# gongaa/Feedback-GNN

Measured on AMD Instinct MI355X. Metric: decoded codewords/sec, [[882,24]] 64-iter BP4 + feedback-GNN, higher is better.
Workload: dtype f32

## Files before the change

### feedback_gnn_amd/_lib.py

```python
import ctypes as C
import os
import subprocess

_HERE = os.path.dirname(os.path.abspath(__file__))
LIB_PATH = os.path.join(_HERE, "lib", "libfgnn_hip.so")
CSRC = os.path.join(_HERE, "csrc")

CN_TYPES = {"boxplus": 0, "boxplus-phi": 1, "minsum": 2}
ROWS_X_LOGIT, ROWS_Z_LOGIT, ROWS_HX_PERP, ROWS_HZ_PERP, ROWS_LX, ROWS_LZ = 0, 1, 2, 3, 4, 5


class FgnnError(RuntimeError):
    pass


def build(force=False, verbose=False):
    cmd = ["make", "-C", CSRC, "-j4"] + (["-B"] if force else [])
    res = subprocess.run(cmd, stdout=subprocess.PIPE, stderr=subprocess.STDOUT, text=True)
    if verbose or res.returncode != 0:
        print(res.stdout)
    if res.returncode != 0:
        raise FgnnError("building libfgnn_hip.so failed")
    return LIB_PATH


KERNEL_SOURCES = {
    "bp4": ("fgnn_bp4.hip", "fgnn_math.h", "fgnn_math_ranged.h", "fgnn_internal.h", "fgnn_rng.h", "fgnn_cn.h", "Makefile"),
    "gnn": ("fgnn_gnn.hip", "fgnn_math.h", "fgnn_internal.h", "fgnn_pk.h", "fgnn_mlp.h", "Makefile"),
    "gnnbp4": ("fgnn_gnnbp4.hip", "fgnn_math.h", "fgnn_internal.h", "fgnn_pk.h", "fgnn_mlp.h", "Makefile"),
}


def source_fingerprint(kind):
    import hashlib
    h = hashlib.sha256()
    for name in KERNEL_SOURCES[kind]:
        h.update(name.encode() + b"\0")
        with open(os.path.join(CSRC, name), "rb") as f:
            h.update(f.read())
        h.update(b"\0")
    return h.hexdigest()


def library_sha256(path=None):
    import hashlib
    h = hashlib.sha256()
    with open(path or os.environ.get("FGNN_LIB_PATH", LIB_PATH), "rb") as f:
        for blk in iter(lambda: f.read(1 << 20), b""):
            h.update(blk)
    return h.hexdigest()


_SIGNATURES = {
    "fgnn_last_error": (C.c_char_p, []),
    "fgnn_version": (C.c_int, []),
    "fgnn_graph_create": (C.c_int, [C.c_int, C.c_int, C.c_int, C.c_int, C.c_void_p, C.c_void_p, C.c_int, C.c_void_p,
                                    C.c_void_p, C.c_int, C.POINTER(C.c_void_p)]),
    "fgnn_graph_destroy": (None, [C.c_void_p]),
    "fgnn_graph_set_rows": (C.c_int, [C.c_void_p, C.c_int, C.c_int, C.c_int, C.c_void_p, C.c_void_p]),
    "fgnn_graph_set_launch": (C.c_int, [C.c_void_p, C.c_int, C.c_int]),
    "fgnn_graph_set_option": (C.c_int, [C.c_void_p, C.c_int, C.c_int]),
    "fgnn_graph_force_generic": (C.c_int, [C.c_void_p, C.c_int]),
    "fgnn_graph_info": (C.c_int, [C.c_void_p, C.c_void_p]),
    "fgnn_graph_edges": (C.c_int, [C.c_void_p, C.c_int, C.c_void_p, C.c_void_p]),
    "fgnn_profile_enable": (C.c_int, [C.c_void_p, C.c_int]),
    "fgnn_profile_read": (C.c_int, [C.c_void_p, C.c_void_p, C.c_void_p, C.c_void_p, C.c_int, C.c_void_p]),
    "fgnn_bp4_decode": (C.c_int, [C.c_void_p, C.c_int, C.c_int, C.c_float, C.c_void_p, C.c_float, C.c_void_p, C.c_void_p,
                                  C.c_int] + [C.c_void_p] * 10),
    "fgnn_bp4_decode_trace": (C.c_int, [C.c_void_p, C.c_int, C.c_int, C.c_float, C.c_void_p, C.c_float, C.c_void_p, C.c_void_p,
                                        C.c_int] + [C.c_void_p] * 10),
    "fgnn_weights_create": (C.c_int, [C.c_void_p, C.c_int, C.POINTER(C.c_void_p)]),
    "fgnn_weights_destroy": (None, [C.c_void_p]),
    "fgnn_feedback_gnn": (C.c_int, [C.c_void_p] * 7 + [C.c_int, C.c_void_p, C.c_void_p]),
    "fgnn_pauli_noise": (C.c_int, [C.c_uint64, C.c_float, C.c_uint64, C.c_int, C.c_int, C.c_void_p, C.c_void_p, C.c_void_p]),
    "fgnn_pauli_noise_xyz": (C.c_int, [C.c_uint64, C.c_float, C.c_float, C.c_float, C.c_uint64, C.c_int, C.c_int, C.c_void_p, C.c_void_p, C.c_void_p]),
    "fgnn_pauli_noise_wt": (C.c_int, [C.c_uint64, C.c_int, C.c_uint64, C.c_int, C.c_int, C.c_void_p, C.c_void_p, C.c_void_p]),
    "fgnn_pauli_noise_dev": (C.c_int, [C.c_uint64, C.c_float, C.c_void_p, C.c_uint64, C.c_int, C.c_int, C.c_void_p, C.c_void_p, C.c_void_p]),
    "fgnn_syndrome": (C.c_int, [C.c_void_p, C.c_void_p, C.c_void_p, C.c_int, C.c_void_p, C.c_void_p, C.c_void_p]),
    "fgnn_flag_update": (C.c_int, [C.c_void_p] * 5 + [C.c_int, C.c_void_p, C.c_void_p]),
    "fgnn_merge": (C.c_int, [C.c_void_p] * 3 + [C.c_int, C.c_int, C.c_void_p, C.c_void_p, C.c_void_p]),
    "fgnn_residual": (C.c_int, [C.c_void_p] * 5 + [C.c_int] + [C.c_void_p] * 4),
    "fgnn_count_flags": (C.c_int, [C.c_void_p, C.c_int, C.c_void_p, C.c_void_p]),
    "fgnn_count_flags_batches": (C.c_int, [C.c_void_p, C.c_int, C.c_int, C.c_void_p, C.c_void_p, C.c_void_p, C.c_void_p]),
    "fgnn_pack_decisions": (C.c_int, [C.c_void_p, C.c_void_p, C.c_int, C.c_int, C.c_void_p, C.c_void_p]),
    "fgnn_unpack_decisions": (C.c_int, [C.c_void_p, C.c_int, C.c_int, C.c_void_p, C.c_void_p, C.c_void_p]),
    "fgnn_sandwich_workspace_bytes": (C.c_size_t, [C.c_void_p, C.c_int]),
    "fgnn_sandwich_decode": (C.c_int, [C.c_void_p, C.c_int, C.c_void_p, C.c_void_p, C.c_void_p, C.c_void_p, C.c_float,
                                       C.c_void_p, C.c_void_p, C.c_int, C.c_int, C.c_void_p, C.c_void_p, C.c_void_p,
                                       C.c_void_p, C.c_void_p, C.c_size_t, C.c_void_p]),
    "fgnn_bp2_decode": (C.c_int, [C.c_void_p, C.c_int, C.c_int, C.c_float, C.c_void_p, C.c_float, C.c_void_p, C.c_int, C.c_void_p,
                                  C.c_void_p, C.c_void_p]),
    "fgnn_relay_decode": (C.c_int, [C.c_void_p, C.c_float, C.c_int, C.c_int, C.c_int, C.c_int, C.c_void_p, C.c_void_p, C.c_float,
                                    C.c_void_p, C.c_int, C.c_void_p, C.c_void_p, C.c_void_p]),
    "fgnn_relay4_decode": (C.c_int, [C.c_void_p, C.c_int, C.c_float, C.c_int, C.c_int, C.c_int, C.c_int, C.c_void_p, C.c_void_p, C.c_float,
                                     C.c_void_p, C.c_void_p, C.c_int, C.c_void_p, C.c_void_p, C.c_void_p, C.c_void_p]),
    "fgnn_bsc_noise": (C.c_int, [C.c_uint64, C.c_float, C.c_uint64, C.c_int, C.c_int, C.c_void_p, C.c_void_p]),
    "fgnn_residual_rows": (C.c_int, [C.c_void_p, C.c_int, C.c_int] + [C.c_void_p] * 4 + [C.c_int] + [C.c_void_p] * 4),
    "fgnn_graph_set_basis": (C.c_int, [C.c_void_p, C.c_int, C.c_int, C.c_void_p]),
    "fgnn_osd0": (C.c_int, [C.c_void_p, C.c_int, C.c_void_p, C.c_void_p, C.c_void_p, C.c_int, C.c_void_p, C.c_int, C.c_void_p, C.c_void_p]),
    "fgnn_osd": (C.c_int, [C.c_void_p, C.c_int, C.c_int, C.c_int, C.c_void_p, C.c_void_p, C.c_void_p, C.c_int, C.c_void_p, C.c_int,
                           C.c_void_p, C.c_void_p, C.c_void_p]),
    "fgnn_osd_resident": (C.c_int, [C.c_void_p, C.c_int, C.c_int, C.POINTER(C.c_int)]),
    "fgnn_osd_workspace_bytes": (C.c_int, [C.c_void_p, C.c_int, C.c_int, C.c_int, C.c_int, C.POINTER(C.c_size_t)]),
    "fgnn_osd_ws": (C.c_int, [C.c_void_p, C.c_int, C.c_int, C.c_int, C.c_void_p, C.c_void_p, C.c_void_p, C.c_int, C.c_void_p, C.c_int,
                              C.c_void_p, C.c_void_p, C.c_void_p, C.c_size_t, C.c_void_p]),
    "fgnn_compact": (C.c_int, [C.c_void_p, C.c_int, C.c_int, C.c_void_p, C.c_void_p, C.c_void_p]),
    "fgnn_gnnbp4_weights_create": (C.c_int, [C.c_void_p, C.c_int, C.c_int, C.c_int, C.POINTER(C.c_void_p)]),
    "fgnn_gnnbp4_weights_destroy": (None, [C.c_void_p]),
    "fgnn_gnnbp4_weights_create_general": (C.c_int, [C.c_void_p, C.c_void_p, C.c_void_p, C.c_int, C.POINTER(C.c_void_p)]),
    "fgnn_gnnbp4_weights_workspace_bytes": (C.c_size_t, [C.c_void_p, C.c_void_p, C.c_int]),
    "fgnn_gnnbp4_workspace_bytes": (C.c_size_t, [C.c_void_p, C.c_int]),
    "fgnn_gnnbp4_decode": (C.c_int, [C.c_void_p, C.c_void_p, C.c_int, C.c_void_p, C.c_void_p, C.c_int] + [C.c_void_p] * 6
                           + [C.c_size_t, C.c_void_p]),
    "fgnn_weights_create_general": (C.c_int, [C.c_void_p, C.c_void_p, C.c_int, C.c_int, C.POINTER(C.c_void_p)]),
    "fgnn_bp4_backward": (C.c_int, [C.c_void_p, C.c_int, C.c_float, C.c_void_p, C.c_void_p, C.c_void_p, C.c_int]
                          + [C.c_void_p] * 7),
    "fgnn_feedback_gnn_backward": (C.c_int, [C.c_void_p, C.c_void_p] + [C.c_void_p] * 5 + [C.c_int] + [C.c_void_p] * 9),
    "fgnn_feedback_gnn_backward_general": (C.c_int, [C.c_void_p, C.c_void_p] + [C.c_void_p] * 5 + [C.c_int] + [C.c_void_p] * 3
                                           + [C.c_int, C.c_void_p]),
    "fgnn_gnnbp4_grad_count": (C.c_int, [C.c_void_p, C.c_void_p, C.POINTER(C.c_int)]),
    "fgnn_gnnbp4_tape_bytes": (C.c_int, [C.c_void_p, C.c_void_p, C.c_int, C.c_int, C.POINTER(C.c_size_t)]),
    "fgnn_gnnbp4_backward_workspace_bytes": (C.c_int, [C.c_void_p, C.c_void_p, C.c_int, C.POINTER(C.c_size_t)]),
    "fgnn_gnnbp4_forward_tape": (C.c_int, [C.c_void_p, C.c_void_p, C.c_int, C.c_void_p, C.c_void_p, C.c_int, C.c_void_p, C.c_void_p,
                                           C.c_void_p, C.c_size_t, C.c_void_p]),
    "fgnn_gnnbp4_backward": (C.c_int, [C.c_void_p, C.c_void_p, C.c_int, C.c_void_p, C.c_void_p, C.c_int, C.c_void_p, C.c_size_t,
                                       C.c_void_p, C.c_void_p, C.c_void_p, C.c_int, C.c_void_p, C.c_size_t, C.c_void_p]),
}

ABI_SYMBOLS = tuple(_SIGNATURES)

_lib = None


def lib():
    global _lib
    if _lib is None:
        if not os.path.exists(LIB_PATH):
            raise FgnnError(f"{LIB_PATH} not found: run `python -c 'import __graft_entry__ as g; g.build()'` "
                            "(there is no CPU fallback for the decoder)")
        import torch
        override = os.environ.get("FGNN_LIB_PATH")
        L = C.CDLL(override or LIB_PATH)
        for name, (res, args) in _SIGNATURES.items():
            try:
                fn = getattr(L, name)
            except AttributeError:
                if override:
                    continue
                raise
            fn.restype = res
            fn.argtypes = args
        _lib = L
    return _lib


def check(rc):
    if rc != 0:
        msg = lib().fgnn_last_error().decode()
        if rc == -1:
            raise ValueError(msg)
        raise FgnnError(f"libfgnn_hip error {rc}: {msg}")
```

### feedback_gnn_amd/csrc/fgnn_bp4.hip

```cpp

#include <type_traits>

#include "fgnn_internal.h"
#include "fgnn_math.h"
#include "fgnn_math_ranged.h"
#include "fgnn_cn.h"

#ifndef FGNN_BP4_WAVES
#define FGNN_BP4_WAVES 7
#endif
#ifndef FGNN_HWT_PIN_CLIP_POINTS
#define FGNN_HWT_PIN_CLIP_POINTS 1
#endif
#ifndef FGNN_PHI_STAGE
#define FGNN_PHI_STAGE 1
#endif

namespace {

struct BpArgs {
    int B, num_iter, tpc, cpb, lds_per_cw, lch_off;
    float factor, llr_const;
    const float* llr_ch;
    const uint8_t* synd_x;
    const uint8_t* synd_z;
    const float* msg_init_x;
    const float* msg_init_z;
    float* llr_out;
    uint8_t* x_hat;
    uint8_t* z_hat;
    float* x_logit;
    float* z_logit;
    float* msg_out_x;
    float* msg_out_z;
    const int* index;
    int shortcut;
    int early_exit;
    int sig_off;
    int lreg;
    int hwt;
    uint8_t* flagged;
    int flag_off;
    float* gmem;
    float* trace_x;
    float* trace_z;
    int trace_off;
    float* tape_x;
    float* tape_z;
    int nt;
    int shared_lse;
};

template <bool HWT>
struct Mx {
    static __device__ __forceinline__ float softplus(float t) { return fg_softplus(t); }
    static __device__ __forceinline__ float lse2(float a, float b) { return fg_lse2_ranged(a, b); }
    static __device__ __forceinline__ float lse2_corr(float a, float b) { return fg_lse2_corr_ranged(a, b); }
    static __device__ __forceinline__ float phi(float x) { return fg_phi(x); }
};
template <>
struct Mx<true> {
    static __device__ __forceinline__ float exp(float x) { return __builtin_amdgcn_exp2f(x * FG_LOG2E); }
    static __device__ __forceinline__ float log(float x) { return __builtin_amdgcn_logf(x) * 0.693147182f; }
    static __device__ __forceinline__ float softplus(float t)
    {
        const float y = exp(FG_CLAMP(t, -87.0f, FG_SOFTPLUS_THRESH));
        const float r = (t < -FG_SOFTPLUS_THRESH) ? ((t < -87.0f) ? 0.0f : y) : log(1.0f + y);
        return (t > FG_SOFTPLUS_THRESH) ? t : r;
    }
    static __device__ __forceinline__ float lse2_corr(float a, float b)
    {
        const float y = exp(-FG_MIN(FG_ABS(a - b), 20.0f));
        return log(1.0f + y);
    }
    static __device__ __forceinline__ float lse2(float a, float b)
    {
        return lse2_corr(a, b) + FG_MAX(a, b);
    }
    static __device__ __forceinline__ float phi(float x)
    {
        const float xc = FG_CLAMP(x, FG_PHI_MIN, FG_PHI_MAX);
        const float y = exp(xc);
        const float sp = (xc > FG_SOFTPLUS_THRESH) ? xc : log(1.0f + y);
        float r = sp - log(y - 1.0f);
#if FGNN_HWT_PIN_CLIP_POINTS
        r = (x >= FG_PHI_MAX) ? 0.0f : r;
        r = (x <= FG_PHI_MIN) ? 16.6355324f : r;
#endif
        return r;
    }
};

template <bool HWT = false>
__device__ __forceinline__ float logit_row_opt(const float* llr, const int* __restrict__ col, int deg, float phi0, bool shortcut)
{
    if (shortcut) {
        unsigned neg = 0;
        bool sat = true;
        for (int j = 0; j < deg; ++j) {
            const float v = llr[col[j]];
            neg ^= (v < 0.0f);
            sat = sat && (FG_ABS(v) >= FG_PHI_MAX);
        }
        if (__all(sat)) return with_sign(phi0, neg);
    }
    return logit_row<Mx<HWT>>(llr, col, deg);
}

template <int N, bool HWT = false>
__device__ __forceinline__ void phi_n(const float (&x)[N], float (&out)[N])
{
    if constexpr (HWT) {
#pragma unroll
        for (int k = 0; k < N; ++k) out[k] = Mx<true>::phi(x[k]);
        return;
    }
    const float* tab = fg_log_tab();
    float xc[N], y[N];
    uint32_t eb1[N], eb2[N], j1[N], j2[N];
#pragma unroll
    for (int k = 0; k < N; ++k) {
        xc[k] = FG_CLAMP(x[k], FG_PHI_MIN, FG_PHI_MAX);
        y[k] = fg_exp(xc[k]);
        const uint32_t w1 = fg_f2u(1.0f + y[k]) - FG_LOG_OFFS;
        const uint32_t w2 = fg_f2u(y[k] - 1.0f) - FG_LOG_OFFS;
        eb1[k] = w1 & 0xff800000u;
        eb2[k] = w2 & 0xff800000u;
        j1[k] = (w1 >> 18) & 31u;
        j2[k] = (w2 >> 18) & 31u;
    }
    __builtin_amdgcn_sched_barrier(0);
    float rc1[N], lc1[N], rc2[N], lc2[N];
#pragma unroll
    for (int k = 0; k < N; ++k) {
        rc1[k] = tab[j1[k]];
        lc1[k] = tab[32 + j1[k]];
        rc2[k] = tab[j2[k]];
        lc2[k] = tab[32 + j2[k]];
    }
    __builtin_amdgcn_sched_barrier(0);
#pragma unroll
    for (int k = 0; k < N; ++k) {
        const float a = fg_u2f(fg_f2u(rc1[k]) - eb1[k]);
        const float r1 = FG_FMA(y[k], a, a - 1.0f);
        float sp = FG_FMA((float)(int32_t)eb1[k], FG_LN2_S23, lc1[k] + fg_log1p_small(r1));
        sp = (xc[k] > FG_SOFTPLUS_THRESH) ? xc[k] : sp;
        const float mm = fg_u2f(fg_f2u(y[k] - 1.0f) - eb2[k]);
        const float r2 = FG_FMA(mm, rc2[k], -1.0f);
        const float lg = FG_FMA((float)(int32_t)eb2[k], FG_LN2_S23, lc2[k] + fg_log1p_small(r2));
        out[k] = sp - lg;
    }
}

template <int DC, bool HWT = false, bool F1 = false>
__device__ __forceinline__ bool cn_phi_regular(float* msg, const int (&sl)[DC], uint32_t neg0, float factor, float phi0,
                                               bool shortcut)
{
    constexpr int H = (DC % FGNN_PHI_STAGE == 0) ? FGNN_PHI_STAGE : DC / 2;
    static_assert(DC % H == 0, "a phi stage must take a whole fraction of a check");
    float v[DC], aa[DC];
    uint32_t neg = neg0;
    bool sat = true;
#pragma unroll
    for (int j = 0; j < DC; ++j) {
        v[j] = slot_ref(msg, sl[j]);
        neg ^= fg_f2u(v[j]);
        sat = sat && (FG_ABS(v[j]) >= FG_PHI_MAX);
    }
    if (shortcut && __all(sat)) {
#pragma unroll
        for (int j = 0; j < DC; ++j) {
            const float o = fg_u2f(fg_f2u(phi0) | ((neg ^ fg_f2u(v[j])) & 0x80000000u));
            slot_ref(msg, sl[j]) = F1 ? o : o * factor;
        }
        return true;
    }
#pragma unroll
    for (int g0 = 0; g0 < DC; g0 += H) {
        float xa[H], oa[H];
#pragma unroll
        for (int j = 0; j < H; ++j) xa[j] = FG_ABS(v[g0 + j]);
        phi_n<H, HWT>(xa, oa);
#pragma unroll
        for (int j = 0; j < H; ++j) aa[g0 + j] = oa[j];
    }
    float T = 0.0f;
#pragma unroll
    for (int j = 0; j < DC; ++j) T = T + aa[j];
#pragma unroll
    for (int g0 = 0; g0 < DC; g0 += H) {
        float xa[H], oa[H];
#pragma unroll
        for (int j = 0; j < H; ++j) xa[j] = T - aa[g0 + j];
        phi_n<H, HWT>(xa, oa);
#pragma unroll
        for (int j = 0; j < H; ++j) {
            const float o = fg_u2f(fg_f2u(oa[j]) | ((neg ^ fg_f2u(v[g0 + j])) & 0x80000000u));
            slot_ref(msg, sl[g0 + j]) = F1 ? o : o * factor;
        }
    }
    return false;
}

template <int DC>
__device__ __forceinline__ void cn_tanh_regular(float* msg, const int (&sl)[DC], unsigned synd, float factor)
{
    float t[DC];
    float P = 1.0f;
#pragma unroll
    for (int j = 0; j < DC; ++j) {
        float tj = fg_tanh(slot_ref(msg, sl[j]) / 2.0f);
        tj = (tj == 0.0f) ? 1e-12f : tj;
        P = (j == 0) ? tj : P * tj;
        t[j] = tj;
    }
    P = P * (synd ? -1.0f : 1.0f);
    const float clipv = 0.99999988f;
#pragma unroll
    for (int j = 0; j < DC; ++j) {
        float q = fg_rcp_unit(t[j]) * P;
        q = (FG_ABS(q) < 1e-7f) ? 0.0f : q;
        q = FG_MIN(FG_MAX(q, -clipv), clipv);
        slot_ref(msg, sl[j]) = (2.0f * fg_atanh(q)) * factor;
    }
}

template <bool HWT = false>
__device__ __forceinline__ bool cn_phi_generic(float* msg, const int* __restrict__ slot, int deg, unsigned synd, float factor,
                                               float phi0, bool shortcut)
{
    if (shortcut) {
        unsigned neg = synd;
        bool sat = true;
        for (int j = 0; j < deg; ++j) {
            const float v = msg[slot[j]];
            neg ^= (v < 0.0f);
            sat = sat && (FG_ABS(v) >= FG_PHI_MAX);
        }
        if (__all(sat)) {
            for (int j = 0; j < deg; ++j) {
                const int s = slot[j];
                msg[s] = with_sign(phi0, neg ^ (unsigned)(msg[s] < 0.0f)) * factor;
            }
            return true;
        }
    }
    cn_update<FGNN_CN_BOXPLUS_PHI, Mx<HWT>>(msg, slot, deg, synd, factor);
    return false;
}

__device__ __forceinline__ float softplus_saturated(float t)
{
    const float y = fg_exp(FG_MIN(FG_MAX(t, -87.0f), 0.0f));
    return (t > 0.0f) ? t : ((t < -87.0f) ? 0.0f : y);
}

template <int CN_TYPE, int DVX, int DVZ, int DC, bool OPT, bool HWT = false, int NQ = 0, bool TRACE = false, bool GMEM = false, int LSE = 2,
          int NT = 0>
__global__ void __launch_bounds__(1024) __attribute__((amdgpu_waves_per_eu(NQ > 0 ? FGNN_BP4_WAVES - 1 : FGNN_BP4_WAVES)))
bp4_kernel(GraphDev g, BpArgs a)
{
    static_assert(!(HWT && OPT), "the hardware-transcendental variant is the fixed dataflow only: the exact shortcuts are proofs about fgnn_math.h");
    static_assert(!GMEM || (DVX == 0 && !OPT && !HWT && NQ == 0 && !TRACE), "the global-memory variant is the plain runtime-degree kernel");
    using MX = Mx<HWT>;
    FG_LOG_TAB_SETUP();
    constexpr bool REGULAR = DVX > 0;
    constexpr bool LREG = NQ > 0;
    constexpr int NQA = LREG ? NQ : 1;
    static_assert(NT == 0 || (DVX > 0 && CN_TYPE == FGNN_CN_BOXPLUS_PHI && !LREG && !TRACE && !GMEM), "compile-time trips: the regular phi kernel");
    constexpr int CT = LREG ? NQ : NT;
    const int tpc = NT > 0 ? 256 : a.tpc;
    const bool opt_shortcut = OPT && a.shortcut != 0;
    const bool opt_exit = OPT && a.early_exit != 0;
    const bool shl = LSE == 2 ? a.shared_lse != 0 : LSE == 1;
    extern __shared__ float lds[];
    const int cwl = NT > 0 ? 0 : threadIdx.x / tpc;
    const int lane = threadIdx.x - cwl * tpc;
    const int slot_b = NT > 0 ? blockIdx.x : blockIdx.x * a.cpb + cwl;
    const bool active = slot_b < a.B;
    const int b = (active && a.index) ? a.index[slot_b] : slot_b;
    float* msg;
    if constexpr (GMEM) msg = a.gmem + (size_t)slot_b * a.lds_per_cw;
    else if constexpr (NT > 0) msg = lds;
    else msg = lds + (size_t)cwl * a.lds_per_cw;
    float* Lch = msg + a.lch_off;
    const int n = g.n;

    constexpr bool CLOSED_OK = REGULAR && CN_TYPE == FGNN_CN_BOXPLUS_PHI && !LREG && !TRACE;
    const bool zero_start = REGULAR && !TRACE && !a.msg_init_x && !a.msg_init_z && a.num_iter > 0;
    const bool first_closed = CLOSED_OK && zero_start && !a.llr_ch;
    const bool first_peeled = zero_start && a.llr_ch != nullptr;
    const bool fill = !first_closed && !first_peeled;
    if (active) {
        if (fill) {
            for (int e = lane; e < g.E_x; e += tpc) msg[e] = a.msg_init_x ? a.msg_init_x[(size_t)b * g.E_x + e] : 0.0f;
            for (int e = lane; e < g.E_z; e += tpc)
                msg[g.E_x + e] = a.msg_init_z ? a.msg_init_z[(size_t)b * g.E_z + e] : 0.0f;
        }
        if (a.llr_ch && !LREG)
            for (int i = lane; i < 3 * n; i += tpc) Lch[i] = a.llr_ch[(size_t)b * 3 * n + i];
    }
    float lreg[3][NQA];
    if constexpr (LREG) {
#pragma unroll
        for (int i = 0; i < NQ; ++i) {
            const int v = lane + i * tpc;
            const bool in = active && v < n;
#pragma unroll
            for (int c = 0; c < 3; ++c) lreg[c][i] = in ? a.llr_ch[(size_t)b * 3 * n + c * n + v] : 0.0f;
        }
    }
    if (fill || (a.llr_ch && !LREG)) __syncthreads();

    const uint8_t* sx = a.synd_x + (size_t)b * g.m_x;
    const uint8_t* sz = a.synd_z + (size_t)b * g.m_z;
    const int lane_c = lane + (tpc >> 1) < tpc ? lane + (tpc >> 1) : lane - tpc + (tpc >> 1);

    const float phi0 = MX::phi(0.0f);
    (void)phi0;
    unsigned* sigw = reinterpret_cast<unsigned*>(msg + a.sig_off);
    int* flags = reinterpret_cast<int*>(sigw + n);
    bool a1 = false, a2 = false;
    if (opt_exit) {
        for (int v = lane; v < n; v += tpc) sigw[v] = fill ? 0xffffffffu : 0u;
        if (lane < 4) flags[lane] = 0;
        __syncthreads();
    }
    int it_begin = 0;
    if constexpr (CLOSED_OK) {
        if (first_closed) {
            const float L = a.llr_const;
            const float Y = (0.0f + 0.0f) + L, X = 0.0f + L, Z = 0.0f + L;
            const float nu_x = MX::softplus(-X) - MX::lse2(-(Z - 0.0f), -(Y - 0.0f));
            const float nu_z = MX::softplus(-Z) - MX::lse2(-(X - 0.0f), -(Y - 0.0f));
            if (active)
                for (int c = lane_c; c < g.m; c += tpc) {
                    const unsigned synd = (c < g.m_x ? sx[c] : sz[c - g.m_x]) & 1u;
                    const uint4 pk = reinterpret_cast<const uint4*>(g.cslot16)[c];
                    const unsigned w[4] = {pk.x, pk.y, pk.z, pk.w};
                    const float nu = c < g.m_x ? nu_x : nu_z;
                    const unsigned ng = nu < 0.0f;
                    unsigned neg = synd;
                    const float aa = MX::phi(FG_ABS(nu));
                    float T = 0.0f;
#pragma unroll
                    for (int j = 0; j < DC; ++j) {
                        neg ^= ng;
                        T = T + aa;
                    }
                    const float val = with_sign(MX::phi(T - aa), neg ^ ng) * a.factor;
#pragma unroll
                    for (int j = 0; j < DC; ++j) slot_ref(msg, (int)((w[j >> 1] >> ((j & 1) * 16)) & 0xffffu)) = val;
                }
            if (opt_exit) a1 = FG_ABS(nu_x) >= FG_PHI_MAX && FG_ABS(nu_z) >= FG_PHI_MAX;
            it_begin = 1;
            __syncthreads();
        }
    }
    const bool cn_one = a.cpb == 1, cn_f1 = a.factor == 1.0f;
    unsigned synd_bits = 0;
    if (active) {
        int i = 0;
        for (int c = lane_c; c < g.m && i < 32; c += tpc, ++i) synd_bits |= ((c < g.m_x ? sx[c] : sz[c - g.m_x]) & 1u) << i;
    }
    const bool synd_in_reg = (g.m + tpc - 1) / tpc <= 32;
    unsigned row_off = 16u * (unsigned)lane_c;
    auto trace_step = [&](const int k) __attribute__((always_inline)) {
        float* tlx = msg + a.trace_off;
        float* tlz = tlx + n;
        if (active && a.tape_x) {
            float* px = a.tape_x + ((size_t)k * a.B + b) * g.E_x;
            float* pz = a.tape_z + ((size_t)k * a.B + b) * g.E_z;
            for (int e = lane; e < g.E_x; e += tpc) px[e] = msg[e];
            for (int e = lane; e < g.E_z; e += tpc) pz[e] = msg[g.E_x + e];
        }
        if (active)
            for (int v = lane; v < n; v += tpc) {
                const int x0 = g.vptr_x[v], x1 = g.vptr_x[v + 1], z0 = g.vptr_z[v], z1 = g.vptr_z[v + 1];
                float Sz = 0.0f, Sx = 0.0f;
                for (int e = z0; e < z1; ++e) Sz = Sz + msg[e];
                for (int e = x0; e < x1; ++e) Sx = Sx + msg[e];
                const float lx = a.llr_ch ? Lch[v] : a.llr_const, ly = a.llr_ch ? Lch[n + v] : a.llr_const,
                            lz = a.llr_ch ? Lch[2 * n + v] : a.llr_const;
                const float Y = (Sz + Sx) + ly;
                const float X = Sz + lx;
                const float Z = Sx + lz;
                tlz[v] = MX::softplus(-X) - MX::lse2(-Z, -Y);
                tlx[v] = MX::softplus(-Z) - MX::lse2(-X, -Y);
            }
        __syncthreads();
        if (active) {
            float* tx = a.trace_x + ((size_t)k * a.B + b) * g.rows[0];
            for (int r = lane; r < g.rows[0]; r += tpc) {
                const int p0 = g.rptr[0][r];
                tx[r] = logit_row<Mx<HWT>>(tlx, g.rcol[0] + p0, g.rptr[0][r + 1] - p0);
            }
            float* tz = a.trace_z + ((size_t)k * a.B + b) * g.rows[1];
            for (int r = lane; r < g.rows[1]; r += tpc) {
                const int p0 = g.rptr[1][r];
                tz[r] = logit_row<Mx<HWT>>(tlz, g.rcol[1] + p0, g.rptr[1][r + 1] - p0);
            }
        }
    };
    if constexpr (TRACE) trace_step(0);
    if constexpr (REGULAR && !TRACE) {
        if (first_peeled && active) {
            auto vn_first = [&](const int v, const float lx, const float ly, const float lz) __attribute__((always_inline)) {
                const float Y = (0.0f + 0.0f) + ly;
                const float X = 0.0f + lx;
                const float Z = 0.0f + lz;
                const float numx = MX::softplus(-X);
                const float numz = MX::softplus(-Z);
                const float Ze = Z - 0.0f, Xe = X - 0.0f, Ye = Y - 0.0f;
                float ox, oz;
                if (shl) {
                    ox = numx - (MX::lse2_corr(-Z, -Y) + FG_MAX(-Ze, -Ye));
                    oz = numz - (MX::lse2_corr(-X, -Y) + FG_MAX(-Xe, -Ye));
                } else {
                    ox = numx - MX::lse2(-Ze, -Ye);
                    oz = numz - MX::lse2(-Xe, -Ye);
                }
                float* px = msg + v * DVX;
                float* pz = msg + g.E_x + v * DVZ;
#pragma unroll
                for (int k = 0; k < DVX; ++k) px[k] = ox;
#pragma unroll
                for (int k = 0; k < DVZ; ++k) pz[k] = oz;
            };
            if constexpr (LREG) {
#pragma unroll
                for (int i = 0; i < NQ; ++i) {
                    const int v = lane + i * tpc;
                    if (v < n) vn_first(v, lreg[0][i], lreg[1][i], lreg[2][i]);
                }
            } else {
                for (int v = lane; v < n; v += tpc) vn_first(v, Lch[v], Lch[n + v], Lch[2 * n + v]);
            }
        }
    }
    for (int it = it_begin; it < a.num_iter; ++it) {
        bool changed = false, cn_slow = false;
        auto vn_body = [&](const int v, const float lx, const float ly, const float lz) __attribute__((always_inline)) {
                if constexpr (REGULAR) {
                    float* px = msg + v * DVX;
                    float* pz = msg + g.E_x + v * DVZ;
                    float mx[DVX], mz[DVZ];
                    float Sz = 0.0f, Sx = 0.0f;
#pragma unroll
                    for (int k = 0; k < DVZ; ++k) { mz[k] = pz[k]; Sz = Sz + mz[k]; }
#pragma unroll
                    for (int k = 0; k < DVX; ++k) { mx[k] = px[k]; Sx = Sx + mx[k]; }
                    if (opt_exit) {
                        unsigned sig = 0;
#pragma unroll
                        for (int k = 0; k < DVX; ++k) sig |= sign_bit(mx[k]) << k;
#pragma unroll
                        for (int k = 0; k < DVZ; ++k) sig |= sign_bit(mz[k]) << (DVX + k);
                        if (sigw[v] != sig) {
                            changed = true;
                            sigw[v] = sig;
                        }
                    }
                    const float Y = (Sz + Sx) + ly;
                    const float X = Sz + lx;
                    const float Z = Sx + lz;
                    bool sat = opt_shortcut && FG_ABS(X) > FG_SOFTPLUS_THRESH && FG_ABS(Z) > FG_SOFTPLUS_THRESH;
                    if (shl) {
                        sat = sat && FG_ABS((-Z) - (-Y)) >= 20.0f && FG_ABS((-X) - (-Y)) >= 20.0f;
                    } else {
#pragma unroll
                        for (int k = 0; k < DVX; ++k) sat = sat && (FG_ABS((Z - mx[k]) - (Y - mx[k])) >= 20.0f);
#pragma unroll
                        for (int k = 0; k < DVZ; ++k) sat = sat && (FG_ABS((X - mz[k]) - (Y - mz[k])) >= 20.0f);
                    }
                    if (opt_shortcut && __all(sat)) {
                        const float numx = softplus_saturated(-X);
                        const float numz = softplus_saturated(-Z);
#pragma unroll
                        for (int k = 0; k < DVX; ++k) {
                            const float Ze = Z - mx[k], Ye = Y - mx[k];
                            px[k] = numx - (0.0f + FG_MAX(-Ze, -Ye));
                        }
#pragma unroll
                        for (int k = 0; k < DVZ; ++k) {
                            const float Xe = X - mz[k], Ye = Y - mz[k];
                            pz[k] = numz - (0.0f + FG_MAX(-Xe, -Ye));
                        }
                        return;
                    }
                    const float numx = MX::softplus(-X);
                    const float numz = MX::softplus(-Z);
                    if (shl) {
                        const float cx = MX::lse2_corr(-Z, -Y), cz = MX::lse2_corr(-X, -Y);
#pragma unroll
                        for (int k = 0; k < DVX; ++k) {
                            const float Ze = Z - mx[k], Ye = Y - mx[k];
                            px[k] = numx - (cx + FG_MAX(-Ze, -Ye));
                        }
#pragma unroll
                        for (int k = 0; k < DVZ; ++k) {
                            const float Xe = X - mz[k], Ye = Y - mz[k];
                            pz[k] = numz - (cz + FG_MAX(-Xe, -Ye));
                        }
                        return;
                    }
#pragma unroll
                    for (int k = 0; k < DVX; ++k) {
                        const float Ze = Z - mx[k], Ye = Y - mx[k];
                        px[k] = numx - MX::lse2(-Ze, -Ye);
                    }
#pragma unroll
                    for (int k = 0; k < DVZ; ++k) {
                        const float Xe = X - mz[k], Ye = Y - mz[k];
                        pz[k] = numz - MX::lse2(-Xe, -Ye);
                    }
                } else {
                    const int x0 = g.vptr_x[v], x1 = g.vptr_x[v + 1], z0 = g.vptr_z[v], z1 = g.vptr_z[v + 1];
                    float Sz = 0.0f, Sx = 0.0f;
                    for (int e = z0; e < z1; ++e) Sz = Sz + msg[e];
                    for (int e = x0; e < x1; ++e) Sx = Sx + msg[e];
                    const float Y = (Sz + Sx) + ly;
                    const float X = Sz + lx;
                    const float Z = Sx + lz;
                    if (opt_shortcut) {
                        bool sat = FG_ABS(X) > FG_SOFTPLUS_THRESH && FG_ABS(Z) > FG_SOFTPLUS_THRESH;
                        if (shl) sat = sat && FG_ABS((-Z) - (-Y)) >= 20.0f && FG_ABS((-X) - (-Y)) >= 20.0f;
                        unsigned sig = 0;
                        for (int e = x0; e < x1; ++e) {
                            const float mm = msg[e];
                            sat = sat && (shl || FG_ABS((Z - mm) - (Y - mm)) >= 20.0f);
                            sig |= sign_bit(mm) << (e - x0);
                        }
                        for (int e = z0; e < z1; ++e) {
                            const float mm = msg[e];
                            sat = sat && (shl || FG_ABS((X - mm) - (Y - mm)) >= 20.0f);
                            sig |= sign_bit(mm) << ((x1 - x0) + (e - z0));
                        }
                        if (opt_exit && sigw[v] != sig) {
                            changed = true;
                            sigw[v] = sig;
                        }
                        if (__all(sat)) {
                            const float nx = softplus_saturated(-X), nz = softplus_saturated(-Z);
                            for (int e = x0; e < x1; ++e) {
                                const float mm = msg[e];
                                const float Ze = Z - mm, Ye = Y - mm;
                                msg[e] = nx - (0.0f + FG_MAX(-Ze, -Ye));
                            }
                            for (int e = z0; e < z1; ++e) {
                                const float mm = msg[e];
                                const float Xe = X - mm, Ye = Y - mm;
                                msg[e] = nz - (0.0f + FG_MAX(-Xe, -Ye));
                            }
                            return;
                        }
                    }
                    const float numx = MX::softplus(-X);
                    const float numz = MX::softplus(-Z);
                    if (shl) {
                        const float cx = MX::lse2_corr(-Z, -Y), cz = MX::lse2_corr(-X, -Y);
                        for (int e = x0; e < x1; ++e) {
                            float m = msg[e];
                            float Ze = Z - m, Ye = Y - m;
                            msg[e] = numx - (cx + FG_MAX(-Ze, -Ye));
                        }
                        for (int e = z0; e < z1; ++e) {
                            float m = msg[e];
                            float Xe = X - m, Ye = Y - m;
                            msg[e] = numz - (cz + FG_MAX(-Xe, -Ye));
                        }
                        return;
                    }
                    for (int e = x0; e < x1; ++e) {
                        float m = msg[e];
                        float Ze = Z - m, Ye = Y - m;
                        msg[e] = numx - MX::lse2(-Ze, -Ye);
                    }
                    for (int e = z0; e < z1; ++e) {
                        float m = msg[e];
                        float Xe = X - m, Ye = Y - m;
                        msg[e] = numz - MX::lse2(-Xe, -Ye);
                    }
                }
            };
        if (active && !(first_peeled && it == 0)) {
            if constexpr (LREG) {
#pragma unroll
                for (int i = 0; i < NQ; ++i) {
                    const int v = lane + i * tpc;
                    if (v < n) vn_body(v, lreg[0][i], lreg[1][i], lreg[2][i]);
                }
            } else if constexpr (NT > 0) {
#pragma unroll
                for (int i = 0; i < NT; ++i) {
                    const int v = lane + i * 256;
                    if (i + 1 < NT || v < n) vn_body(v, a.llr_const, a.llr_const, a.llr_const);
                }
            } else {
                for (int v = lane; v < n; v += tpc) {
                    if (a.llr_ch) vn_body(v, Lch[v], Lch[n + v], Lch[2 * n + v]);
                    else vn_body(v, a.llr_const, a.llr_const, a.llr_const);
                }
            }
        }
        if (opt_exit && changed) flags[2 * (it & 1)] = 1;
        __syncthreads();
        if (opt_exit && lane == 0) {
            flags[2 * ((it + 1) & 1)] = 0;
            flags[2 * ((it + 1) & 1) + 1] = 0;
        }
        if constexpr (REGULAR && CT > 0 && CN_TYPE == FGNN_CN_BOXPLUS_PHI) {
            auto cn_trips = [&](auto f1) __attribute__((always_inline)) {
                constexpr bool F1 = decltype(f1)::value;
                const char* rows = reinterpret_cast<const char*>(g.cslot16);
#pragma unroll
                for (int i = 0; i < CT; ++i) {
                    const bool in = (!LREG && i + 1 < CT) || lane_c + i * tpc < g.m;
                    if (in) {
                        const char* base = rows + (size_t)i * (size_t)(16u * (unsigned)tpc);
                        asm volatile("" : "+v"(row_off));
                        if constexpr (NT > 0) asm volatile("" : "+s"(base));
                        typedef unsigned Row __attribute__((ext_vector_type(4)));
                        const Row pk = *(const __attribute__((address_space(1))) Row*)(base + row_off);
                        const unsigned w[4] = {pk.x, pk.y, pk.z, pk.w};
                        int sl[DC];
#pragma unroll
                        for (int j = 0; j < DC; ++j) sl[j] = (int)((w[j >> 1] >> ((j & 1) * 16)) & 0xffffu);
                        const bool fast = cn_phi_regular<DC, HWT, F1>(lds, sl, synd_bits << (31 - i), F1 ? 1.0f : a.factor, phi0, opt_shortcut);
                        cn_slow = !fast || cn_slow;
                    }
                }
            };
            if (active) {
                if (cn_f1) cn_trips(std::true_type{});
                else cn_trips(std::false_type{});
            }
        } else if (active) {
            int ci = 0;
            for (int c = lane_c; c < g.m; c += tpc, ++ci) {
                const unsigned synd = synd_in_reg ? (synd_bits >> ci) & 1u : (c < g.m_x ? sx[c] : sz[c - g.m_x]) & 1u;
                if constexpr (REGULAR) {
                    const uint4 pk = reinterpret_cast<const uint4*>(g.cslot16)[c];
                    const unsigned w[4] = {pk.x, pk.y, pk.z, pk.w};
                    int sl[DC];
#pragma unroll
                    for (int j = 0; j < DC; ++j) sl[j] = (int)((w[j >> 1] >> ((j & 1) * 16)) & 0xffffu);
                    if constexpr (CN_TYPE == FGNN_CN_BOXPLUS_PHI) {
                        bool fast;
                        if (cn_one && cn_f1) fast = cn_phi_regular<DC, HWT, true>(lds, sl, synd << 31, 1.0f, phi0, opt_shortcut);
                        else if (cn_one) fast = cn_phi_regular<DC, HWT, false>(lds, sl, synd << 31, a.factor, phi0, opt_shortcut);
                        else fast = cn_phi_regular<DC, HWT, false>(msg, sl, synd << 31, a.factor, phi0, opt_shortcut);
                        cn_slow = !fast || cn_slow;
                    } else if constexpr (CN_TYPE == FGNN_CN_MINSUM) {
                        cn_minsum_regular<DC>(msg, sl, DC, synd, a.factor);
                    } else {
                        cn_tanh_regular<DC>(msg, sl, synd, a.factor);
                    }
                } else {
                    const int c0 = g.cptr[c], deg = g.cptr[c + 1] - c0;
                    if constexpr (CN_TYPE == FGNN_CN_BOXPLUS_PHI)
                        cn_slow = !cn_phi_generic<HWT>(msg, g.cslot + c0, deg, synd, a.factor, phi0, opt_shortcut) || cn_slow;
                    else cn_update<CN_TYPE, Mx<HWT>>(msg, g.cslot + c0, deg, synd, a.factor);
                }
            }
        }
        if (opt_exit && cn_slow) flags[2 * (it & 1) + 1] = 1;
        __syncthreads();
        if (opt_exit) {
            const bool stable = a1 && a2 && flags[2 * (it & 1)] == 0;
            a2 = a1;
            a1 = flags[2 * (it & 1) + 1] == 0;
            if (stable) break;
        }
        if constexpr (TRACE) trace_step(it + 1);
    }

    if (active) {
        if (a.msg_out_x)
            for (int e = lane; e < g.E_x; e += tpc) a.msg_out_x[(size_t)b * g.E_x + e] = msg[e];
        if (a.msg_out_z)
            for (int e = lane; e < g.E_z; e += tpc) a.msg_out_z[(size_t)b * g.E_z + e] = msg[g.E_x + e];
    }
    auto total_body = [&](const int v, const float lx, const float ly, const float lz) __attribute__((always_inline)) {
            const int x0 = g.vptr_x[v], x1 = g.vptr_x[v + 1], z0 = g.vptr_z[v], z1 = g.vptr_z[v + 1];
            float Sz = 0.0f, Sx = 0.0f;
            for (int e = z0; e < z1; ++e) Sz = Sz + msg[e];
            for (int e = x0; e < x1; ++e) Sx = Sx + msg[e];
            const float Y = (Sz + Sx) + ly;
            const float X = Sz + lx;
            const float Z = Sx + lz;
            float* o = a.llr_out + (size_t)b * 3 * n;
            o[v] = X;
            o[n + v] = Y;
            o[2 * n + v] = Z;
            int d = 0;
            float best = 0.0f;
            if (X < best) { best = X; d = 1; }
            if (Z < best) { best = Z; d = 2; }
            if (Y < best) { best = Y; d = 3; }
            a.x_hat[(size_t)b * n + v] = (uint8_t)(d & 1);
            a.z_hat[(size_t)b * n + v] = (uint8_t)(d >> 1);
    };
    if (active) {
        if constexpr (LREG) {
#pragma unroll
            for (int i = 0; i < NQ; ++i) {
                const int v = lane + i * tpc;
                if (v < n) total_body(v, lreg[0][i], lreg[1][i], lreg[2][i]);
            }
        } else {
            for (int v = lane; v < n; v += tpc) {
                if (a.llr_ch) total_body(v, Lch[v], Lch[n + v], Lch[2 * n + v]);
                else total_body(v, a.llr_const, a.llr_const, a.llr_const);
            }
        }
    }
    if (a.flagged) {
        uint8_t* dec = reinterpret_cast<uint8_t*>(msg + a.flag_off);
        unsigned* fword = reinterpret_cast<unsigned*>(dec + ((n + 3) & ~3));
        __syncthreads();
        if (active)
            for (int v = lane; v < n; v += tpc) {
                dec[v] = (uint8_t)(a.x_hat[(size_t)b * n + v] | (a.z_hat[(size_t)b * n + v] << 1));
            }
        if (lane == 0) *fword = 0u;
        __syncthreads();
        unsigned mine = 0;
        if (active)
            for (int c = lane; c < g.m; c += tpc) {
                const int sh = c < g.m_x ? 1 : 0;
                unsigned par = (c < g.m_x ? sx[c] : sz[c - g.m_x]) & 1u;
                for (int e = g.cptr[c]; e < g.cptr[c + 1]; ++e) par ^= (dec[g.cvn[e]] >> sh) & 1u;
                mine |= par;
            }
        if (mine) atomicOr(fword, 1u);
        __syncthreads();
        if (active && lane == 0) a.flagged[b] = (uint8_t)(*fword != 0u);
    }
    if (!a.x_logit && !a.z_logit) return;
    __syncthreads();
    float* llx = msg;
    float* llz = msg + n;
    if (active)
        for (int v = lane; v < n; v += tpc) {
            const float* o = a.llr_out + (size_t)b * 3 * n;
            const float X = o[v], Y = o[n + v], Z = o[2 * n + v];
            const bool sat = opt_shortcut && FG_ABS(X) > FG_SOFTPLUS_THRESH && FG_ABS(Z) > FG_SOFTPLUS_THRESH &&
                             FG_ABS((-Z) - (-Y)) >= 20.0f && FG_ABS((-X) - (-Y)) >= 20.0f;
            if (opt_shortcut && __all(sat)) {
                llz[v] = softplus_saturated(-X) - (0.0f + FG_MAX(-Z, -Y));
                llx[v] = softplus_saturated(-Z) - (0.0f + FG_MAX(-X, -Y));
                continue;
            }
            llz[v] = MX::softplus(-X) - MX::lse2(-Z, -Y);
            llx[v] = MX::softplus(-Z) - MX::lse2(-X, -Y);
        }
    __syncthreads();
    if (active) {
        if (a.x_logit)
            for (int r = lane; r < g.rows[0]; r += tpc) {
                const int p0 = g.rptr[0][r];
                a.x_logit[(size_t)b * g.rows[0] + r] = logit_row_opt<HWT>(llx, g.rcol[0] + p0, g.rptr[0][r + 1] - p0, phi0, opt_shortcut);
            }
        if (a.z_logit)
            for (int r = lane; r < g.rows[1]; r += tpc) {
                const int p0 = g.rptr[1][r];
                a.z_logit[(size_t)b * g.rows[1] + r] = logit_row_opt<HWT>(llz, g.rcol[1] + p0, g.rptr[1][r + 1] - p0, phi0, opt_shortcut);
            }
    }
}

using Bp4Kernel = void (*)(GraphDev, BpArgs);

template <int NQ, bool OPT, int LSE, int NT = 0>
constexpr Bp4Kernel bp4_lse_kernel = bp4_kernel<FGNN_CN_BOXPLUS_PHI, 3, 3, 6, OPT, false, NQ, false, false, LSE, NT>;
constexpr Bp4Kernel bp4_lse_kernels[3][2][2] = {
    {{bp4_lse_kernel<0, false, 0>, bp4_lse_kernel<0, false, 1>}, {bp4_lse_kernel<0, true, 0>, bp4_lse_kernel<0, true, 1>}},
    {{bp4_lse_kernel<4, false, 0>, bp4_lse_kernel<4, false, 1>}, {bp4_lse_kernel<4, true, 0>, bp4_lse_kernel<4, true, 1>}},
    {{bp4_lse_kernel<5, false, 0>, bp4_lse_kernel<5, false, 1>}, {bp4_lse_kernel<5, true, 0>, bp4_lse_kernel<5, true, 1>}}};

constexpr Bp4Kernel bp4_nt_kernels[2][2][2] = {
    {{bp4_lse_kernel<0, false, 0, 4>, bp4_lse_kernel<0, false, 1, 4>}, {bp4_lse_kernel<0, true, 0, 4>, bp4_lse_kernel<0, true, 1, 4>}},
    {{bp4_lse_kernel<0, false, 0, 5>, bp4_lse_kernel<0, false, 1, 5>}, {bp4_lse_kernel<0, true, 0, 5>, bp4_lse_kernel<0, true, 1, 5>}}};

template <int CN_TYPE, int DVX, int DVZ, int DC>
int launch_bp4_k(const fgnn_graph* g, const BpArgs& a, const LaunchGeom& L, size_t lds_bytes, hipStream_t st)
{
    Bp4Kernel kern = a.shortcut ? bp4_kernel<CN_TYPE, DVX, DVZ, DC, true> : bp4_kernel<CN_TYPE, DVX, DVZ, DC, false>;
    if constexpr ((DVX == 3 && DVZ == 3 && DC == 6) || DVX == 0) {
        if (a.trace_x) kern = bp4_kernel<CN_TYPE, DVX, DVZ, DC, false, false, 0, true>;
    }
    if constexpr (CN_TYPE == FGNN_CN_BOXPLUS_PHI) {
        if (a.hwt) kern = bp4_kernel<CN_TYPE, DVX, DVZ, DC, false, true>;
        if constexpr (DVX == 3 && DVZ == 3 && DC == 6) {
            if (!a.trace_x && !a.hwt) kern = bp4_lse_kernels[a.lreg ? a.lreg - 3 : 0][a.shortcut][a.shared_lse];
            if (!a.trace_x && !a.hwt && a.nt) kern = bp4_nt_kernels[a.nt - 4][a.shortcut][a.shared_lse];
        }
    }
    return fgnn_launch(kern, dim3(L.blocks), dim3(L.threads), lds_bytes, st, g->d, a);
}

struct Bp4Plan {
    size_t lds_bytes;
    bool gmem;
    size_t ws_bytes;
};

template <int CN_TYPE>
int launch_bp4(const fgnn_graph* g, const BpArgs& a, const LaunchGeom& L, const Bp4Plan& p, hipStream_t st)
{
    if (p.gmem)
        return fgnn_launch(bp4_kernel<CN_TYPE, 0, 0, 0, false, false, 0, false, true>, dim3(L.blocks), dim3(L.threads), 0, st, g->d, a);
    const GraphDev& d = g->d;
    if (d.cslot16 && !g->force_generic) {
        if (d.dvx == 3 && d.dvz == 3 && d.dc == 6) return launch_bp4_k<CN_TYPE, 3, 3, 6>(g, a, L, p.lds_bytes, st);
        if (d.dvx == 4 && d.dvz == 4 && d.dc == 8 && !a.trace_x) return launch_bp4_k<CN_TYPE, 4, 4, 8>(g, a, L, p.lds_bytes, st);
    }
    return launch_bp4_k<CN_TYPE, 0, 0, 0>(g, a, L, p.lds_bytes, st);
}

Bp4Plan plan_bp4(const fgnn_graph* g, int cn_type, const LaunchGeom& L, BpArgs& a, bool gmem = false)
{
    const GraphDev& d = g->d;
    const int n = d.n;
    const bool trace = a.trace_x != nullptr, phi = cn_type == FGNN_CN_BOXPLUS_PHI;
    auto round4 = [](int floats) { return (floats + 3) & ~3; };
    a.shared_lse = g->bp4_shared_lse ? 1 : 0;
    a.hwt = (g->hw_transcendentals && phi && !trace && !gmem) ? 1 : 0;
    a.shortcut = (g->shortcut && !a.hwt && !trace && !gmem) ? 1 : 0;
    a.lch_off = d.E > 2 * n ? d.E : 2 * n;
    const int per_thread = (n + L.tpc - 1) / L.tpc, per_thread_c = (d.m + L.tpc - 1) / L.tpc;
    const int trips = per_thread > per_thread_c ? per_thread : per_thread_c;
    const bool r336 = d.cslot16 && !g->force_generic && d.dvx == 3 && d.dvz == 3 && d.dc == 6;
    const bool fixed_trips = !trace && !a.hwt && !gmem && phi && L.cpb == 1 && r336;
    a.lreg = (a.llr_ch && fixed_trips && trips <= 5) ? (trips <= 4 ? 4 : 5) : 0;
    a.nt = (!a.llr_ch && fixed_trips && L.tpc == 256 && per_thread == per_thread_c && (trips == 4 || trips == 5)) ? trips : 0;
    int per = a.lch_off + ((a.llr_ch && !a.lreg) ? 3 * n : 0);
    a.trace_off = 0;
    if (trace) {
        a.trace_off = per;
        per += 2 * n;
    }
    if (!gmem) per = round4(per);
    a.sig_off = per;
    int tail = 0;
    a.early_exit = (a.shortcut && g->early_exit && d.max_vdeg <= 32 && phi && L.cpb == 1 && a.num_iter > 2) ? 1 : 0;
    if (a.early_exit) {
        if (((size_t)per * L.cpb + n + 4) * sizeof(float) <= FGNN_LDS_BUDGET) tail += n + 4;
        else a.early_exit = 0;
    }
    a.flag_off = 0;
    if (a.flagged) {
        const int need = round4(n) / 4 + 1;
        if (a.lch_off >= 2 * n + need) {
            a.flag_off = 2 * n;
        } else {
            a.flag_off = per + tail;
            tail += need;
        }
    }
    if (gmem) {
        a.lds_per_cw = round4(per + tail);
        return {0, true, (size_t)L.blocks * (size_t)a.lds_per_cw * sizeof(float)};
    }
    a.lds_per_cw = per;
    const size_t lds_bytes = ((size_t)per * L.cpb + tail) * sizeof(float);
    if (lds_bytes > FGNN_LDS_BUDGET) return plan_bp4(g, cn_type, L, a, true);
    return {lds_bytes, false, 0};
}

}

static int bp4_decode_core(const fgnn_graph* g, int cn_type, int num_iter, float normalization_factor, const float* llr_ch,
                           float llr_const, const uint8_t* synd_x, const uint8_t* synd_z, int B, const float* msg_init_x,
                           const float* msg_init_z, float* llr_out, uint8_t* x_hat, uint8_t* z_hat, float* x_logit,
                           float* z_logit, float* msg_out_x, float* msg_out_z, const int* index, uint8_t* flagged,
                           float* trace_x, float* trace_z, float* tape_x, float* tape_z, void* stream)
{
    if (!g) return fgnn_fail(FGNN_ERR_ARG, "graph is NULL");
    if (B < 0 || num_iter < 0) return fgnn_fail(FGNN_ERR_ARG, "B and num_iter must be >= 0");
    if (cn_type < 0 || cn_type > 2) return fgnn_fail(FGNN_ERR_ARG, "Unknown node type.");
    if ((x_logit && !g->d.rptr[0]) || (z_logit && !g->d.rptr[1]))
        return fgnn_fail(FGNN_ERR_STATE, "logit row sets not installed (fgnn_graph_set_rows)");
    if (B == 0) return FGNN_OK;
    if (!synd_x || !synd_z || !llr_out || !x_hat || !z_hat) return fgnn_fail(FGNN_ERR_ARG, "required buffer is NULL");
    FGNN_DEVICE_GUARD(g->device);
    const LaunchGeom L = fgnn_geom(g, B);
    if (flagged && L.cpb != 1) return fgnn_fail(FGNN_ERR_STATE, "the fused flag test needs one codeword per workgroup");
    BpArgs a;
    a.B = B;
    a.num_iter = num_iter;
    a.tpc = L.tpc;
    a.cpb = L.cpb;
    a.factor = normalization_factor;
    a.llr_const = llr_const;
    a.llr_ch = llr_ch;
    a.synd_x = synd_x;
    a.synd_z = synd_z;
    a.msg_init_x = msg_init_x;
    a.msg_init_z = msg_init_z;
    a.llr_out = llr_out;
    a.x_hat = x_hat;
    a.z_hat = z_hat;
    a.x_logit = x_logit;
    a.z_logit = z_logit;
    a.msg_out_x = msg_out_x;
    a.msg_out_z = msg_out_z;
    a.index = index;
    a.flagged = flagged;
    a.gmem = nullptr;
    a.trace_x = trace_x;
    a.trace_z = trace_z;
    a.tape_x = tape_x;
    a.tape_z = tape_z;
    const Bp4Plan p = plan_bp4(g, cn_type, L, a);
    hipStream_t st = static_cast<hipStream_t>(stream);
    if (p.gmem) {
        if (trace_x) return fgnn_fail(FGNN_ERR_ARG, "code too large for the LDS-resident trace kernel");
        if (L.cpb != 1) return fgnn_fail(FGNN_ERR_STATE, "the global-memory BP4 variant needs one codeword per workgroup");
        const size_t row_bytes = (size_t)a.lds_per_cw * sizeof(float);
        {
            size_t free_b = 0, total_b = 0;
            if (hipMemGetInfo(&free_b, &total_b) == hipSuccess && p.ws_bytes > free_b)
                return fgnn_fail(FGNN_ERR_ARG, "code too large for the LDS-resident kernel: the global-memory variant needs " +
                                                   std::to_string(p.ws_bytes >> 20) + " MiB of workspace for " + std::to_string(B) +
                                                   " codewords (" + std::to_string(row_bytes >> 10) + " KiB each) and " +
                                                   std::to_string(free_b >> 20) + " MiB are free: decode in batches of at most " +
                                                   std::to_string(free_b / (row_bytes * 2)) + " codewords");
        }
        void* ws = nullptr;
        FGNN_HIP_CHECK(hipMallocAsync(&ws, p.ws_bytes, st));
        a.gmem = static_cast<float*>(ws);
    }
    fgnn_prof_scope prof(g, st);
    int rc;
    switch (cn_type) {
    case FGNN_CN_BOXPLUS_PHI: rc = launch_bp4<FGNN_CN_BOXPLUS_PHI>(g, a, L, p, st); break;
    case FGNN_CN_MINSUM: rc = launch_bp4<FGNN_CN_MINSUM>(g, a, L, p, st); break;
    default: rc = launch_bp4<FGNN_CN_BOXPLUS>(g, a, L, p, st); break;
    }
    if (a.gmem) (void)hipFreeAsync(a.gmem, st);
    if (rc == FGNN_OK) prof.done(num_iter, B);
    return rc;
}

int fgnn_bp4_decode_impl(const fgnn_graph* g, int cn_type, int num_iter, float normalization_factor, const float* llr_ch,
                         float llr_const, const uint8_t* synd_x, const uint8_t* synd_z, int B, const float* msg_init_x,
                         const float* msg_init_z, float* llr_out, uint8_t* x_hat, uint8_t* z_hat, float* x_logit,
                         float* z_logit, float* msg_out_x, float* msg_out_z, const int* index, uint8_t* flagged, void* stream)
{
    return bp4_decode_core(g, cn_type, num_iter, normalization_factor, llr_ch, llr_const, synd_x, synd_z, B, msg_init_x, msg_init_z,
                           llr_out, x_hat, z_hat, x_logit, z_logit, msg_out_x, msg_out_z, index, flagged, nullptr, nullptr, nullptr,
                           nullptr, stream);
}

extern "C" int fgnn_bp4_decode_trace(const fgnn_graph* g, int cn_type, int num_iter, float normalization_factor,
                                     const float* llr_ch, float llr_const, const uint8_t* synd_x, const uint8_t* synd_z, int B,
                                     const float* msg_init_x, const float* msg_init_z, float* llr_out, uint8_t* x_hat,
                                     uint8_t* z_hat, float* x_logit_trace, float* z_logit_trace, float* tape_x,
                                     float* tape_z, void* stream)
{
    if (B == 0 && g) return FGNN_OK;
    if (!x_logit_trace || !z_logit_trace) return fgnn_fail(FGNN_ERR_ARG, "trace buffer is NULL");
    if ((tape_x == nullptr) != (tape_z == nullptr)) return fgnn_fail(FGNN_ERR_ARG, "tape_x and tape_z go together");
    if (g && (!g->d.rptr[0] || !g->d.rptr[1]))
        return fgnn_fail(FGNN_ERR_STATE, "logit row sets not installed (fgnn_graph_set_rows)");
    return bp4_decode_core(g, cn_type, num_iter, normalization_factor, llr_ch, llr_const, synd_x, synd_z, B, msg_init_x, msg_init_z,
                           llr_out, x_hat, z_hat, nullptr, nullptr, nullptr, nullptr, nullptr, nullptr, x_logit_trace,
                           z_logit_trace, tape_x, tape_z, stream);
}

extern "C" int fgnn_bp4_decode(const fgnn_graph* g, int cn_type, int num_iter, float normalization_factor,
                               const float* llr_ch, float llr_const, const uint8_t* synd_x, const uint8_t* synd_z, int B,
                               const float* msg_init_x, const float* msg_init_z, float* llr_out, uint8_t* x_hat,
                               uint8_t* z_hat, float* x_logit, float* z_logit, float* msg_out_x, float* msg_out_z,
                               void* stream)
{
    return fgnn_bp4_decode_impl(g, cn_type, num_iter, normalization_factor, llr_ch, llr_const, synd_x, synd_z, B, msg_init_x,
                                msg_init_z, llr_out, x_hat, z_hat, x_logit, z_logit, msg_out_x, msg_out_z, nullptr, nullptr, stream);
}
```

### feedback_gnn_amd/csrc/fgnn_channel.hip

```cpp
#include "fgnn_internal.h"
#include "fgnn_math.h"
#include "fgnn_rng.h"

namespace {

template <bool XYZ>
__global__ void __launch_bounds__(256) pauli_kernel(uint64_t seed, float p, fg_pauli_thr thr_in, uint64_t first,
                                                    const unsigned long long* __restrict__ base, int B, int n, int nblk,
                                                    uint8_t* __restrict__ ex, uint8_t* __restrict__ ez)
{
    const long long t = (long long)blockIdx.x * blockDim.x + threadIdx.x;
    if (t >= (long long)B * nblk) return;
    if (base) first += (uint64_t)*base;
    const int b = (int)(t / nblk), blk = (int)(t - (long long)b * nblk);
    const fg_pauli_thr thr = XYZ ? thr_in : fg_pauli_thresholds(p);
    float u[4];
    fg_uniform4(seed, first + (uint64_t)b, (uint32_t)blk, u);
    const int q0 = blk * 4;
#pragma unroll
    for (int k = 0; k < 4; ++k)
        if (q0 + k < n) {
            ex[(size_t)b * n + q0 + k] = fg_pauli_x(u[k], thr);
            ez[(size_t)b * n + q0 + k] = fg_pauli_z(u[k], thr);
        }
}

__global__ void __launch_bounds__(256) pauli_wt_kernel(uint64_t seed, int wt, uint64_t first, int B, int n, uint8_t* __restrict__ ex,
                                                       uint8_t* __restrict__ ez)
{
    extern __shared__ unsigned short perm_all[];
    const int wave = threadIdx.x >> 6, lane = threadIdx.x & 63;
    const int b = blockIdx.x * 4 + wave;
    if (b >= B) return;
    unsigned short* perm = perm_all + (size_t)wave * n;
    uint8_t* rx = ex + (size_t)b * n;
    uint8_t* rz = ez + (size_t)b * n;
    for (int v = lane; v < n; v += 64) {
        perm[v] = (unsigned short)v;
        rx[v] = 0;
        rz[v] = 0;
    }
    __builtin_amdgcn_fence(__ATOMIC_RELEASE, "workgroup");
    __builtin_amdgcn_wave_barrier();
    __builtin_amdgcn_fence(__ATOMIC_ACQUIRE, "workgroup");
    if (lane != 0) return;
    float up[4] = {0, 0, 0, 0}, ut[4] = {0, 0, 0, 0};
    for (int i = 0; i < wt; ++i) {
        if ((i & 3) == 0) {
            fg_uniform4s(seed, first + (uint64_t)b, (uint32_t)(i >> 2), 1u, up);
            fg_uniform4s(seed, first + (uint64_t)b, (uint32_t)(i >> 2), 2u, ut);
        }
        const int j = i + fg_fy_pick(up[i & 3], n - i);
        const unsigned short t = perm[i];
        perm[i] = perm[j];
        perm[j] = t;
        const float u = ut[i & 3];
        rx[perm[i]] = (uint8_t)(u < (2.0f / 3.0f));
        rz[perm[i]] = (uint8_t)(u > (1.0f / 3.0f));
    }
}

__device__ __forceinline__ unsigned row_parity(const uint8_t* x, const int* __restrict__ col, int p0, int p1)
{
    unsigned a = 0;
    for (int j = p0; j < p1; ++j) a ^= x[col[j]];
    return a & 1u;
}

__global__ void __launch_bounds__(1024) syndrome_kernel(GraphDev g, int B, int tpc, int cpb, const uint8_t* __restrict__ ex,
                                                        const uint8_t* __restrict__ ez, uint8_t* __restrict__ sx,
                                                        uint8_t* __restrict__ sz)
{
    extern __shared__ uint8_t sm[];
    const int cwl = threadIdx.x / tpc, lane = threadIdx.x - cwl * tpc, b = blockIdx.x * cpb + cwl;
    const bool active = b < B;
    const int n = g.n;
    uint8_t* lx = sm + (size_t)cwl * 2 * n;
    uint8_t* lz = lx + n;
    if (active)
        for (int v = lane; v < n; v += tpc) {
            lx[v] = ex[(size_t)b * n + v];
            lz[v] = ez[(size_t)b * n + v];
        }
    __syncthreads();
    if (!active) return;
    for (int c = lane; c < g.m; c += tpc) {
        const int p0 = g.cptr[c], p1 = g.cptr[c + 1];
        if (c < g.m_x) sx[(size_t)b * g.m_x + c] = (uint8_t)row_parity(lz, g.cvn, p0, p1);
        else sz[(size_t)b * g.m_z + (c - g.m_x)] = (uint8_t)row_parity(lx, g.cvn, p0, p1);
    }
}

__global__ void __launch_bounds__(1024) flag_kernel(GraphDev g, int B, int tpc, int cpb, const uint8_t* __restrict__ xh,
                                                    const uint8_t* __restrict__ zh, const uint8_t* __restrict__ sx,
                                                    const uint8_t* __restrict__ sz, uint8_t* __restrict__ errors,
                                                    const int* __restrict__ index)
{
    extern __shared__ uint8_t sm[];
    const int cwl = threadIdx.x / tpc, lane = threadIdx.x - cwl * tpc, slot = blockIdx.x * cpb + cwl;
    const bool active = slot < B;
    const int b = (active && index) ? index[slot] : slot;
    const int n = g.n;
    unsigned* neq = reinterpret_cast<unsigned*>(sm);
    uint8_t* lx = sm + ((cpb * sizeof(unsigned) + 15) & ~size_t(15)) + (size_t)cwl * 2 * n;
    uint8_t* lz = lx + n;
    if (lane == 0) neq[cwl] = 0;
    if (active)
        for (int v = lane; v < n; v += tpc) {
            lx[v] = xh[(size_t)b * n + v];
            lz[v] = zh[(size_t)b * n + v];
        }
    __syncthreads();
    unsigned mine = 0;
    if (active)
        for (int c = lane; c < g.m; c += tpc) {
            const int p0 = g.cptr[c], p1 = g.cptr[c + 1];
            if (c < g.m_x) mine |= row_parity(lz, g.cvn, p0, p1) ^ (sx[(size_t)b * g.m_x + c] & 1u);
            else mine |= row_parity(lx, g.cvn, p0, p1) ^ (sz[(size_t)b * g.m_z + (c - g.m_x)] & 1u);
        }
    if (mine) atomicOr(&neq[cwl], 1u);
    __syncthreads();
    if (active && lane == 0) errors[b] = (uint8_t)((errors[b] != 0) && (neq[cwl] != 0));
}

__global__ void __launch_bounds__(256) merge_kernel(const uint8_t* __restrict__ errors, const uint8_t* __restrict__ xu,
                                                    const uint8_t* __restrict__ zu, long long total, int n,
                                                    uint8_t* __restrict__ xh, uint8_t* __restrict__ zh,
                                                    const int* __restrict__ index)
{
    long long i = (long long)blockIdx.x * blockDim.x + threadIdx.x;
    if (i >= total) return;
    if (index) {
        const long long slot = i / n;
        i = (long long)index[slot] * n + (i - slot * n);
    }
    if (errors[i / n]) {
        xh[i] = xu[i];
        zh[i] = zu[i];
    }
}

__global__ void __launch_bounds__(1024) residual_kernel(GraphDev g, int RX, int RZ, int B, int tpc, int cpb, const uint8_t* __restrict__ ex,
                                                        const uint8_t* __restrict__ ez, const uint8_t* __restrict__ xh,
                                                        const uint8_t* __restrict__ zh, uint8_t* __restrict__ s_hat,
                                                        uint8_t* __restrict__ ls_hat, uint8_t* __restrict__ flags)
{
    extern __shared__ uint8_t sm[];
    const int cwl = threadIdx.x / tpc, lane = threadIdx.x - cwl * tpc, b = blockIdx.x * cpb + cwl;
    const bool active = b < B;
    const int n = g.n;
    unsigned* fl = reinterpret_cast<unsigned*>(sm);
    uint8_t* xd = sm + ((cpb * sizeof(unsigned) + 15) & ~size_t(15)) + (size_t)cwl * 2 * n;
    uint8_t* zd = xd + n;
    if (lane == 0) fl[cwl] = 0;
    __syncthreads();
    unsigned any_diff = 0;
    if (active)
        for (int v = lane; v < n; v += tpc) {
            xd[v] = ex[(size_t)b * n + v] ^ xh[(size_t)b * n + v];
            zd[v] = ez[(size_t)b * n + v] ^ zh[(size_t)b * n + v];
            any_diff |= xd[v] | zd[v];
        }
    if (any_diff) atomicOr(&fl[cwl], 4u);
    __syncthreads();
    unsigned mine = 0;
    if (active && ((fl[cwl] & 4u) || s_hat || ls_hat)) {
        const int ms = g.m_z + g.m_x;
        for (int c = lane; c < g.m; c += tpc) {
            const int p0 = g.cptr[c], p1 = g.cptr[c + 1];
            unsigned bit;
            int pos;
            if (c < g.m_x) { bit = row_parity(zd, g.cvn, p0, p1); pos = g.m_z + c; }
            else { bit = row_parity(xd, g.cvn, p0, p1); pos = c - g.m_x; }
            if (s_hat) s_hat[(size_t)b * ms + pos] = (uint8_t)bit;
            mine |= bit;
        }
        const int r0 = g.rows[RX], r1 = g.rows[RZ];
        for (int r = lane; r < r0 + r1; r += tpc) {
            unsigned bit;
            if (r < r0) bit = row_parity(xd, g.rcol[RX], g.rptr[RX][r], g.rptr[RX][r + 1]);
            else bit = row_parity(zd, g.rcol[RZ], g.rptr[RZ][r - r0], g.rptr[RZ][r - r0 + 1]);
            if (ls_hat) ls_hat[(size_t)b * (r0 + r1) + r] = (uint8_t)bit;
            mine |= bit << 1;
        }
    }
    if (mine) atomicOr(&fl[cwl], mine);
    __syncthreads();
    if (active && lane == 0 && flags) flags[b] = (uint8_t)(fl[cwl] & 3u);
}

__global__ void __launch_bounds__(256) count_kernel(const uint8_t* __restrict__ flags, int B, unsigned long long* counts)
{
    __shared__ unsigned sh[2];
    if (threadIdx.x < 2) sh[threadIdx.x] = 0;
    __syncthreads();
    unsigned f = 0, l = 0;
    for (int i = blockIdx.x * blockDim.x + threadIdx.x; i < B; i += gridDim.x * blockDim.x) {
        f += flags[i] & 1u;
        l += (flags[i] >> 1) & 1u;
    }
    if (f) atomicAdd(&sh[0], f);
    if (l) atomicAdd(&sh[1], l);
    __syncthreads();
    if (threadIdx.x == 0) {
        if (sh[0]) atomicAdd(&counts[0], (unsigned long long)sh[0]);
        if (sh[1]) atomicAdd(&counts[1], (unsigned long long)sh[1]);
        if (blockIdx.x == 0) atomicAdd(&counts[2], (unsigned long long)B);
    }
}

__global__ void __launch_bounds__(256) count_batches_kernel(const uint8_t* __restrict__ flags, int batch, unsigned* __restrict__ part)
{
    __shared__ unsigned sh[2];
    if (threadIdx.x < 2) sh[threadIdx.x] = 0;
    __syncthreads();
    const uint8_t* f0 = flags + (size_t)blockIdx.x * batch;
    unsigned f = 0, l = 0;
    for (int i = threadIdx.x; i < batch; i += blockDim.x) {
        f += f0[i] & 1u;
        l += (f0[i] >> 1) & 1u;
    }
    if (f) atomicAdd(&sh[0], f);
    if (l) atomicAdd(&sh[1], l);
    __syncthreads();
    if (threadIdx.x < 2) part[2 * blockIdx.x + threadIdx.x] = sh[threadIdx.x];
}

__global__ void count_scan_kernel(const unsigned* __restrict__ part, int num_batches, int batch, unsigned long long* counts,
                                  unsigned long long* ring)
{
    if (blockIdx.x != 0 || threadIdx.x != 0) return;
    unsigned long long c0 = counts[0], c1 = counts[1], c2 = counts[2];
    for (int j = 0; j < num_batches; ++j) {
        c0 += part[2 * j];
        c1 += part[2 * j + 1];
        c2 += (unsigned long long)batch;
        ring[3 * j] = c0;
        ring[3 * j + 1] = c1;
        ring[3 * j + 2] = c2;
    }
    counts[0] = c0;
    counts[1] = c1;
    counts[2] = c2;
}

__global__ void __launch_bounds__(256) pack_kernel(const uint8_t* __restrict__ x_hat, const uint8_t* __restrict__ z_hat,
                                                   long long total, int n, int nb, uint8_t* __restrict__ packed)
{
    const long long i = (long long)blockIdx.x * blockDim.x + threadIdx.x;
    if (i >= total) return;
    const long long b = i / nb;
    const int byte = (int)(i - b * nb);
    const uint8_t* xr = x_hat + b * n;
    const uint8_t* zr = z_hat + b * n;
    unsigned v = 0;
#pragma unroll
    for (int k = 0; k < 8; ++k) {
        const int pos = byte * 8 + k;
        unsigned bit = 0;
        if (pos < n) bit = xr[pos] & 1u;
        else if (pos < 2 * n) bit = zr[pos - n] & 1u;
        v |= bit << (7 - k);
    }
    packed[i] = (uint8_t)v;
}

__global__ void __launch_bounds__(256) unpack_kernel(const uint8_t* __restrict__ packed, long long total, int n, int nb,
                                                     uint8_t* __restrict__ x_hat, uint8_t* __restrict__ z_hat)
{
    const long long i = (long long)blockIdx.x * blockDim.x + threadIdx.x;
    if (i >= total) return;
    const long long b = i / (2 * n);
    const int pos = (int)(i - b * 2 * n);
    const uint8_t v = (uint8_t)((packed[b * nb + (pos >> 3)] >> (7 - (pos & 7))) & 1u);
    if (pos < n) x_hat[b * n + pos] = v;
    else z_hat[b * n + pos - n] = v;
}

}

extern "C" int fgnn_pack_decisions(const uint8_t* x_hat, const uint8_t* z_hat, int B, int n, uint8_t* packed, void* stream)
{
    if (B < 0 || n <= 0) return fgnn_fail(FGNN_ERR_ARG, "bad pack arguments");
    if (B == 0) return FGNN_OK;
    if (!x_hat || !z_hat || !packed) return fgnn_fail(FGNN_ERR_ARG, "bad pack arguments");
    const int nb = (2 * n + 7) / 8;
    const long long total = (long long)B * nb;
    return fgnn_launch(pack_kernel, dim3((unsigned)((total + 255) / 256)), dim3(256), 0, static_cast<hipStream_t>(stream), x_hat,
                       z_hat, total, n, nb, packed);
}

extern "C" int fgnn_unpack_decisions(const uint8_t* packed, int B, int n, uint8_t* x_hat, uint8_t* z_hat, void* stream)
{
    if (B < 0 || n <= 0) return fgnn_fail(FGNN_ERR_ARG, "bad unpack arguments");
    if (B == 0) return FGNN_OK;
    if (!x_hat || !z_hat || !packed) return fgnn_fail(FGNN_ERR_ARG, "bad unpack arguments");
    const int nb = (2 * n + 7) / 8;
    const long long total = (long long)B * 2 * n;
    return fgnn_launch(unpack_kernel, dim3((unsigned)((total + 255) / 256)), dim3(256), 0, static_cast<hipStream_t>(stream), packed,
                       total, n, nb, x_hat, z_hat);
}

extern "C" int fgnn_pauli_noise(uint64_t seed, float p, uint64_t first_sample, int B, int n, uint8_t* noise_x,
                                uint8_t* noise_z, void* stream)
{
    if (B < 0 || n <= 0) return fgnn_fail(FGNN_ERR_ARG, "bad noise arguments");
    if (B == 0) return FGNN_OK;
    if (!noise_x || !noise_z) return fgnn_fail(FGNN_ERR_ARG, "bad noise arguments");
    const int nblk = (n + 3) / 4;
    const long long total = (long long)B * nblk;
    return fgnn_launch(pauli_kernel<false>, dim3((unsigned)((total + 255) / 256)), dim3(256), 0, static_cast<hipStream_t>(stream), seed,
                       p, fg_pauli_thr{0.0f, 0.0f, 0.0f}, first_sample, static_cast<const unsigned long long*>(nullptr), B, n, nblk,
                       noise_x, noise_z);
}

extern "C" int fgnn_pauli_noise_xyz(uint64_t seed, float px, float py, float pz, uint64_t first_sample, int B, int n,
                                    uint8_t* noise_x, uint8_t* noise_z, void* stream)
{
    if (B < 0 || n <= 0 || !(px == px && py == py && pz == pz)) return fgnn_fail(FGNN_ERR_ARG, "bad noise arguments");
    if (B == 0) return FGNN_OK;
    if (!noise_x || !noise_z) return fgnn_fail(FGNN_ERR_ARG, "bad noise arguments");
    const int nblk = (n + 3) / 4;
    const long long total = (long long)B * nblk;
    return fgnn_launch(pauli_kernel<true>, dim3((unsigned)((total + 255) / 256)), dim3(256), 0, static_cast<hipStream_t>(stream), seed,
                       0.0f, fg_pauli_thresholds_xyz(px, py, pz), first_sample, static_cast<const unsigned long long*>(nullptr), B, n,
                       nblk, noise_x, noise_z);
}

extern "C" int fgnn_pauli_noise_dev(uint64_t seed, float p, const uint64_t* first_sample_dev, uint64_t offset, int B, int n,
                                    uint8_t* noise_x, uint8_t* noise_z, void* stream)
{
    if (B < 0 || n <= 0 || !(p >= 0.0f && p <= 1.0f)) return fgnn_fail(FGNN_ERR_ARG, "bad noise arguments");
    if (B == 0) return FGNN_OK;
    if (!noise_x || !noise_z || !first_sample_dev) return fgnn_fail(FGNN_ERR_ARG, "bad noise arguments");
    const int nblk = (n + 3) / 4;
    const long long total = (long long)B * nblk;
    return fgnn_launch(pauli_kernel<false>, dim3((unsigned)((total + 255) / 256)), dim3(256), 0, static_cast<hipStream_t>(stream), seed,
                       p, fg_pauli_thr{0.0f, 0.0f, 0.0f}, offset, reinterpret_cast<const unsigned long long*>(first_sample_dev), B, n,
                       nblk, noise_x, noise_z);
}

extern "C" int fgnn_pauli_noise_wt(uint64_t seed, int wt, uint64_t first_sample, int B, int n, uint8_t* noise_x, uint8_t* noise_z,
                                   void* stream)
{
    if (B < 0 || n <= 0 || n > 65535 || wt < 0 || wt > n) return fgnn_fail(FGNN_ERR_ARG, "bad fixed-weight noise arguments");
    if (B == 0) return FGNN_OK;
    if (!noise_x || !noise_z) return fgnn_fail(FGNN_ERR_ARG, "bad fixed-weight noise arguments");
    return fgnn_launch(pauli_wt_kernel, dim3((B + 3) / 4), dim3(256), (size_t)4 * n * sizeof(unsigned short),
                       static_cast<hipStream_t>(stream), seed, wt, first_sample, B, n, noise_x, noise_z);
}

extern "C" int fgnn_syndrome(const fgnn_graph* g, const uint8_t* noise_x, const uint8_t* noise_z, int B, uint8_t* synd_x,
                             uint8_t* synd_z, void* stream)
{
    if (!g || B < 0) return fgnn_fail(FGNN_ERR_ARG, "bad syndrome arguments");
    if (B == 0) return FGNN_OK;
    if (!noise_x || !noise_z || !synd_x || !synd_z) return fgnn_fail(FGNN_ERR_ARG, "bad syndrome arguments");
    FGNN_DEVICE_GUARD(g->device);
    LaunchGeom L = fgnn_geom(g, B);
    size_t lds = (size_t)L.cpb * 2 * g->d.n;
    return fgnn_launch(syndrome_kernel, dim3(L.blocks), dim3(L.threads), lds, static_cast<hipStream_t>(stream), g->d, B, L.tpc,
                       L.cpb, noise_x, noise_z, synd_x, synd_z);
}

int fgnn_flag_update_impl(const fgnn_graph* g, const uint8_t* x_hat, const uint8_t* z_hat, const uint8_t* synd_x,
                          const uint8_t* synd_z, int B, uint8_t* errors, const int* index, void* stream)
{
    if (!g || B < 0) return fgnn_fail(FGNN_ERR_ARG, "bad flag arguments");
    if (B == 0) return FGNN_OK;
    if (!x_hat || !z_hat || !synd_x || !synd_z || !errors) return fgnn_fail(FGNN_ERR_ARG, "bad flag arguments");
    FGNN_DEVICE_GUARD(g->device);
    LaunchGeom L = fgnn_geom(g, B);
    size_t lds = ((L.cpb * sizeof(unsigned) + 15) & ~size_t(15)) + (size_t)L.cpb * 2 * g->d.n;
    return fgnn_launch(flag_kernel, dim3(L.blocks), dim3(L.threads), lds, static_cast<hipStream_t>(stream), g->d, B, L.tpc, L.cpb,
                       x_hat, z_hat, synd_x, synd_z, errors, index);
}

extern "C" int fgnn_flag_update(const fgnn_graph* g, const uint8_t* x_hat, const uint8_t* z_hat, const uint8_t* synd_x,
                                const uint8_t* synd_z, int B, uint8_t* errors, void* stream)
{
    return fgnn_flag_update_impl(g, x_hat, z_hat, synd_x, synd_z, B, errors, nullptr, stream);
}

int fgnn_merge_impl(const uint8_t* errors, const uint8_t* x_upd, const uint8_t* z_upd, int B, int n, uint8_t* x_hat, uint8_t* z_hat,
                    const int* index, void* stream)
{
    if (B < 0 || n <= 0) return fgnn_fail(FGNN_ERR_ARG, "bad merge arguments");
    if (B == 0) return FGNN_OK;
    if (!errors || !x_upd || !z_upd || !x_hat || !z_hat) return fgnn_fail(FGNN_ERR_ARG, "bad merge arguments");
    const long long total = (long long)B * n;
    return fgnn_launch(merge_kernel, dim3((unsigned)((total + 255) / 256)), dim3(256), 0, static_cast<hipStream_t>(stream), errors,
                       x_upd, z_upd, total, n, x_hat, z_hat, index);
}

extern "C" int fgnn_merge(const uint8_t* errors, const uint8_t* x_upd, const uint8_t* z_upd, int B, int n, uint8_t* x_hat,
                          uint8_t* z_hat, void* stream)
{
    return fgnn_merge_impl(errors, x_upd, z_upd, B, n, x_hat, z_hat, nullptr, stream);
}

extern "C" int fgnn_residual_rows(const fgnn_graph* g, int rows_x, int rows_z, const uint8_t* noise_x, const uint8_t* noise_z,
                                  const uint8_t* x_hat, const uint8_t* z_hat, int B, uint8_t* s_hat, uint8_t* ls_hat, uint8_t* flags,
                                  void* stream)
{
    if (!g || B < 0) return fgnn_fail(FGNN_ERR_ARG, "bad residual arguments");
    if (rows_x < 0 || rows_x > 5 || rows_z < 0 || rows_z > 5 || !g->d.rptr[rows_x] || !g->d.rptr[rows_z])
        return fgnn_fail(FGNN_ERR_STATE, "row sets for the residual check not installed (fgnn_graph_set_rows)");
    if (B == 0) return FGNN_OK;
    if (!noise_x || !noise_z || !x_hat || !z_hat) return fgnn_fail(FGNN_ERR_ARG, "bad residual arguments");
    FGNN_DEVICE_GUARD(g->device);
    LaunchGeom L = fgnn_geom(g, B);
    size_t lds = ((L.cpb * sizeof(unsigned) + 15) & ~size_t(15)) + (size_t)L.cpb * 2 * g->d.n;
    return fgnn_launch(residual_kernel, dim3(L.blocks), dim3(L.threads), lds, static_cast<hipStream_t>(stream), g->d, rows_x, rows_z, B,
                       L.tpc, L.cpb, noise_x, noise_z, x_hat, z_hat, s_hat, ls_hat, flags);
}

extern "C" int fgnn_residual(const fgnn_graph* g, const uint8_t* noise_x, const uint8_t* noise_z, const uint8_t* x_hat,
                             const uint8_t* z_hat, int B, uint8_t* s_hat, uint8_t* ls_hat, uint8_t* flags, void* stream)
{
    return fgnn_residual_rows(g, FGNN_ROWS_HX_PERP, FGNN_ROWS_HZ_PERP, noise_x, noise_z, x_hat, z_hat, B, s_hat, ls_hat, flags, stream);
}

extern "C" int fgnn_count_flags_batches(const uint8_t* flags, int num_batches, int batch, uint64_t* counts, uint64_t* ring,
                                        uint32_t* scratch, void* stream)
{
    if (!flags || !counts || !ring || !scratch || num_batches < 0 || batch <= 0) return fgnn_fail(FGNN_ERR_ARG, "bad count arguments");
    if (num_batches == 0) return FGNN_OK;
    hipStream_t st = static_cast<hipStream_t>(stream);
    const int rc = fgnn_launch(count_batches_kernel, dim3(num_batches), dim3(256), 0, st, flags, batch, scratch);
    if (rc) return rc;
    return fgnn_launch(count_scan_kernel, dim3(1), dim3(64), 0, st, scratch, num_batches, batch,
                       reinterpret_cast<unsigned long long*>(counts), reinterpret_cast<unsigned long long*>(ring));
}

extern "C" int fgnn_count_flags(const uint8_t* flags, int B, uint64_t* counts, void* stream)
{
    if (!counts || B < 0) return fgnn_fail(FGNN_ERR_ARG, "bad count arguments");
    if (B == 0) return FGNN_OK;
    if (!flags) return fgnn_fail(FGNN_ERR_ARG, "bad count arguments");
    int blocks = (B + 255) / 256;
    if (blocks > 1024) blocks = 1024;
    return fgnn_launch(count_kernel, dim3(blocks), dim3(256), 0, static_cast<hipStream_t>(stream), flags, B,
                       reinterpret_cast<unsigned long long*>(counts));
}
```

### feedback_gnn_amd/csrc/fgnn_gnn.hip

```cpp
#include <algorithm>
#include <cstring>

#include "fgnn_internal.h"
#include "fgnn_math.h"
#include "fgnn_mlp.h"
#include "fgnn_pk.h"

namespace {

constexpr int HID = 40;
constexpr int MSG = 20;

struct GnnArgs {
    int B, tpc, cpb, lds_per_cw;
    const float* llr;
    const float* logit_hx;
    const float* logit_hz;
    const uint8_t* synd_x;
    const uint8_t* synd_z;
    float* out;
    const int* index;
    int nsplit;
};

__device__ __forceinline__ void edge_mlp(float gv, float X, float Y, float Z, scalar_fp w1t, scalar_fp b1, scalar_fp w2, scalar_fp b2,
                                         float (&msg)[MSG])
{
#pragma unroll
    for (int i = 0; i < MSG; ++i) msg[i] = 0.0f;
#pragma unroll 2
    for (int j = 0; j < HID; ++j) {
        scalar_fp r = w1t + j * 4;
        float a = 0.0f;
        a = FG_FMA(gv, r[0], a);
        a = FG_FMA(X, r[1], a);
        a = FG_FMA(Y, r[2], a);
        a = FG_FMA(Z, r[3], a);
        const float h = fg_tanh(a + b1[j]);
        scalar_fp r2 = w2 + j * MSG;
#pragma unroll
        for (int i = 0; i < MSG; ++i) msg[i] = FG_FMA(h, r2[i], msg[i]);
    }
#pragma unroll
    for (int i = 0; i < MSG; ++i) msg[i] = msg[i] + b2[i];
}

__device__ __forceinline__ void side_mean(const GraphDev& g, const int* __restrict__ vptr, int v, const float* gcn,
                                          float X, float Y, float Z, scalar_fp w1t, scalar_fp b1, scalar_fp w2, scalar_fp b2,
                                          float (&mean)[MSG])
{
    const int e0 = vptr[v], e1 = vptr[v + 1];
    float msg[MSG];
#pragma unroll
    for (int i = 0; i < MSG; ++i) mean[i] = 0.0f;
    for (int e = e0; e < e1; ++e) {
        edge_mlp(gcn[g.vchk[e]], X, Y, Z, w1t, b1, w2, b2, msg);
#pragma unroll
        for (int i = 0; i < MSG; ++i) mean[i] = (e == e0) ? msg[i] : mean[i] + msg[i];
    }
    const int deg = e1 - e0;
    if (deg > 0) {
        const float fd = (float)deg;
#pragma unroll
        for (int i = 0; i < MSG; ++i) mean[i] = mean[i] / fd;
    }
}

__device__ __forceinline__ void side_mean_factored(const GraphDev& g, const int* __restrict__ vptr, int v, const float* gcn,
                                                   float X, float Y, float Z, scalar_fp w1t, scalar_fp b1, scalar_fp w2, scalar_fp b2,
                                                   float (&mean)[MSG])
{
    const int e0 = vptr[v], e1 = vptr[v + 1];
#pragma unroll
    for (int i = 0; i < MSG; ++i) mean[i] = 0.0f;
#pragma unroll 2
    for (int j = 0; j < HID; ++j) {
        scalar_fp r = w1t + j * 4;
        float a = 0.0f;
        a = FG_FMA(X, r[1], a);
        a = FG_FMA(Y, r[2], a);
        a = FG_FMA(Z, r[3], a);
        const float pb = a + b1[j];
        float hs = 0.0f;
        for (int e = e0; e < e1; ++e) {
            const float h = fg_tanh(FG_FMA(gcn[g.vchk[e]], r[0], pb));
            hs = (e == e0) ? h : hs + h;
        }
        scalar_fp r2 = w2 + j * MSG;
#pragma unroll
        for (int i = 0; i < MSG; ++i) mean[i] = FG_FMA(hs, r2[i], mean[i]);
    }
    const int deg = e1 - e0;
    if (deg > 0) {
        const float fd = (float)deg;
#pragma unroll
        for (int i = 0; i < MSG; ++i) mean[i] = mean[i] / fd + b2[i];
    }
}

enum {
    T_W1 = 0,
    T_B1 = 6,
    T_W2 = 26,
    T_B2 = 66,
    T_WE = 76,
    T_BE = 109,
    T_WO = 119,
    T_BO = 129,
    T_W10 = 132,
    T_COUNT = 152
};

#ifndef FGNN_GNN_CPB
#define FGNN_GNN_CPB 4
#endif
#ifdef FGNN_GNN_WAVES
#define FGNN_GNN_OCC __attribute__((amdgpu_waves_per_eu(FGNN_GNN_WAVES, FGNN_GNN_WAVES)))
#else
#define FGNN_GNN_OCC
#endif
template <int DV, int CPB, bool FACT>
__global__ void __launch_bounds__(256 * CPB) FGNN_GNN_OCC gnn_mfma_kernel(GraphDev g, WeightsDev w, GnnArgs a)
{
    extern __shared__ float lds[];
    const int cwl = threadIdx.x >> 8, tid = threadIdx.x & 255;
    const int slot = blockIdx.x * CPB + cwl;
    const int slot_b = slot / a.nsplit, part = slot - slot_b * a.nsplit;
    const bool active = slot_b < a.B;
    const int b = (active && a.index) ? a.index[slot_b] : slot_b;
    float* tabs = lds;
    float* gcn = lds + T_COUNT * 64 + cwl * a.lds_per_cw;
    const int n = g.n;
    for (int i = threadIdx.x; i < T_COUNT * 64; i += 256 * CPB) tabs[i] = w.lane_tab[i];
    if (active) stage_check_features(g, a.logit_hx, a.logit_hz, a.synd_x, a.synd_z, b, gcn, tid, 256);
    __syncthreads();
    if (!active) return;

    const int l = threadIdx.x & 63, wave = tid >> 6;
    const int j = l & 15, q = l >> 4;
#define TAB(e) tabs[toff + (e) * 64]
#define FRESH_TAB() int toff = l; asm volatile("" : "+v"(toff))
    const float* in = a.llr + (size_t)b * 3 * n;
    float* out = a.out + (size_t)b * 3 * n;
    const f4 zero = {0.0f, 0.0f, 0.0f, 0.0f};
    const int ntiles = (n + 15) >> 4;
    for (int tile = wave + 4 * part; tile < ntiles; tile += 4 * a.nsplit) {
        const int vraw = tile * 16 + j;
        const bool valid = vraw < n;
        const int v = valid ? vraw : n - 1;
        const float feat_own = (q == 0) ? 0.0f : in[(q - 1) * n + v];
        const float xyz0 = (q < 3) ? in[q * n + v] : 0.0f;
        float mean[2][5];
#pragma unroll
        for (int s2 = 0; s2 < 2; ++s2) {
            const int ebase = (s2 ? g.E_x : 0) + v * DV;
            const float* gside = gcn + (s2 ? g.m_x : 0);
            float esum[5];
            if constexpr (FACT) {
                float Pb[10], Hs[10];
                {
                    FRESH_TAB();
                    f4 d[3];
#pragma unroll
                    for (int t = 0; t < 3; ++t) d[t] = mfma4(TAB(T_W1 + s2 * 3 + t), feat_own, zero);
#pragma unroll
                    for (int s = 0; s < 10; ++s) Pb[s] = d[s >> 2][s & 3] + TAB(T_B1 + s2 * 10 + s);
                }
#pragma unroll
                for (int k = 0; k < DV; ++k) {
                    FRESH_TAB();
                    const float gv = gside[g.vchk[ebase + k]];
#pragma unroll
                    for (int s = 0; s < 10; ++s) {
                        const float h = fg_tanh(FG_FMA(gv, TAB(T_W10 + s2 * 10 + s), Pb[s]));
                        Hs[s] = (k == 0) ? h : Hs[s] + h;
                    }
                }
                FRESH_TAB();
                f4 m0 = zero, m1 = zero;
#pragma unroll
                for (int s = 0; s < 10; ++s) {
                    m0 = mfma4(TAB(T_W2 + (s2 * 2 + 0) * 10 + s), Hs[s], m0);
                    m1 = mfma4(TAB(T_W2 + (s2 * 2 + 1) * 10 + s), Hs[s], m1);
                }
                const float ms[5] = {m0[0], m0[1], m0[2], m0[3], m1[0]};
#pragma unroll
                for (int i = 0; i < 5; ++i)
                    mean[s2][i] = (DV == 3 ? fg_div3(ms[i]) : ms[i] / (float)DV) + TAB(T_B2 + s2 * 5 + i);
                continue;
            }
#pragma unroll
            for (int k = 0; k < DV; ++k) {
                FRESH_TAB();
                const float gv = gside[g.vchk[ebase + k]];
                const float F = (q == 0) ? gv : feat_own;
                f4 d[3];
#pragma unroll
                for (int t = 0; t < 3; ++t) d[t] = mfma4(TAB(T_W1 + s2 * 3 + t), F, zero);
                float H[10];
#pragma unroll
                for (int s = 0; s < 10; ++s) H[s] = fg_tanh(d[s >> 2][s & 3] + TAB(T_B1 + s2 * 10 + s));
                f4 m0 = zero, m1 = zero;
#pragma unroll
                for (int s = 0; s < 10; ++s) {
                    m0 = mfma4(TAB(T_W2 + (s2 * 2 + 0) * 10 + s), H[s], m0);
                    m1 = mfma4(TAB(T_W2 + (s2 * 2 + 1) * 10 + s), H[s], m1);
                }
                float msg[5] = {m0[0] + TAB(T_B2 + s2 * 5 + 0), m0[1] + TAB(T_B2 + s2 * 5 + 1), m0[2] + TAB(T_B2 + s2 * 5 + 2),
                                m0[3] + TAB(T_B2 + s2 * 5 + 3), m1[0] + TAB(T_B2 + s2 * 5 + 4)};
#pragma unroll
                for (int i = 0; i < 5; ++i) esum[i] = (k == 0) ? msg[i] : esum[i] + msg[i];
            }
#pragma unroll
            for (int i = 0; i < 5; ++i) mean[s2][i] = DV == 3 ? fg_div3(esum[i]) : esum[i] / (float)DV;
        }
        FRESH_TAB();
        f4 e[3] = {zero, zero, zero};
#pragma unroll
        for (int s = 0; s < 11; ++s) {
            const float Bs = (s < 5) ? mean[0][s] : (s < 10) ? mean[1][s - 5] : xyz0;
#pragma unroll
            for (int t = 0; t < 3; ++t) e[t] = mfma4(TAB(T_WE + t * 11 + s), Bs, e[t]);
        }
        f4 o = zero;
#pragma unroll
        for (int s = 0; s < 10; ++s) o = mfma4(TAB(T_WO + s), fg_tanh(e[s >> 2][s & 3] + TAB(T_BE + s)), o);
        if (valid && q == 0) {
            out[v] = o[0] + TAB(T_BO + 0);
            out[n + v] = o[1] + TAB(T_BO + 1);
            out[2 * n + v] = o[2] + TAB(T_BO + 2);
        }
    }
#undef TAB
#undef FRESH_TAB
}

template <bool FACT>
__global__ void __launch_bounds__(1024) gnn_kernel(GraphDev g, WeightsDev w, GnnArgs a)
{
    extern __shared__ float lds[];
    const int cwl = threadIdx.x / a.tpc;
    const int lane = threadIdx.x - cwl * a.tpc;
    const int slot_b = blockIdx.x * a.cpb + cwl;
    const bool active = slot_b < a.B;
    const int b = (active && a.index) ? a.index[slot_b] : slot_b;
    float* gcn = lds + (size_t)cwl * a.lds_per_cw;
    const int n = g.n;
    if (active) stage_check_features(g, a.logit_hx, a.logit_hz, a.synd_x, a.synd_z, b, gcn, lane, a.tpc);
    __syncthreads();
    if (!active) return;
    const float* in = a.llr + (size_t)b * 3 * n;
    float* out = a.out + (size_t)b * 3 * n;
    for (int v = lane; v < n; v += a.tpc) {
        const float X = in[v], Y = in[n + v], Z = in[2 * n + v];
        float feat[2 * MSG];
        {
            float mean[MSG];
            if constexpr (FACT) side_mean_factored(g, g.vptr_x, v, gcn, X, Y, Z, as_scalar(w.w1t[0]), as_scalar(w.b1[0]), as_scalar(w.w2[0]), as_scalar(w.b2[0]), mean);
            else side_mean(g, g.vptr_x, v, gcn, X, Y, Z, as_scalar(w.w1t[0]), as_scalar(w.b1[0]), as_scalar(w.w2[0]), as_scalar(w.b2[0]), mean);
#pragma unroll
            for (int i = 0; i < MSG; ++i) feat[i] = mean[i];
            if constexpr (FACT) side_mean_factored(g, g.vptr_z, v, gcn + g.m_x, X, Y, Z, as_scalar(w.w1t[1]), as_scalar(w.b1[1]), as_scalar(w.w2[1]), as_scalar(w.b2[1]), mean);
            else side_mean(g, g.vptr_z, v, gcn + g.m_x, X, Y, Z, as_scalar(w.w1t[1]), as_scalar(w.b1[1]), as_scalar(w.w2[1]), as_scalar(w.b2[1]), mean);
#pragma unroll
            for (int i = 0; i < MSG; ++i) feat[MSG + i] = mean[i];
        }
        float o0 = 0.0f, o1 = 0.0f, o2 = 0.0f;
#pragma unroll 2
        for (int j = 0; j < HID; ++j) {
            scalar_fp r = as_scalar(w.wet) + j * 44;
            float acc = 0.0f;
#pragma unroll
            for (int k = 0; k < 2 * MSG; ++k) acc = FG_FMA(feat[k], r[k], acc);
            acc = FG_FMA(X, r[40], acc);
            acc = FG_FMA(Y, r[41], acc);
            acc = FG_FMA(Z, r[42], acc);
            const float h = fg_tanh(acc + as_scalar(w.be)[j]);
            scalar_fp ro = as_scalar(w.wout) + j * 4;
            o0 = FG_FMA(h, ro[0], o0);
            o1 = FG_FMA(h, ro[1], o1);
            o2 = FG_FMA(h, ro[2], o2);
        }
        out[v] = o0 + w.bout[0];
        out[n + v] = o1 + w.bout[1];
        out[2 * n + v] = o2 + w.bout[2];
    }
}


#ifndef FGNN_GNNS_EMB_U
#define FGNN_GNNS_EMB_U 4
#endif
constexpr int EMB_U = FGNN_GNNS_EMB_U;
constexpr int SROW = 32, EROW = 48, EQUAD = ((43 + 1 + 3) * EMB_U + 31) / 32 * 32;
static_assert(HID % EMB_U == 0 && EMB_U % 2 == 0, "the embed MLP walks its hidden units in blocks");
#ifndef FGNN_GNNS_UNROLL
#define FGNN_GNNS_UNROLL 1
#endif
#ifndef FGNN_GNNS_WAVES
#define FGNN_GNNS_WAVES 7
#endif
#ifndef FGNN_GNNS_EMBPK_FACT
#define FGNN_GNNS_EMBPK_FACT 1
#endif
#ifndef FGNN_GNNS_EMBPK_LIT
#define FGNN_GNNS_EMBPK_LIT 1
#endif
#ifndef FGNN_GNNS_EMB_KG
#define FGNN_GNNS_EMB_KG 4
#endif
#ifndef FGNN_GNNS_LIT_UNROLL
#define FGNN_GNNS_LIT_UNROLL 1
#endif
#ifndef FGNN_GNNS_LIT_WAVES
#define FGNN_GNNS_LIT_WAVES 5
#endif

#define FGNN_GNNS_OCC __attribute__((amdgpu_waves_per_eu(FGNN_GNNS_WAVES, FGNN_GNNS_WAVES)))

struct MsgRow {
    float w1[4], b1, w2[MSG];
};
__device__ __forceinline__ MsgRow load_msg_row(scalar_fp r)
{
    MsgRow m;
#pragma unroll
    for (int k = 0; k < 4; ++k) m.w1[k] = r[k];
    m.b1 = r[4];
#pragma unroll
    for (int i = 0; i < MSG; ++i) m.w2[i] = r[8 + i];
    return m;
}

template <int DV>
__device__ __forceinline__ float msg_hidden(const MsgRow& r, const float (&gv)[DV], float X, float Y, float Z)
{
    float p = 0.0f;
    p = FG_FMA(X, r.w1[1], p);
    p = FG_FMA(Y, r.w1[2], p);
    p = FG_FMA(Z, r.w1[3], p);
    const float pb = p + r.b1;
    float hs = fg_tanh(FG_FMA(gv[0], r.w1[0], pb));
#pragma unroll
    for (int k = 1; k < DV; ++k) hs = hs + fg_tanh(FG_FMA(gv[k], r.w1[0], pb));
    return hs;
}
template <int DV>
__device__ __forceinline__ void msg_unit(const MsgRow& r, const float (&gv)[DV], float X, float Y, float Z, float (&acc)[MSG])
{
    const float hs = msg_hidden<DV>(r, gv, X, Y, Z);
#pragma unroll
    for (int i = 0; i < MSG; ++i) acc[i] = FG_FMA(hs, r.w2[i], acc[i]);
}

template <int DV>
__device__ __forceinline__ void side_stream(scalar_fp rows, scalar_fp b2, const float (&gv)[DV],
                                            float X, float Y, float Z, float* __restrict__ feat)
{
    float acc[MSG];
#pragma unroll
    for (int i = 0; i < MSG; ++i) acc[i] = 0.0f;
#pragma unroll FGNN_GNNS_UNROLL
    for (int j = 0; j < HID; ++j) msg_unit<DV>(load_msg_row(rows + j * SROW), gv, X, Y, Z, acc);
#pragma unroll
    for (int i = 0; i < MSG; ++i) feat[i] = (DV == 3 ? fg_div3(acc[i]) : acc[i] / (float)DV) + b2[i];
}

template <int DV>
__device__ __forceinline__ void side_stream_literal(scalar_fp rows, scalar_fp b2, const float (&gv)[DV], float X, float Y, float Z,
                                                    float* __restrict__ feat)
{
#pragma unroll 1
    for (int e = 0; e < DV; ++e) {
        float ge = gv[0];
#pragma unroll
        for (int k = 1; k < DV; ++k) ge = e == k ? gv[k] : ge;
        f2 m[MSG / 2];
#pragma unroll
        for (int i = 0; i < MSG / 2; ++i) m[i] = bc2(0.0f);
#pragma unroll FGNN_GNNS_LIT_UNROLL
        for (int j = 0; j < HID; ++j) {
            scalar_fp r = rows + j * SROW;
            scalar_f2p w2 = (scalar_f2p)(r + 8);
            float a = 0.0f;
            a = FG_FMA(ge, r[0], a);
            a = FG_FMA(X, r[1], a);
            a = FG_FMA(Y, r[2], a);
            a = FG_FMA(Z, r[3], a);
            const f2 h = bc_lo(fg_tanh(a + r[4]));
#pragma unroll
            for (int i = 0; i < MSG / 2; ++i) m[i] = pk_fma(h, w2[i], m[i]);
        }
#pragma unroll
        for (int i = 0; i < MSG / 2; ++i) {
            const float m0 = m[i].x + b2[2 * i], m1 = m[i].y + b2[2 * i + 1];
            feat[2 * i] = (e == 0) ? m0 : feat[2 * i] + m0;
            feat[2 * i + 1] = (e == 0) ? m1 : feat[2 * i + 1] + m1;
        }
    }
#pragma unroll
    for (int i = 0; i < MSG; ++i) feat[i] = DV == 3 ? fg_div3(feat[i]) : feat[i] / (float)DV;
}

struct EmbRow {
    float we[2 * MSG + 3], be, wo[3];
};
__device__ __forceinline__ EmbRow load_emb_row(scalar_fp r)
{
    EmbRow m;
#pragma unroll
    for (int k = 0; k < 2 * MSG + 3; ++k) m.we[k] = r[k];
    m.be = r[43];
#pragma unroll
    for (int i = 0; i < 3; ++i) m.wo[i] = r[44 + i];
    return m;
}
__device__ __forceinline__ void emb_unit(const EmbRow& r, const float* __restrict__ feat, float X, float Y, float Z, float (&o)[3])
{
    float acc = 0.0f;
#pragma unroll
    for (int k = 0; k < 2 * MSG; ++k) acc = FG_FMA(feat[k], r.we[k], acc);
    acc = FG_FMA(X, r.we[40], acc);
    acc = FG_FMA(Y, r.we[41], acc);
    acc = FG_FMA(Z, r.we[42], acc);
    const float h = fg_tanh(acc + r.be);
#pragma unroll
    for (int i = 0; i < 3; ++i) o[i] = FG_FMA(h, r.wo[i], o[i]);
}

__device__ __forceinline__ void emb_quad(const float* quad, f2 (&fx)[2 * MSG / 2 + 2], float (&o)[3])
{
#pragma unroll
    for (int q = 0; q < 2 * MSG / 2 + 2; ++q) asm volatile("" : "+v"(fx[q]));
    f2 acc[EMB_U / 2];
#pragma unroll
    for (int jp = 0; jp < EMB_U / 2; ++jp) acc[jp] = bc2(0.0f);
    dense_pk<2 * MSG + 3, EMB_U / 2, FGNN_GNNS_EMB_KG, false>(fx, quad, EMB_U, acc);
    scalar_fp r = as_scalar(quad);
    float h[EMB_U];
#pragma unroll
    for (int jp = 0; jp < EMB_U / 2; ++jp) {
        h[2 * jp] = fg_tanh(acc[jp].x + r[43 * EMB_U + 2 * jp]);
        h[2 * jp + 1] = fg_tanh(acc[jp].y + r[43 * EMB_U + 2 * jp + 1]);
    }
#pragma unroll
    for (int u = 0; u < EMB_U; ++u)
#pragma unroll
        for (int i = 0; i < 3; ++i) o[i] = FG_FMA(h[u], r[44 * EMB_U + 3 * u + i], o[i]);
}

template <int DV, bool LITERAL = false, bool EMBPK = false>
__global__ void __launch_bounds__(1024) __attribute__((amdgpu_waves_per_eu(LITERAL ? FGNN_GNNS_LIT_WAVES : FGNN_GNNS_WAVES, LITERAL ? FGNN_GNNS_LIT_WAVES : FGNN_GNNS_WAVES)))
gnn_stream_kernel(GraphDev g, WeightsDev w, GnnArgs a)
{
    extern __shared__ float lds[];
    const int slot_b = blockIdx.x;
    const int b = a.index ? a.index[slot_b] : slot_b;
    float* gcn = lds;
    const int n = g.n;
    stage_check_features(g, a.logit_hx, a.logit_hz, a.synd_x, a.synd_z, b, gcn, threadIdx.x, blockDim.x);
    __syncthreads();
    const float* in = a.llr + (size_t)b * 3 * n;
    float* out = a.out + (size_t)b * 3 * n;
    scalar_fp mrx = as_scalar((const float*)__builtin_assume_aligned(w.msg_rows[0], 128));
    scalar_fp mrz = as_scalar((const float*)__builtin_assume_aligned(w.msg_rows[1], 128));
    scalar_fp er = as_scalar((const float*)__builtin_assume_aligned(w.emb_rows, 64));
    scalar_fp b2x = as_scalar(w.b2[0]), b2z = as_scalar(w.b2[1]), bo = as_scalar(w.bout);
    for (int v = threadIdx.x; v < n; v += blockDim.x) {
        const float X = in[v], Y = in[n + v], Z = in[2 * n + v];
        f2 fx[MSG + 2];
        float* feat = reinterpret_cast<float*>(fx);
        float gv[DV];
#pragma unroll
        for (int k = 0; k < DV; ++k) gv[k] = gcn[g.vchk[v * DV + k]];
#pragma unroll
        for (int k = 0; k < DV; ++k) asm volatile("" : "+v"(gv[k]));
        if constexpr (LITERAL) side_stream_literal<DV>(mrx, b2x, gv, X, Y, Z, feat);
        else side_stream<DV>(mrx, b2x, gv, X, Y, Z, feat);
#pragma unroll
        for (int k = 0; k < DV; ++k) gv[k] = gcn[g.m_x + g.vchk[g.E_x + v * DV + k]];
#pragma unroll
        for (int k = 0; k < DV; ++k) asm volatile("" : "+v"(gv[k]));
        if constexpr (LITERAL) side_stream_literal<DV>(mrz, b2z, gv, X, Y, Z, feat + MSG);
        else side_stream<DV>(mrz, b2z, gv, X, Y, Z, feat + MSG);
        float o[3] = {0.0f, 0.0f, 0.0f};
        if constexpr (EMBPK) {
            fx[MSG] = f2{X, Y};
            fx[MSG + 1] = f2{Z, 0.0f};
#pragma unroll 1
            for (int q = 0; q < HID / EMB_U; ++q) emb_quad(w.emb_quads + q * EQUAD, fx, o);
        } else {
#pragma unroll FGNN_GNNS_UNROLL
            for (int j = 0; j < HID; ++j) emb_unit(load_emb_row(er + j * EROW), feat, X, Y, Z, o);
        }
        out[v] = o[0] + bo[0];
        out[n + v] = o[1] + bo[1];
        out[2 * n + v] = o[2] + bo[2];
    }
}

__global__ void __launch_bounds__(1024) gnn_general_kernel(GraphDev g, GnnGeneralDev w, GnnArgs a)
{
    extern __shared__ float lds[];
    const int cwl = threadIdx.x / a.tpc;
    const int lane = threadIdx.x - cwl * a.tpc;
    const int slot_b = blockIdx.x * a.cpb + cwl;
    const bool active = slot_b < a.B;
    const int b = (active && a.index) ? a.index[slot_b] : slot_b;
    float* gcn = lds + (size_t)cwl * a.lds_per_cw;
    const int n = g.n;
    if (active) stage_check_features(g, a.logit_hx, a.logit_hz, a.synd_x, a.synd_z, b, gcn, lane, a.tpc);
    __syncthreads();
    if (!active) return;
    const float* in = a.llr + (size_t)b * 3 * n;
    float* out = a.out + (size_t)b * 3 * n;
    const int D = w.D, L = w.L;
    for (int v = lane; v < n; v += a.tpc) {
        const float X = in[v], Y = in[n + v], Z = in[2 * n + v];
        float bufA[FGNN_GEN_MAX_W], bufB[FGNN_GEN_MAX_W], z[2 * FGNN_GEN_MAX_D + 3];
        for (int s = 0; s < 2; ++s) {
            const int* vptr = s == 0 ? g.vptr_x : g.vptr_z;
            const float* gc = s == 0 ? gcn : gcn + g.m_x;
            const int e0 = vptr[v], e1 = vptr[v + 1];
            float* acc = z + s * D;
            for (int i = 0; i < D; ++i) acc[i] = 0.0f;
            for (int e = e0; e < e1; ++e) {
                float* cur = bufA;
                float* nxt = bufB;
                cur[0] = gc[g.vchk[e]];
                cur[1] = X;
                cur[2] = Y;
                cur[3] = Z;
                for (int l = 0; l < L; ++l) {
                    gen_dense(w, s * L + l, cur, nxt);
                    float* t = cur;
                    cur = nxt;
                    nxt = t;
                }
                gg_reduce(acc, cur, D, e == e0, w.reduce_op);
            }
            if (w.reduce_op == FGNN_REDUCE_MEAN && e1 > e0) {
                const float fd = (float)(e1 - e0);
                for (int i = 0; i < D; ++i) acc[i] = acc[i] / fd;
            }
        }
        z[2 * D] = X;
        z[2 * D + 1] = Y;
        z[2 * D + 2] = Z;
        const float* cur = z;
        float* nxt = bufA;
        for (int l = 0; l < L - 1; ++l) {
            gen_dense(w, 2 * L + l, cur, nxt);
            cur = nxt;
            nxt = (nxt == bufA) ? bufB : bufA;
        }
        float o[3];
        gen_dense(w, 3 * L - 1, cur, o);
        out[v] = o[0];
        out[n + v] = o[1];
        out[2 * n + v] = o[2];
    }
}

}

extern "C" int fgnn_weights_create(const float* const host_arrays[12], int device, fgnn_weights** out)
{
    if (!host_arrays || !out) return fgnn_fail(FGNN_ERR_ARG, "NULL argument");
    for (int i = 0; i < 12; ++i)
        if (!host_arrays[i]) return fgnn_fail(FGNN_ERR_ARG, "weight array is NULL");
    FGNN_DEVICE_GUARD(device);
    std::vector<float> h;
    size_t off[12];
    auto push = [&](size_t count) {
        size_t o = h.size();
        h.resize(o + ((count + 3) & ~size_t(3)), 0.0f);
        return o;
    };
    for (int s = 0; s < 2; ++s) {
        const float* W1 = host_arrays[2 + 4 * s];
        const float* B1 = host_arrays[3 + 4 * s];
        const float* W2 = host_arrays[4 + 4 * s];
        const float* B2 = host_arrays[5 + 4 * s];
        off[4 * s + 0] = push(HID * 4);
        for (int j = 0; j < HID; ++j)
            for (int k = 0; k < 4; ++k) h[off[4 * s + 0] + j * 4 + k] = W1[k * HID + j];
        off[4 * s + 1] = push(HID);
        std::memcpy(&h[off[4 * s + 1]], B1, HID * sizeof(float));
        off[4 * s + 2] = push(HID * MSG);
        std::memcpy(&h[off[4 * s + 2]], W2, HID * MSG * sizeof(float));
        off[4 * s + 3] = push(MSG);
        std::memcpy(&h[off[4 * s + 3]], B2, MSG * sizeof(float));
    }
    off[8] = push(HID * 44);
    for (int j = 0; j < HID; ++j)
        for (int k = 0; k < 43; ++k) h[off[8] + j * 44 + k] = host_arrays[10][k * HID + j];
    off[9] = push(HID);
    std::memcpy(&h[off[9]], host_arrays[11], HID * sizeof(float));
    off[10] = push(HID * 4);
    for (int j = 0; j < HID; ++j)
        for (int i = 0; i < 3; ++i) h[off[10] + j * 4 + i] = host_arrays[0][j * 3 + i];
    off[11] = push(4);
    std::memcpy(&h[off[11]], host_arrays[1], 3 * sizeof(float));

    size_t off_mr[2];
    for (int s = 0; s < 2; ++s) {
        while (h.size() % 32) h.push_back(0.0f);
        off_mr[s] = push((size_t)HID * SROW);
        const float* W1 = host_arrays[2 + 4 * s];
        const float* B1 = host_arrays[3 + 4 * s];
        const float* W2 = host_arrays[4 + 4 * s];
        for (int j = 0; j < HID; ++j) {
            float* r = &h[off_mr[s] + (size_t)j * SROW];
            for (int k = 0; k < 4; ++k) r[k] = W1[k * HID + j];
            r[4] = B1[j];
            for (int i = 0; i < MSG; ++i) r[8 + i] = W2[j * MSG + i];
        }
    }
    while (h.size() % 32) h.push_back(0.0f);
    const size_t off_er = push((size_t)HID * EROW);
    for (int j = 0; j < HID; ++j) {
        float* r = &h[off_er + (size_t)j * EROW];
        for (int k = 0; k < 43; ++k) r[k] = host_arrays[10][k * HID + j];
        r[43] = host_arrays[11][j];
        for (int i = 0; i < 3; ++i) r[44 + i] = host_arrays[0][j * 3 + i];
    }
    while (h.size() % 32) h.push_back(0.0f);
    const size_t off_eq = push((size_t)(HID / EMB_U) * EQUAD);
    for (int q = 0; q < HID / EMB_U; ++q) {
        float* r = &h[off_eq + (size_t)q * EQUAD];
        for (int k = 0; k < 43; ++k)
            for (int u = 0; u < EMB_U; ++u) r[EMB_U * k + u] = host_arrays[10][k * HID + EMB_U * q + u];
        for (int u = 0; u < EMB_U; ++u) {
            r[43 * EMB_U + u] = host_arrays[11][EMB_U * q + u];
            for (int i = 0; i < 3; ++i) r[44 * EMB_U + 3 * u + i] = host_arrays[0][(EMB_U * q + u) * 3 + i];
        }
    }
    const size_t off_tab = push((size_t)T_COUNT * 64);
    {
        auto entry = [&](int e) { return &h[off_tab + (size_t)e * 64]; };
        for (int s2 = 0; s2 < 2; ++s2) {
            const float* W1 = host_arrays[2 + 4 * s2];
            for (int t = 0; t < 3; ++t) mfma_fill_w1(entry(T_W1 + s2 * 3 + t), W1, 4, HID, t, 0);
            for (int s = 0; s < 10; ++s) mfma_fill_b1(entry(T_B1 + s2 * 10 + s), host_arrays[3 + 4 * s2], s);
            for (int u = 0; u < 2; ++u)
                for (int s = 0; s < 10; ++s) mfma_fill_w2(entry(T_W2 + (s2 * 2 + u) * 10 + s), host_arrays[4 + 4 * s2], MSG, u, s);
            for (int i = 0; i < 5; ++i) mfma_fill_b2(entry(T_B2 + s2 * 5 + i), host_arrays[5 + 4 * s2], i);
            for (int s = 0; s < 10; ++s) mfma_fill_b1(entry(T_W10 + s2 * 10 + s), W1, s);
        }
        for (int t = 0; t < 3; ++t)
            for (int s = 0; s < 11; ++s) mfma_fill_w1(entry(T_WE + t * 11 + s), host_arrays[10], 43, HID, t, s);
        for (int s = 0; s < 10; ++s) {
            mfma_fill_b1(entry(T_BE + s), host_arrays[11], s);
            mfma_fill_wout(entry(T_WO + s), host_arrays[0], s);
        }
        for (int r = 0; r < 3; ++r) std::fill_n(entry(T_BO + r), 64, host_arrays[1][r]);
    }

    fgnn_weights* w = new fgnn_weights();
    w->device = device;
    if (int rc = fgnn_weights_upload(w, h, "weights upload: ")) return rc;
    const float* base = static_cast<const float*>(w->blob);
    for (int s = 0; s < 2; ++s) {
        w->d.w1t[s] = base + off[4 * s + 0];
        w->d.b1[s] = base + off[4 * s + 1];
        w->d.w2[s] = base + off[4 * s + 2];
        w->d.b2[s] = base + off[4 * s + 3];
    }
    w->d.wet = base + off[8];
    w->d.be = base + off[9];
    w->d.wout = base + off[10];
    w->d.bout = base + off[11];
    w->d.lane_tab = base + off_tab;
    w->d.msg_rows[0] = base + off_mr[0];
    w->d.msg_rows[1] = base + off_mr[1];
    w->d.emb_rows = base + off_er;
    w->d.emb_quads = base + off_eq;
    *out = w;
    return FGNN_OK;
}

extern "C" int fgnn_weights_create_general(const fgnn_gnn_config* cfg, const float* const* host_arrays, int num_arrays,
                                           int device, fgnn_weights** out)
{
    if (!cfg || !host_arrays || !out) return fgnn_fail(FGNN_ERR_ARG, "NULL argument");
    const int D = cfg->num_msg_dims, H = cfg->num_hidden_units, L = cfg->num_mlp_layers, bias = cfg->use_bias ? 1 : 0;
    if (D < 1 || D > FGNN_GEN_MAX_D || L < 1 || L > 4 || (L > 1 && (H < 1 || H > FGNN_GEN_MAX_W)))
        return fgnn_fail(FGNN_ERR_ARG, "general feedback GNN: need 1 <= num_msg_dims <= 32, 1 <= num_hidden_units <= 96, "
                                       "1 <= num_mlp_layers <= 4");
    if (cfg->reduce_op < 0 || cfg->reduce_op > 3) return fgnn_fail(FGNN_ERR_ARG, "unknown reduce operation");
    if (cfg->activation < 0 || cfg->activation > 3) return fgnn_fail(FGNN_ERR_ARG, "unsupported activation");
    if (num_arrays != 3 * L * (1 + bias)) return fgnn_fail(FGNN_ERR_ARG, "wrong number of weight arrays for this configuration");
    for (int i = 0; i < num_arrays; ++i)
        if (!host_arrays[i]) return fgnn_fail(FGNN_ERR_ARG, "weight array is NULL");
    FGNN_DEVICE_GUARD(device);
    fgnn_weights* w = new fgnn_weights();
    w->device = device;
    w->general = true;
    std::memset(&w->d, 0, sizeof(w->d));
    GnnGeneralDev& G = w->gen;
    std::memset(&G, 0, sizeof(G));
    G.D = D; G.H = H; G.L = L; G.reduce_op = cfg->reduce_op; G.act = cfg->activation; G.bias = bias; G.nl = 3 * L;
    const int emb_out = L > 1 ? H : 2 * D + 3;
    for (int s = 0; s < 2; ++s)
        for (int l = 0; l < L; ++l) {
            const int li = s * L + l;
            G.K[li] = l == 0 ? 4 : H;
            G.J[li] = l == L - 1 ? D : H;
            G.act_l[li] = l == L - 1 ? FGNN_ACT_LINEAR : cfg->activation;
        }
    for (int l = 0; l < L - 1; ++l) {
        const int li = 2 * L + l;
        G.K[li] = l == 0 ? 2 * D + 3 : H;
        G.J[li] = H;
        G.act_l[li] = cfg->activation;
    }
    G.K[3 * L - 1] = emb_out;
    G.J[3 * L - 1] = 3;
    G.act_l[3 * L - 1] = FGNN_ACT_LINEAR;
    std::vector<float> h;
    std::vector<size_t> offW(G.nl), offB(G.nl);
    auto file_index = [&](int li) { return li == 3 * L - 1 ? 0 : li + 1; };
    for (int li = 0; li < G.nl; ++li) {
        const int f = file_index(li) * (1 + bias);
        const size_t cnt = (size_t)G.K[li] * G.J[li];
        offW[li] = h.size();
        h.insert(h.end(), host_arrays[f], host_arrays[f] + cnt);
        h.resize((h.size() + 3) & ~size_t(3), 0.0f);
        offB[li] = h.size();
        if (bias) {
            h.insert(h.end(), host_arrays[f + 1], host_arrays[f + 1] + G.J[li]);
            h.resize((h.size() + 3) & ~size_t(3), 0.0f);
        }
    }
    if (int rc = fgnn_weights_upload(w, h, "weights upload: ")) return rc;
    const float* base = static_cast<const float*>(w->blob);
    for (int li = 0; li < G.nl; ++li) {
        G.W[li] = base + offW[li];
        G.b[li] = bias ? base + offB[li] : nullptr;
    }
    *out = w;
    return FGNN_OK;
}

extern "C" void fgnn_weights_destroy(fgnn_weights* w)
{
    fgnn_weights_free(w);
}

int fgnn_feedback_gnn_impl(const fgnn_graph* g, const fgnn_weights* w, const float* llr, const float* logit_hx,
                           const float* logit_hz, const uint8_t* synd_x, const uint8_t* synd_z, int B, float* out,
                           const int* index, void* stream)
{
    if (!g || !w) return fgnn_fail(FGNN_ERR_ARG, "graph or weights is NULL");
    if (B < 0) return fgnn_fail(FGNN_ERR_ARG, "B must be >= 0");
    if (w->device != g->device) return fgnn_fail(FGNN_ERR_ARG, "weights and graph live on different devices");
    if (B == 0) return FGNN_OK;
    if (!llr || !logit_hx || !logit_hz || !synd_x || !synd_z || !out) return fgnn_fail(FGNN_ERR_ARG, "buffer is NULL");
    FGNN_DEVICE_GUARD(g->device);
    LaunchGeom L = fgnn_geom(g, B);
    GnnArgs a{B, L.tpc, L.cpb, (g->d.m + 3) & ~3, llr, logit_hx, logit_hz, synd_x, synd_z, out, index, 1};
    fgnn_prof_scope prof(g, static_cast<hipStream_t>(stream));
    auto launch = [&](auto kern, unsigned blocks, int threads, size_t lds, const auto& wdev) {
        const int rc = fgnn_launch(kern, dim3(blocks), dim3(threads), lds, static_cast<hipStream_t>(stream), g->d, wdev, a);
        if (rc == FGNN_OK) prof.done(FGNN_PROF_TAG_GNN, B);
        return rc;
    };
    const size_t lds_packed = (size_t)a.lds_per_cw * sizeof(float) * (size_t)L.cpb;
    if (w->general) return launch(gnn_general_kernel, L.blocks, L.threads, lds_packed, w->gen);
    const bool stream_pays = g->gnn_stream == 2 || g->d.dvx != 3 || B >= 4096;
    if (g->d.dvx == g->d.dvz && g->d.dvx >= 3 && g->d.dvx <= 5 && !g->force_generic && g->gnn_stream && stream_pays) {
        const int n = g->d.n;
        int best_tpc = 0, best_cost = 1 << 30;
        for (int k = 1; k <= 32; ++k) {
            const int per = (n + k - 1) / k, tpc = (per + 63) & ~63;
            if (tpc > 1024 || tpc < 128) continue;
            const int cost = (tpc / 64) * k;
            const bool better_tie = B <= 2048 ? tpc > best_tpc : (tpc <= 256 ? (best_tpc > 256 || tpc > best_tpc) : tpc < best_tpc);
            if (cost < best_cost || (cost == best_cost && better_tie)) { best_cost = cost; best_tpc = tpc; }
        }
        if (!best_tpc) best_tpc = 128;
#ifdef FGNN_GNNS_TPC
        best_tpc = FGNN_GNNS_TPC;
#endif
        const size_t lds_s = (size_t)a.lds_per_cw * sizeof(float);
        constexpr bool PF = FGNN_GNNS_EMBPK_FACT != 0, PL = FGNN_GNNS_EMBPK_LIT != 0;
        auto skern = g->gnn_factored ? (g->d.dvx == 3 ? gnn_stream_kernel<3, false, PF> : g->d.dvx == 4 ? gnn_stream_kernel<4, false, PF> : gnn_stream_kernel<5, false, PF>)
                                     : (g->d.dvx == 3 ? gnn_stream_kernel<3, true, PL> : g->d.dvx == 4 ? gnn_stream_kernel<4, true, PL> : gnn_stream_kernel<5, true, PL>);
        return launch(skern, (unsigned)B, best_tpc, lds_s, w->d);
    }
    if (g->d.dvx == 3 && g->d.dvz == 3 && !g->force_generic) {
        constexpr int GNN_CPB = FGNN_GNN_CPB;
        const int ntiles = (g->d.n + 15) / 16;
        a.nsplit = 1;
        while (a.nsplit < 16 && (long long)B * a.nsplit * 2 <= 2048 && a.nsplit * 4 < ntiles) a.nsplit *= 2;
        const size_t lds_mfma = (size_t)(T_COUNT * 64 + GNN_CPB * a.lds_per_cw) * sizeof(float);
        auto kern = g->gnn_factored ? gnn_mfma_kernel<3, GNN_CPB, true> : gnn_mfma_kernel<3, GNN_CPB, false>;
        return launch(kern, (unsigned)(((long long)B * a.nsplit + GNN_CPB - 1) / GNN_CPB), 256 * GNN_CPB, lds_mfma, w->d);
    }
    return launch(g->gnn_factored ? gnn_kernel<true> : gnn_kernel<false>, L.blocks, L.threads, lds_packed, w->d);
}

extern "C" int fgnn_feedback_gnn(const fgnn_graph* g, const fgnn_weights* w, const float* llr, const float* logit_hx,
                                 const float* logit_hz, const uint8_t* synd_x, const uint8_t* synd_z, int B, float* out,
                                 void* stream)
{
    return fgnn_feedback_gnn_impl(g, w, llr, logit_hx, logit_hz, synd_x, synd_z, B, out, nullptr, stream);
}
```

### feedback_gnn_amd/csrc/fgnn_graph.hip

```cpp
#include <algorithm>
#include <cstring>
#include <numeric>

#include "fgnn_internal.h"

static thread_local std::string g_err;
void fgnn_set_error(const std::string& s) { g_err = s; }
int fgnn_fail(int code, const std::string& s)
{
    g_err = s;
    return code;
}
extern "C" const char* fgnn_last_error(void) { return g_err.c_str(); }
extern "C" int fgnn_version(void) { return 2; }

namespace {

template <typename T>
int upload(fgnn_graph* g, const std::vector<T>& h, const T** dst)
{
    void* p = nullptr;
    size_t bytes = std::max<size_t>(h.size(), 1) * sizeof(T);
    FGNN_HIP_CHECK(hipMalloc(&p, bytes));
    g->allocs.push_back(p);
    if (!h.empty()) FGNN_HIP_CHECK(hipMemcpy(p, h.data(), h.size() * sizeof(T), hipMemcpyHostToDevice));
    *dst = static_cast<const T*>(p);
    return FGNN_OK;
}

void coo_to_csr(int rows, int nnz, const int32_t* r, const int32_t* c, std::vector<int>& ptr, std::vector<int>& col)
{
    std::vector<int> order(nnz);
    std::iota(order.begin(), order.end(), 0);
    std::sort(order.begin(), order.end(), [&](int a, int b) { return r[a] != r[b] ? r[a] < r[b] : c[a] < c[b]; });
    ptr.assign(rows + 1, 0);
    col.resize(nnz);
    for (int i = 0; i < nnz; ++i) {
        ptr[r[order[i]] + 1]++;
        col[i] = c[order[i]];
    }
    for (int i = 0; i < rows; ++i) ptr[i + 1] += ptr[i];
}

int uniform_degree(const std::vector<int>& ptr)
{
    if (ptr.size() < 2) return 0;
    int d = ptr[1] - ptr[0];
    for (size_t i = 1; i + 1 < ptr.size(); ++i)
        if (ptr[i + 1] - ptr[i] != d) return 0;
    return d;
}

void default_launch(fgnn_graph* g)
{
    const int nodes = std::max(g->d.n, g->d.m);
    int tpc = nodes;
    int cpb = 1;
    if (nodes >= 256) {
        tpc = 256;
    } else if (tpc >= 64) {
        tpc = (tpc + 63) / 64 * 64;
    } else {
        int p2 = 1;
        while (p2 < tpc) p2 <<= 1;
        tpc = p2;
        cpb = 256 / tpc;
    }
    g->tpc = tpc;
    g->cpb = cpb;
}

}

LaunchGeom fgnn_geom(const fgnn_graph* g, int B)
{
    LaunchGeom L;
    L.tpc = g->tpc;
    L.cpb = g->cpb;
    if (!g->user_launch && g->cpb == 1 && B <= 256) {
        const int nodes = std::max(g->d.n, g->d.m);
        L.tpc = std::min(1024, std::max(g->tpc, (nodes + 63) / 64 * 64));
    }
    L.threads = L.tpc * L.cpb;
    L.blocks = (B + g->cpb - 1) / g->cpb;
    return L;
}

extern "C" int fgnn_graph_create(int n, int m_x, int m_z, int nnz_x, const int32_t* chk_x, const int32_t* var_x,
                                 int nnz_z, const int32_t* chk_z, const int32_t* var_z, int device, fgnn_graph** out)
{
    if (!out) return fgnn_fail(FGNN_ERR_ARG, "out is NULL");
    if (n <= 0 || m_x <= 0 || m_z <= 0 || nnz_x <= 0 || nnz_z <= 0)
        return fgnn_fail(FGNN_ERR_ARG, "n, m_x, m_z and the edge counts must be positive");
    const int32_t* chk[2] = {chk_x, chk_z};
    const int32_t* var[2] = {var_x, var_z};
    const int nnz[2] = {nnz_x, nnz_z};
    const int m[2] = {m_x, m_z};
    for (int s = 0; s < 2; ++s)
        for (int i = 0; i < nnz[s]; ++i)
            if (chk[s][i] < 0 || chk[s][i] >= m[s] || var[s][i] < 0 || var[s][i] >= n)
                return fgnn_fail(FGNN_ERR_ARG, "edge index out of range");
    FGNN_DEVICE_GUARD(device);
    fgnn_graph* g = new fgnn_graph();
    std::memset(&g->d, 0, sizeof(g->d));
    std::memset(g->row_alloc, 0, sizeof(g->row_alloc));
    g->device = device;
    g->user_launch = false;
    GraphDev& d = g->d;
    d.n = n;
    d.m_x = m_x;
    d.m_z = m_z;
    d.m = m_x + m_z;
    d.E_x = nnz_x;
    d.E_z = nnz_z;
    d.E = nnz_x + nnz_z;

    std::vector<int> vptr[2], vchk_side[2];
    for (int s = 0; s < 2; ++s) {
        coo_to_csr(n, nnz[s], var[s], chk[s], vptr[s], vchk_side[s]);
        for (int v = 0; v < n; ++v)
            for (int e = vptr[s][v]; e + 1 < vptr[s][v + 1]; ++e)
                if (vchk_side[s][e] == vchk_side[s][e + 1]) {
                    delete g;
                    return fgnn_fail(FGNN_ERR_ARG, "duplicate edge");
                }
        g->h_chk[s] = std::vector<int32_t>(vchk_side[s].begin(), vchk_side[s].end());
        g->h_var[s].resize(nnz[s]);
        for (int v = 0; v < n; ++v)
            for (int e = vptr[s][v]; e < vptr[s][v + 1]; ++e) g->h_var[s][e] = v;
    }
    std::vector<int> vptr_x = vptr[0], vptr_z = vptr[1], vchk(d.E);
    for (auto& x : vptr_z) x += d.E_x;
    std::copy(vchk_side[0].begin(), vchk_side[0].end(), vchk.begin());
    std::copy(vchk_side[1].begin(), vchk_side[1].end(), vchk.begin() + d.E_x);
    std::vector<int> cptr(d.m + 1, 0), cslot(d.E), cvn(d.E);
    {
        std::vector<int> deg(d.m, 0);
        for (int s = 0; s < 2; ++s)
            for (int i = 0; i < nnz[s]; ++i) deg[(s ? m_x : 0) + chk[s][i]]++;
        for (int c = 0; c < d.m; ++c) cptr[c + 1] = cptr[c] + deg[c];
        std::vector<int> fill(d.m, 0);
        for (int s = 0; s < 2; ++s)
            for (int v = 0; v < n; ++v)
                for (int e = vptr[s][v]; e < vptr[s][v + 1]; ++e) {
                    int c = (s ? m_x : 0) + vchk_side[s][e];
                    int pos = cptr[c] + fill[c]++;
                    cslot[pos] = e + (s ? d.E_x : 0);
                    cvn[pos] = v;
                }
    }
    d.dvx = uniform_degree(vptr[0]);
    d.dvz = uniform_degree(vptr[1]);
    d.dc = uniform_degree(cptr);
    d.max_vdeg = 0;
    for (int v = 0; v < n; ++v)
        d.max_vdeg = std::max(d.max_vdeg, (vptr[0][v + 1] - vptr[0][v]) + (vptr[1][v + 1] - vptr[1][v]));
    d.max_cdeg = d.max_cdeg_x = 0;
    for (int c = 0; c < d.m; ++c) {
        d.max_cdeg = std::max(d.max_cdeg, cptr[c + 1] - cptr[c]);
        if (c < m_x) d.max_cdeg_x = std::max(d.max_cdeg_x, cptr[c + 1] - cptr[c]);
    }
    int rc;
    if (d.dvx > 0 && d.dvz > 0 && d.dc > 0 && d.dc <= 8 && (long long)d.E * 4 < 65536) {
        std::vector<uint16_t> pk((size_t)d.m * 8, 0);
        for (int c = 0; c < d.m; ++c)
            for (int j = 0; j < d.dc; ++j) pk[(size_t)c * 8 + j] = (uint16_t)(4 * cslot[cptr[c] + j]);
        if ((rc = upload(g, pk, &d.cslot16))) {
            fgnn_graph_destroy(g);
            return rc;
        }
    }
    if ((rc = upload(g, vptr_x, &d.vptr_x)) || (rc = upload(g, vptr_z, &d.vptr_z)) || (rc = upload(g, vchk, &d.vchk)) ||
        (rc = upload(g, cptr, &d.cptr)) || (rc = upload(g, cslot, &d.cslot)) || (rc = upload(g, cvn, &d.cvn))) {
        fgnn_graph_destroy(g);
        return rc;
    }
    default_launch(g);
    *out = g;
    return FGNN_OK;
}

extern "C" void fgnn_graph_destroy(fgnn_graph* g)
{
    if (!g) return;
    fgnn_device_guard _dg(g->device);
    for (hipEvent_t e : g->prof_ev) (void)hipEventDestroy(e);
    for (void* p : g->basis_dev)
        if (p) (void)hipFree(p);
    for (void* p : g->allocs) (void)hipFree(p);
    for (auto& r : g->row_alloc)
        for (void* p : r)
            if (p) (void)hipFree(p);
    delete g;
}

extern "C" int fgnn_graph_set_rows(fgnn_graph* g, int which, int rows, int nnz, const int32_t* row, const int32_t* col)
{
    if (!g || which < 0 || which > 5 || rows < 0 || nnz < 0) return fgnn_fail(FGNN_ERR_ARG, "bad row-set arguments");
    for (int i = 0; i < nnz; ++i)
        if (row[i] < 0 || row[i] >= rows || col[i] < 0 || col[i] >= g->d.n)
            return fgnn_fail(FGNN_ERR_ARG, "row-set index out of range");
    FGNN_DEVICE_GUARD(g->device);
    std::vector<int> ptr, c;
    coo_to_csr(rows, nnz, row, col, ptr, c);
    for (void*& p : g->row_alloc[which])
        if (p) {
            (void)hipFree(p);
            p = nullptr;
        }
    void *dp = nullptr, *dc = nullptr;
    FGNN_HIP_CHECK(hipMalloc(&dp, ptr.size() * sizeof(int)));
    g->row_alloc[which][0] = dp;
    FGNN_HIP_CHECK(hipMalloc(&dc, std::max<size_t>(c.size(), 1) * sizeof(int)));
    g->row_alloc[which][1] = dc;
    FGNN_HIP_CHECK(hipMemcpy(dp, ptr.data(), ptr.size() * sizeof(int), hipMemcpyHostToDevice));
    if (!c.empty()) FGNN_HIP_CHECK(hipMemcpy(dc, c.data(), c.size() * sizeof(int), hipMemcpyHostToDevice));
    g->d.rows[which] = rows;
    g->d.rptr[which] = static_cast<const int*>(dp);
    g->d.rcol[which] = static_cast<const int*>(dc);
    if (which < 2) {
        const int n = g->d.n;
        std::vector<int> tp(n + 1, 0), tr(std::max<size_t>(c.size(), 1), 0);
        for (int x : c) tp[x + 1]++;
        for (int v = 0; v < n; ++v) tp[v + 1] += tp[v];
        std::vector<int> fill(tp.begin(), tp.end() - 1);
        for (int r = 0; r < rows; ++r)
            for (int p = ptr[r]; p < ptr[r + 1]; ++p) tr[fill[c[p]]++] = r;
        void *tpd = nullptr, *trd = nullptr;
        FGNN_HIP_CHECK(hipMalloc(&tpd, tp.size() * sizeof(int)));
        g->row_alloc[which][2] = tpd;
        FGNN_HIP_CHECK(hipMalloc(&trd, tr.size() * sizeof(int)));
        g->row_alloc[which][3] = trd;
        FGNN_HIP_CHECK(hipMemcpy(tpd, tp.data(), tp.size() * sizeof(int), hipMemcpyHostToDevice));
        FGNN_HIP_CHECK(hipMemcpy(trd, tr.data(), tr.size() * sizeof(int), hipMemcpyHostToDevice));
        g->d.tptr[which] = static_cast<const int*>(tpd);
        g->d.trow[which] = static_cast<const int*>(trd);
    }
    return FGNN_OK;
}

extern "C" int fgnn_graph_set_launch(fgnn_graph* g, int threads_per_codeword, int codewords_per_block)
{
    if (!g) return fgnn_fail(FGNN_ERR_ARG, "graph is NULL");
    if (threads_per_codeword <= 0 && codewords_per_block <= 0) {
        default_launch(g);
        g->user_launch = false;
        return FGNN_OK;
    }
    int tpc = threads_per_codeword > 0 ? threads_per_codeword : g->tpc;
    int cpb = codewords_per_block > 0 ? codewords_per_block : 1;
    if (tpc * cpb > 1024 || (tpc * cpb) % 64 != 0)
        return fgnn_fail(FGNN_ERR_ARG, "threads_per_codeword*codewords_per_block must be a multiple of 64 and <= 1024");
    g->tpc = tpc;
    g->cpb = cpb;
    g->user_launch = true;
    return FGNN_OK;
}

extern "C" int fgnn_graph_set_option(fgnn_graph* g, int option, int value)
{
    if (!g) return fgnn_fail(FGNN_ERR_ARG, "graph is NULL");
    switch (option) {
    case FGNN_OPT_SATURATION_SHORTCUT: g->shortcut = value != 0; return FGNN_OK;
    case FGNN_OPT_FIXED_POINT_EXIT: g->early_exit = value != 0; return FGNN_OK;
    case FGNN_OPT_HW_TRANSCENDENTALS: g->hw_transcendentals = value != 0; return FGNN_OK;
    case FGNN_OPT_GNN_FACTORED: g->gnn_factored = value != 0; return FGNN_OK;
    case FGNN_OPT_BP4_SHARED_LSE: g->bp4_shared_lse = value != 0; return FGNN_OK;
    case FGNN_OPT_GNN_STREAM:
        if (value < 0 || value > 2) return fgnn_fail(FGNN_ERR_ARG, "FGNN_OPT_GNN_STREAM takes 0, 1 or 2");
        g->gnn_stream = value;
        return FGNN_OK;
    default: return fgnn_fail(FGNN_ERR_ARG, "unknown option");
    }
}

extern "C" int fgnn_graph_force_generic(fgnn_graph* g, int on)
{
    if (!g) return fgnn_fail(FGNN_ERR_ARG, "graph is NULL");
    g->force_generic = on != 0;
    return FGNN_OK;
}

extern "C" int fgnn_graph_info(const fgnn_graph* g, int32_t info[16])
{
    if (!g || !info) return fgnn_fail(FGNN_ERR_ARG, "NULL argument");
    std::memset(info, 0, 16 * sizeof(int32_t));
    info[0] = g->d.n;
    info[1] = g->d.m_x;
    info[2] = g->d.m_z;
    info[3] = g->d.E_x;
    info[4] = g->d.E_z;
    info[5] = g->tpc;
    info[6] = g->cpb;
    info[7] = (int)((size_t)g->cpb * (size_t)(g->d.E + 3 * g->d.n) * sizeof(float));
    info[8] = (g->d.dvx > 0 && g->d.dvz > 0 && g->d.dc > 0) ? 1 : 0;
    info[9] = g->device;
    info[10] = g->d.dvx;
    info[11] = g->d.dvz;
    info[12] = g->d.dc;
    return FGNN_OK;
}

extern "C" int fgnn_graph_edges(const fgnn_graph* g, int side, int32_t* chk, int32_t* var)
{
    if (!g || side < 0 || side > 1 || !chk || !var) return fgnn_fail(FGNN_ERR_ARG, "bad arguments");
    std::copy(g->h_chk[side].begin(), g->h_chk[side].end(), chk);
    std::copy(g->h_var[side].begin(), g->h_var[side].end(), var);
    return FGNN_OK;
}

extern "C" int fgnn_profile_enable(fgnn_graph* g, int max_launches)
{
    if (!g || max_launches < 0) return fgnn_fail(FGNN_ERR_ARG, "bad profile arguments");
    FGNN_DEVICE_GUARD(g->device);
    for (hipEvent_t e : g->prof_ev) (void)hipEventDestroy(e);
    g->prof_ev.clear();
    g->prof_n = 0;
    g->prof_on = max_launches > 0;
    g->prof_iters.assign(max_launches, 0);
    g->prof_batch.assign(max_launches, 0);
    for (int i = 0; i < 2 * max_launches; ++i) {
        hipEvent_t e;
        FGNN_HIP_CHECK(hipEventCreate(&e));
        g->prof_ev.push_back(e);
    }
    return FGNN_OK;
}

extern "C" int fgnn_profile_read(fgnn_graph* g, float* ms, int32_t* iters, int32_t* batch, int cap, int32_t* count)
{
    if (!g || !ms || !iters || !batch || !count) return fgnn_fail(FGNN_ERR_ARG, "NULL argument");
    FGNN_DEVICE_GUARD(g->device);
    int n = g->prof_n < cap ? g->prof_n : cap;
    if (g->prof_n > 0) FGNN_HIP_CHECK(hipEventSynchronize(g->prof_ev[2 * g->prof_n - 1]));
    for (int i = 0; i < n; ++i) {
        FGNN_HIP_CHECK(hipEventElapsedTime(&ms[i], g->prof_ev[2 * i], g->prof_ev[2 * i + 1]));
        iters[i] = g->prof_iters[i];
        batch[i] = g->prof_batch[i];
    }
    *count = n;
    g->prof_n = 0;
    return FGNN_OK;
}
```

### feedback_gnn_amd/csrc/fgnn_internal.h

```cpp
#pragma once
#include <hip/hip_runtime.h>
#include <stdint.h>
#include <string>
#include <vector>

#include "../../include/fgnn.h"

struct GraphDev {
    int n, m_x, m_z, m, E_x, E_z, E;
    const int* vptr_x;
    const int* vptr_z;
    const int* vchk;
    const int* cptr;
    const int* cslot;
    const int* cvn;
    const uint16_t* cslot16;
    int rows[6];
    const int* rptr[6];
    const int* rcol[6];
    const int* tptr[2];
    const int* trow[2];
    int dvx, dvz, dc;
    int max_vdeg;
    int max_cdeg, max_cdeg_x;
};

struct fgnn_graph {
    GraphDev d;
    int device;
    int tpc, cpb;
    bool user_launch;
    bool shortcut = true;
    bool early_exit = true;
    bool hw_transcendentals = false;
    bool bp4_shared_lse = false;
    int gnn_stream = 1;
    bool gnn_factored = false;
    bool force_generic = false;
    std::vector<void*> allocs;
    std::vector<int32_t> h_chk[2], h_var[2];
    void* row_alloc[6][4];
    void* basis_dev[2] = {nullptr, nullptr};
    int basis_rank[2] = {0, 0};
    mutable bool prof_on = false;
    mutable int prof_n = 0;
    mutable std::vector<hipEvent_t> prof_ev;
    mutable std::vector<int> prof_iters, prof_batch;
};

#if defined(__HIPCC__)
typedef const float __attribute__((address_space(4)))* scalar_fp;
__device__ __forceinline__ scalar_fp as_scalar(const float* p) { return (scalar_fp)(unsigned long long)p; }
#endif

struct WeightsDev {
    const float* w1t[2];
    const float* b1[2];
    const float* w2[2];
    const float* b2[2];
    const float* wet;
    const float* be;
    const float* wout;
    const float* bout;
    const float* lane_tab;
    const float* msg_rows[2];
    const float* emb_rows;
    const float* emb_quads;
};

constexpr int FGNN_GEN_MAX_LAYERS = 12;
constexpr int FGNN_GEN_MAX_D = 32, FGNN_GEN_MAX_W = 96;
struct GnnGeneralDev {
    int D, H, L, reduce_op, act, bias, nl;
    int K[FGNN_GEN_MAX_LAYERS], J[FGNN_GEN_MAX_LAYERS], act_l[FGNN_GEN_MAX_LAYERS];
    const float* W[FGNN_GEN_MAX_LAYERS];
    const float* b[FGNN_GEN_MAX_LAYERS];
};

struct fgnn_weights {
    WeightsDev d;
    int device;
    void* blob;
    bool general = false;
    GnnGeneralDev gen;
};

struct fgnn_gnnbp4_train_view {
    int device, D, H, L, reduce_op, act, bias, use_attributes;
    const float* W[7][4];
    const float* b[7][4];
    int K[7][4], J[7][4];
    const float* winv;
    const float* binv;
};
bool fgnn_gnnbp4_weights_train_view(const fgnn_gnnbp4_weights* w, fgnn_gnnbp4_train_view* out);

void fgnn_set_error(const std::string& s);
int fgnn_fail(int code, const std::string& s);
#define FGNN_HIP_CHECK(expr)                                                                          \
    do {                                                                                              \
        hipError_t _e = (expr);                                                                       \
        if (_e != hipSuccess)                                                                         \
            return fgnn_fail(FGNN_ERR_HIP, std::string(#expr) + ": " + hipGetErrorString(_e));        \
    } while (0)

struct fgnn_device_guard {
    int prev = -1;
    hipError_t err = hipSuccess;
    explicit fgnn_device_guard(int device)
    {
        err = hipGetDevice(&prev);
        if (err == hipSuccess && prev != device) err = hipSetDevice(device);
        else prev = -1;
    }
    ~fgnn_device_guard()
    {
        if (prev >= 0) (void)hipSetDevice(prev);
    }
    fgnn_device_guard(const fgnn_device_guard&) = delete;
    fgnn_device_guard& operator=(const fgnn_device_guard&) = delete;
};
#define FGNN_DEVICE_GUARD(device)                                                                     \
    fgnn_device_guard _dev_guard(device);                                                             \
    if (_dev_guard.err != hipSuccess)                                                                 \
        return fgnn_fail(FGNN_ERR_HIP, std::string("hipSetDevice: ") + hipGetErrorString(_dev_guard.err))

template <typename W>
int fgnn_weights_upload(W* w, const std::vector<float>& h, const char* what)
{
    w->blob = nullptr;
    hipError_t e = hipMalloc(&w->blob, h.size() * sizeof(float));
    if (e == hipSuccess) e = hipMemcpy(w->blob, h.data(), h.size() * sizeof(float), hipMemcpyHostToDevice);
    if (e != hipSuccess) {
        if (w->blob) (void)hipFree(w->blob);
        delete w;
        return fgnn_fail(FGNN_ERR_HIP, std::string(what) + hipGetErrorString(e));
    }
    return FGNN_OK;
}

template <typename W>
void fgnn_weights_free(W* w)
{
    if (!w) return;
    fgnn_device_guard _dg(w->device);
    if (w->blob) (void)hipFree(w->blob);
    delete w;
}

constexpr int FGNN_PROF_TAG_GNN = -1;
constexpr int FGNN_PROF_TAG_GNNBP4 = -2;
struct fgnn_prof_scope {
    const fgnn_graph* g;
    hipStream_t st;
    bool on;
    fgnn_prof_scope(const fgnn_graph* g_, hipStream_t st_) : g(g_), st(st_)
    {
        on = g->prof_on && (size_t)(2 * g->prof_n + 1) < g->prof_ev.size();
        if (on && hipEventRecord(g->prof_ev[2 * g->prof_n], st) != hipSuccess) on = false;
    }
    void done(int tag, int B)
    {
        if (!on) return;
        if (hipEventRecord(g->prof_ev[2 * g->prof_n + 1], st) != hipSuccess) return;
        g->prof_iters[g->prof_n] = tag;
        g->prof_batch[g->prof_n] = B;
        g->prof_n++;
    }
};

constexpr size_t FGNN_LDS_BUDGET = 160 * 1024 - 256;

template <typename... Params, typename... Args>
int fgnn_launch(void (*kern)(Params...), dim3 grid, dim3 block, size_t lds, hipStream_t st, Args... args)
{
    if (lds > 48 * 1024)
        FGNN_HIP_CHECK(hipFuncSetAttribute(reinterpret_cast<const void*>(kern), hipFuncAttributeMaxDynamicSharedMemorySize, (int)lds));
    hipLaunchKernelGGL(kern, grid, block, lds, st, args...);
    FGNN_HIP_CHECK(hipGetLastError());
    return FGNN_OK;
}

struct LaunchGeom {
    int tpc, cpb, threads, blocks;
};
LaunchGeom fgnn_geom(const fgnn_graph* g, int B);

int fgnn_bp4_decode_impl(const fgnn_graph* g, int cn_type, int num_iter, float normalization_factor, const float* llr_ch,
                         float llr_const, const uint8_t* synd_x, const uint8_t* synd_z, int B, const float* msg_init_x,
                         const float* msg_init_z, float* llr_out, uint8_t* x_hat, uint8_t* z_hat, float* x_logit,
                         float* z_logit, float* msg_out_x, float* msg_out_z, const int* index, uint8_t* flagged, void* stream);
int fgnn_feedback_gnn_impl(const fgnn_graph* g, const fgnn_weights* w, const float* llr, const float* logit_hx,
                           const float* logit_hz, const uint8_t* synd_x, const uint8_t* synd_z, int B, float* out,
                           const int* index, void* stream);
int fgnn_flag_update_impl(const fgnn_graph* g, const uint8_t* x_hat, const uint8_t* z_hat, const uint8_t* synd_x,
                          const uint8_t* synd_z, int B, uint8_t* errors, const int* index, void* stream);
int fgnn_merge_impl(const uint8_t* errors, const uint8_t* x_upd, const uint8_t* z_upd, int B, int n, uint8_t* x_hat, uint8_t* z_hat,
                    const int* index, void* stream);
```

### include/fgnn.h

```cpp
#ifndef FGNN_H
#define FGNN_H

#include <stddef.h>
#include <stdint.h>

#ifdef __cplusplus
extern "C" {
#endif

typedef struct fgnn_graph fgnn_graph;
typedef struct fgnn_weights fgnn_weights;
typedef struct fgnn_gnnbp4_weights fgnn_gnnbp4_weights;

enum { FGNN_CN_BOXPLUS = 0, FGNN_CN_BOXPLUS_PHI = 1, FGNN_CN_MINSUM = 2 };
enum { FGNN_ROWS_X_LOGIT = 0, FGNN_ROWS_Z_LOGIT = 1, FGNN_ROWS_HX_PERP = 2, FGNN_ROWS_HZ_PERP = 3, FGNN_ROWS_LX = 4, FGNN_ROWS_LZ = 5 };

enum {
    FGNN_OK = 0,
    FGNN_ERR_ARG = -1,
    FGNN_ERR_HIP = -2,
    FGNN_ERR_STATE = -3,
    FGNN_ERR_NOMEM = -4
};

const char* fgnn_last_error(void);
int fgnn_version(void);

int fgnn_graph_create(int n, int m_x, int m_z, int nnz_x, const int32_t* chk_x, const int32_t* var_x, int nnz_z,
                      const int32_t* chk_z, const int32_t* var_z, int device, fgnn_graph** out);
void fgnn_graph_destroy(fgnn_graph* g);

int fgnn_graph_set_rows(fgnn_graph* g, int which, int rows, int nnz, const int32_t* row, const int32_t* col);

int fgnn_graph_set_launch(fgnn_graph* g, int threads_per_codeword, int codewords_per_block);
enum { FGNN_OPT_SATURATION_SHORTCUT = 1, FGNN_OPT_FIXED_POINT_EXIT = 2, FGNN_OPT_HW_TRANSCENDENTALS = 3, FGNN_OPT_GNN_FACTORED = 4,
       FGNN_OPT_BP4_SHARED_LSE = 5, FGNN_OPT_GNN_STREAM = 6 };
int fgnn_graph_set_option(fgnn_graph* g, int option, int value);
int fgnn_graph_force_generic(fgnn_graph* g, int on);
int fgnn_graph_info(const fgnn_graph* g, int32_t info[16]);
int fgnn_graph_edges(const fgnn_graph* g, int side, int32_t* chk, int32_t* var);

int fgnn_profile_enable(fgnn_graph* g, int max_launches);
int fgnn_profile_read(fgnn_graph* g, float* ms, int32_t* iters, int32_t* batch, int cap, int32_t* count);

int fgnn_bp4_decode(const fgnn_graph* g, int cn_type, int num_iter, float normalization_factor, const float* llr_ch,
                    float llr_const, const uint8_t* synd_x, const uint8_t* synd_z, int B, const float* msg_init_x,
                    const float* msg_init_z, float* llr_out, uint8_t* x_hat, uint8_t* z_hat, float* x_logit,
                    float* z_logit, float* msg_out_x, float* msg_out_z, void* stream);

int fgnn_bp4_decode_trace(const fgnn_graph* g, int cn_type, int num_iter, float normalization_factor, const float* llr_ch,
                          float llr_const, const uint8_t* synd_x, const uint8_t* synd_z, int B, const float* msg_init_x,
                          const float* msg_init_z, float* llr_out, uint8_t* x_hat, uint8_t* z_hat, float* x_logit_trace,
                          float* z_logit_trace, float* tape_x, float* tape_z, void* stream);

int fgnn_weights_create(const float* const host_arrays[12], int device, fgnn_weights** out);
void fgnn_weights_destroy(fgnn_weights* w);

typedef struct {
    int num_msg_dims, num_hidden_units, num_mlp_layers;
    int reduce_op;
    int activation;
    int use_bias;
} fgnn_gnn_config;
enum { FGNN_REDUCE_SUM = 0, FGNN_REDUCE_MEAN = 1, FGNN_REDUCE_MAX = 2, FGNN_REDUCE_MIN = 3 };
enum { FGNN_ACT_LINEAR = 0, FGNN_ACT_TANH = 1, FGNN_ACT_RELU = 2, FGNN_ACT_SIGMOID = 3 };
int fgnn_weights_create_general(const fgnn_gnn_config* cfg, const float* const* host_arrays, int num_arrays, int device,
                                fgnn_weights** out);

int fgnn_feedback_gnn(const fgnn_graph* g, const fgnn_weights* w, const float* llr, const float* logit_hx,
                      const float* logit_hz, const uint8_t* synd_x, const uint8_t* synd_z, int B, float* out,
                      void* stream);

int fgnn_pauli_noise(uint64_t seed, float p, uint64_t first_sample, int B, int n, uint8_t* noise_x, uint8_t* noise_z,
                     void* stream);
int fgnn_pauli_noise_xyz(uint64_t seed, float px, float py, float pz, uint64_t first_sample, int B, int n, uint8_t* noise_x,
                         uint8_t* noise_z, void* stream);
int fgnn_pauli_noise_dev(uint64_t seed, float p, const uint64_t* first_sample_dev, uint64_t offset, int B, int n, uint8_t* noise_x,
                         uint8_t* noise_z, void* stream);
int fgnn_pauli_noise_wt(uint64_t seed, int wt, uint64_t first_sample, int B, int n, uint8_t* noise_x, uint8_t* noise_z, void* stream);
int fgnn_syndrome(const fgnn_graph* g, const uint8_t* noise_x, const uint8_t* noise_z, int B, uint8_t* synd_x,
                  uint8_t* synd_z, void* stream);
int fgnn_flag_update(const fgnn_graph* g, const uint8_t* x_hat, const uint8_t* z_hat, const uint8_t* synd_x,
                     const uint8_t* synd_z, int B, uint8_t* errors, void* stream);
int fgnn_merge(const uint8_t* errors, const uint8_t* x_upd, const uint8_t* z_upd, int B, int n, uint8_t* x_hat,
               uint8_t* z_hat, void* stream);
int fgnn_residual(const fgnn_graph* g, const uint8_t* noise_x, const uint8_t* noise_z, const uint8_t* x_hat,
                  const uint8_t* z_hat, int B, uint8_t* s_hat, uint8_t* ls_hat, uint8_t* flags, void* stream);
int fgnn_residual_rows(const fgnn_graph* g, int rows_x, int rows_z, const uint8_t* noise_x, const uint8_t* noise_z,
                       const uint8_t* x_hat, const uint8_t* z_hat, int B, uint8_t* s_hat, uint8_t* ls_hat, uint8_t* flags, void* stream);
int fgnn_pack_decisions(const uint8_t* x_hat, const uint8_t* z_hat, int B, int n, uint8_t* packed, void* stream);
int fgnn_unpack_decisions(const uint8_t* packed, int B, int n, uint8_t* x_hat, uint8_t* z_hat, void* stream);
int fgnn_count_flags(const uint8_t* flags, int B, uint64_t* counts, void* stream);
int fgnn_count_flags_batches(const uint8_t* flags, int num_batches, int batch, uint64_t* counts, uint64_t* ring, uint32_t* scratch,
                             void* stream);

size_t fgnn_sandwich_workspace_bytes(const fgnn_graph* g, int B);
int fgnn_sandwich_decode(const fgnn_graph* g, int num_layers, const int32_t* iters, const float* factors,
                         const int32_t* cn_types, const fgnn_weights* const* weights, float llr_const,
                         const uint8_t* synd_x, const uint8_t* synd_z, int B, int compact, uint8_t* x_hat,
                         uint8_t* z_hat, float* llr_final, uint8_t* rounds, void* workspace, size_t ws_bytes,
                         void* stream);

int fgnn_bp2_decode(const fgnn_graph* g, int cn_type, int num_iter, float normalization_factor, const float* llr_ch,
                    float llr_const, const uint8_t* synd, int B, float* soft_out, uint8_t* hard_out, void* stream);
int fgnn_relay_decode(const fgnn_graph* g, float normalization_factor, int pre_iter, int num_legs, int leg_iter, int stop_nconv,
                      const float* gamma, const float* llr_ch, float llr_const, const uint8_t* synd, int B, uint8_t* hard_out,
                      int32_t* stats, void* stream);
int fgnn_relay4_decode(const fgnn_graph* g, int cn_type, float normalization_factor, int pre_iter, int num_legs, int leg_iter,
                       int stop_nconv, const float* gamma, const float* llr_ch, float llr_const, const uint8_t* synd_x,
                       const uint8_t* synd_z, int B, uint8_t* x_hat, uint8_t* z_hat, int32_t* stats, void* stream);
int fgnn_bsc_noise(uint64_t seed, float p, uint64_t first_sample, int B, int n, uint8_t* noise, void* stream);

int fgnn_graph_set_basis(fgnn_graph* g, int side, int rank, const int32_t* pivot_rows);
int fgnn_osd0(const fgnn_graph* g, int side, const float* marg, const float* llr_bin, const uint8_t* synd, int B,
              const int32_t* index, int nact, uint8_t* e_hat, void* stream);
enum { FGNN_OSD_0 = 0, FGNN_OSD_E = 1, FGNN_OSD_CS = 2 };
int fgnn_osd(const fgnn_graph* g, int side, int method, int order, const float* marg, const float* llr_bin, const uint8_t* synd, int B,
             const int32_t* index, int nact, uint8_t* e_hat, int32_t* chosen, void* stream);
int fgnn_osd_resident(const fgnn_graph* g, int side, int method, int* fits);
int fgnn_osd_workspace_bytes(const fgnn_graph* g, int side, int method, int order, int slots, size_t* bytes);
int fgnn_osd_ws(const fgnn_graph* g, int side, int method, int order, const float* marg, const float* llr_bin, const uint8_t* synd,
                int B, const int32_t* index, int nact, uint8_t* e_hat, int32_t* chosen, void* workspace, size_t workspace_bytes,
                void* stream);
int fgnn_compact(const uint8_t* mask, int bit, int B, int32_t* index, int32_t* count, void* stream);

int fgnn_gnnbp4_weights_create(const float* const host_arrays[30], int num_embed_dims, int num_hidden_units, int device,
                               fgnn_gnnbp4_weights** out);
void fgnn_gnnbp4_weights_destroy(fgnn_gnnbp4_weights* w);
size_t fgnn_gnnbp4_workspace_bytes(const fgnn_graph* g, int B);
typedef struct {
    int num_embed_dims, num_hidden_units, num_mlp_layers;
    int reduce_op;
    int activation;
    int use_bias, use_attributes, node_attribute_dims, msg_attribute_dims;
} fgnn_gnnbp4_config;
int fgnn_gnnbp4_weights_create_general(const fgnn_graph* g, const fgnn_gnnbp4_config* cfg, const float* const* host_arrays,
                                       int num_arrays, fgnn_gnnbp4_weights** out);
size_t fgnn_gnnbp4_weights_workspace_bytes(const fgnn_graph* g, const fgnn_gnnbp4_weights* w, int B);
int fgnn_gnnbp4_decode(const fgnn_graph* g, const fgnn_gnnbp4_weights* w, int num_iter, const uint8_t* synd_x,
                       const uint8_t* synd_z, int B, uint8_t* x_hat, uint8_t* z_hat, float* llr_out, float* x_logit_all,
                       float* z_logit_all, void* workspace, size_t ws_bytes, void* stream);

int fgnn_bp4_backward(const fgnn_graph* g, int num_iter, float normalization_factor, const float* llr_ch,
                      const uint8_t* synd_x, const uint8_t* synd_z, int B, const float* tape_x, const float* tape_z,
                      const float* grad_x_logit, const float* grad_z_logit, const uint8_t* has_grad, float* grad_llr_ch,
                      void* stream);

int fgnn_feedback_gnn_backward(const fgnn_graph* g, const fgnn_weights* w, const float* llr, const float* logit_hx,
                               const float* logit_hz, const uint8_t* synd_x, const uint8_t* synd_z, int B,
                               const float* grad_out, float* node_in, float* node_h2, float* node_d2,
                               float* const edge_feat[2], float* const edge_h1[2], float* const edge_d1[2],
                               float* const edge_dm[2], void* stream);
int fgnn_feedback_gnn_backward_general(const fgnn_graph* g, const fgnn_weights* w, const float* llr, const float* logit_hx,
                                       const float* logit_hz, const uint8_t* synd_x, const uint8_t* synd_z, int B,
                                       const float* grad_out, float* const* acts, float* const* deltas, int num_layers, void* stream);

int fgnn_gnnbp4_grad_count(const fgnn_graph* g, const fgnn_gnnbp4_weights* w, int* count);
int fgnn_gnnbp4_tape_bytes(const fgnn_graph* g, const fgnn_gnnbp4_weights* w, int num_iter, int B, size_t* bytes);
int fgnn_gnnbp4_backward_workspace_bytes(const fgnn_graph* g, const fgnn_gnnbp4_weights* w, int B, size_t* bytes);
int fgnn_gnnbp4_forward_tape(const fgnn_graph* g, const fgnn_gnnbp4_weights* w, int num_iter, const uint8_t* synd_x,
                             const uint8_t* synd_z, int B, float* x_logit_all, float* z_logit_all, float* tape, size_t tape_bytes,
                             void* stream);
int fgnn_gnnbp4_backward(const fgnn_graph* g, const fgnn_gnnbp4_weights* w, int num_iter, const uint8_t* synd_x,
                         const uint8_t* synd_z, int B, const float* tape, size_t tape_bytes, const float* grad_x_logit_all,
                         const float* grad_z_logit_all, float* grad_weights, int grad_count, void* workspace, size_t ws_bytes,
                         void* stream);

#ifdef __cplusplus
}
#endif
#endif
```

Before: 969,700.

## Widen check-slot rows to 32-bit LDS addresses and precompute phi for logit rows

Check-node slot tables are widened from packed 16-bit to 32-bit entries so the regular phi kernel can address LDS directly, offset by the static LDS size, which a runtime attribute check enforces. The end of the decode now keeps hard decisions in registers for the flag parity check. It precomputes phi of the final LLRs once per variable so each logit row becomes a sum plus one phi. A packed cvn16 table is added for the syndrome and parity kernels, the GNN edge loop gets scheduling hints, and a host-only row-checking API is added. The cost is extra graph memory and tighter coupling to the static LDS layout.

Measured after the change: 987,900, median of 6. +1.9%, better.

```diff
diff --git a/feedback_gnn_amd/_lib.py b/feedback_gnn_amd/_lib.py
--- a/feedback_gnn_amd/_lib.py
+++ b/feedback_gnn_amd/_lib.py
@@ -63,6 +63,8 @@
     "fgnn_graph_force_generic": (C.c_int, [C.c_void_p, C.c_int]),
     "fgnn_graph_info": (C.c_int, [C.c_void_p, C.c_void_p]),
     "fgnn_graph_edges": (C.c_int, [C.c_void_p, C.c_int, C.c_void_p, C.c_void_p]),
+    "fgnn_check_rows": (C.c_int, [C.c_int, C.c_int, C.c_int, C.c_int, C.c_void_p, C.c_void_p, C.c_int, C.c_void_p, C.c_void_p,
+                                  C.c_void_p, C.c_void_p, C.c_void_p]),
     "fgnn_profile_enable": (C.c_int, [C.c_void_p, C.c_int]),
     "fgnn_profile_read": (C.c_int, [C.c_void_p, C.c_void_p, C.c_void_p, C.c_void_p, C.c_int, C.c_void_p]),
     "fgnn_bp4_decode": (C.c_int, [C.c_void_p, C.c_int, C.c_int, C.c_float, C.c_void_p, C.c_float, C.c_void_p, C.c_void_p,
diff --git a/feedback_gnn_amd/csrc/fgnn_bp4.hip b/feedback_gnn_amd/csrc/fgnn_bp4.hip
--- a/feedback_gnn_amd/csrc/fgnn_bp4.hip
+++ b/feedback_gnn_amd/csrc/fgnn_bp4.hip
@@ -17,6 +17,8 @@
 #endif
 
 namespace {
+
+constexpr int BP4_STATIC_LDS = 64 * (int)sizeof(float);
 
 struct BpArgs {
     int B, num_iter, tpc, cpb, lds_per_cw, lch_off;
@@ -107,6 +109,23 @@
     return logit_row<Mx<HWT>>(llr, col, deg);
 }
 
+__device__ __forceinline__ float logit_row_ready(const float* llr, const float* phis, const int* __restrict__ col, int deg, float phi0,
+                                                 bool shortcut)
+{
+    unsigned neg = 0;
+    bool sat = true;
+    float T = 0.0f;
+    for (int j = 0; j < deg; ++j) {
+        const int c = col[j];
+        const float v = llr[c];
+        neg ^= (v < 0.0f);
+        sat = sat && (FG_ABS(v) >= FG_PHI_MAX);
+        T = T + phis[c];
+    }
+    if (shortcut && __all(sat)) return with_sign(phi0, neg);
+    return with_sign(Mx<false>::phi(T), neg);
+}
+
 template <int N, bool HWT = false>
 __device__ __forceinline__ void phi_n(const float (&x)[N], float (&out)[N])
 {
@@ -152,7 +171,14 @@
     }
 }
 
-template <int DC, bool HWT = false, bool F1 = false>
+typedef __attribute__((address_space(3))) float lds_float;
+template <int LDSB, typename IDX>
+__device__ __forceinline__ decltype(auto) cn_slot(float* msg, IDX byte_off)
+{
+    if constexpr (LDSB >= 0) return *(lds_float*)(uintptr_t)((unsigned)byte_off + (unsigned)LDSB);
+    else return slot_ref(msg, byte_off);
+}
+template <int DC, bool HWT = false, bool F1 = false, int LDSB = -1>
 __device__ __forceinline__ bool cn_phi_regular(float* msg, const int (&sl)[DC], uint32_t neg0, float factor, float phi0,
                                                bool shortcut)
 {
@@ -163,7 +189,7 @@
     bool sat = true;
 #pragma unroll
     for (int j = 0; j < DC; ++j) {
-        v[j] = slot_ref(msg, sl[j]);
+        v[j] = cn_slot<LDSB>(msg, sl[j]);
         neg ^= fg_f2u(v[j]);
         sat = sat && (FG_ABS(v[j]) >= FG_PHI_MAX);
     }
@@ -171,7 +197,7 @@
 #pragma unroll
         for (int j = 0; j < DC; ++j) {
             const float o = fg_u2f(fg_f2u(phi0) | ((neg ^ fg_f2u(v[j])) & 0x80000000u));
-            slot_ref(msg, sl[j]) = F1 ? o : o * factor;
+            cn_slot<LDSB>(msg, sl[j]) = F1 ? o : o * factor;
         }
         return true;
     }
@@ -196,7 +222,7 @@
 #pragma unroll
         for (int j = 0; j < H; ++j) {
             const float o = fg_u2f(fg_f2u(oa[j]) | ((neg ^ fg_f2u(v[g0 + j])) & 0x80000000u));
-            slot_ref(msg, sl[g0 + j]) = F1 ? o : o * factor;
+            cn_slot<LDSB>(msg, sl[g0 + j]) = F1 ? o : o * factor;
         }
     }
     return false;
@@ -269,6 +295,7 @@
     constexpr int NQA = LREG ? NQ : 1;
     static_assert(NT == 0 || (DVX > 0 && CN_TYPE == FGNN_CN_BOXPLUS_PHI && !LREG && !TRACE && !GMEM), "compile-time trips: the regular phi kernel");
     constexpr int CT = LREG ? NQ : NT;
+    constexpr bool READY = REGULAR && CT > 0 && CN_TYPE == FGNN_CN_BOXPLUS_PHI && !HWT;
     const int tpc = NT > 0 ? 256 : a.tpc;
     const bool opt_shortcut = OPT && a.shortcut != 0;
     const bool opt_exit = OPT && a.early_exit != 0;
@@ -364,7 +391,7 @@
         for (int c = lane_c; c < g.m && i < 32; c += tpc, ++i) synd_bits |= ((c < g.m_x ? sx[c] : sz[c - g.m_x]) & 1u) << i;
     }
     const bool synd_in_reg = (g.m + tpc - 1) / tpc <= 32;
-    unsigned row_off = 16u * (unsigned)lane_c;
+    unsigned row_off = 32u * (unsigned)lane_c;
     auto trace_step = [&](const int k) __attribute__((always_inline)) {
         float* tlx = msg + a.trace_off;
         float* tlz = tlx + n;
@@ -612,21 +639,24 @@
         if constexpr (REGULAR && CT > 0 && CN_TYPE == FGNN_CN_BOXPLUS_PHI) {
             auto cn_trips = [&](auto f1) __attribute__((always_inline)) {
                 constexpr bool F1 = decltype(f1)::value;
-                const char* rows = reinterpret_cast<const char*>(g.cslot16);
+                const char* rows = reinterpret_cast<const char*>(g.cslot32);
 #pragma unroll
                 for (int i = 0; i < CT; ++i) {
                     const bool in = (!LREG && i + 1 < CT) || lane_c + i * tpc < g.m;
                     if (in) {
-                        const char* base = rows + (size_t)i * (size_t)(16u * (unsigned)tpc);
+                        static_assert(DC > 4 && DC <= 8, "a cslot32 row is read as four dwords and two or four more");
+                        const char* base = rows + (size_t)i * (size_t)(32u * (unsigned)tpc);
                         asm volatile("" : "+v"(row_off));
                         if constexpr (NT > 0) asm volatile("" : "+s"(base));
-                        typedef unsigned Row __attribute__((ext_vector_type(4)));
-                        const Row pk = *(const __attribute__((address_space(1))) Row*)(base + row_off);
-                        const unsigned w[4] = {pk.x, pk.y, pk.z, pk.w};
+                        typedef unsigned Row4 __attribute__((ext_vector_type(4)));
+                        typedef unsigned Row2 __attribute__((ext_vector_type(2)));
+                        typedef std::conditional_t<(DC > 6), Row4, Row2> RowT;
+                        const Row4 pk = *(const __attribute__((address_space(1))) Row4*)(base + row_off);
+                        const RowT pt = *(const __attribute__((address_space(1))) RowT*)(base + row_off + 16);
                         int sl[DC];
 #pragma unroll
-                        for (int j = 0; j < DC; ++j) sl[j] = (int)((w[j >> 1] >> ((j & 1) * 16)) & 0xffffu);
-                        const bool fast = cn_phi_regular<DC, HWT, F1>(lds, sl, synd_bits << (31 - i), F1 ? 1.0f : a.factor, phi0, opt_shortcut);
+                        for (int j = 0; j < DC; ++j) sl[j] = (int)(j < 4 ? pk[j] : pt[j - 4]);
+                        const bool fast = cn_phi_regular<DC, HWT, F1, BP4_STATIC_LDS>(lds, sl, synd_bits << (31 - i), F1 ? 1.0f : a.factor, phi0, opt_shortcut);
                         cn_slow = !fast || cn_slow;
                     }
                 }
@@ -700,13 +730,22 @@
             if (Y < best) { best = Y; d = 3; }
             a.x_hat[(size_t)b * n + v] = (uint8_t)(d & 1);
             a.z_hat[(size_t)b * n + v] = (uint8_t)(d >> 1);
+            return (unsigned)d;
     };
+    unsigned dbits = 0;
+    (void)dbits;
     if (active) {
         if constexpr (LREG) {
 #pragma unroll
             for (int i = 0; i < NQ; ++i) {
                 const int v = lane + i * tpc;
-                if (v < n) total_body(v, lreg[0][i], lreg[1][i], lreg[2][i]);
+                if (v < n) dbits |= total_body(v, lreg[0][i], lreg[1][i], lreg[2][i]) << (2 * i);
+            }
+        } else if constexpr (NT > 0) {
+#pragma unroll
+            for (int i = 0; i < NT; ++i) {
+                const int v = lane + i * 256;
+                if (i + 1 < NT || v < n) dbits |= total_body(v, a.llr_const, a.llr_const, a.llr_const) << (2 * i);
             }
         } else {
             for (int v = lane; v < n; v += tpc) {
@@ -719,10 +758,19 @@
         uint8_t* dec = reinterpret_cast<uint8_t*>(msg + a.flag_off);
         unsigned* fword = reinterpret_cast<unsigned*>(dec + ((n + 3) & ~3));
         __syncthreads();
-        if (active)
+        if constexpr (READY) {
+            if (active) {
+#pragma unroll
+                for (int i = 0; i < CT; ++i) {
+                    const int v = lane + i * tpc;
+                    if (v < n) dec[v] = (uint8_t)((dbits >> (2 * i)) & 3u);
+                }
+            }
+        } else if (active) {
             for (int v = lane; v < n; v += tpc) {
                 dec[v] = (uint8_t)(a.x_hat[(size_t)b * n + v] | (a.z_hat[(size_t)b * n + v] << 1));
             }
+        }
         if (lane == 0) *fword = 0u;
         __syncthreads();
         unsigned mine = 0;
@@ -730,7 +778,16 @@
             for (int c = lane; c < g.m; c += tpc) {
                 const int sh = c < g.m_x ? 1 : 0;
                 unsigned par = (c < g.m_x ? sx[c] : sz[c - g.m_x]) & 1u;
-                for (int e = g.cptr[c]; e < g.cptr[c + 1]; ++e) par ^= (dec[g.cvn[e]] >> sh) & 1u;
+                if constexpr (READY) {
+                    const uint4 pk = reinterpret_cast<const uint4*>(g.cvn16)[c];
+                    const unsigned w[4] = {pk.x, pk.y, pk.z, pk.w};
+                    unsigned acc = 0;
+#pragma unroll
+                    for (int j = 0; j < DC; ++j) acc ^= dec[(w[j >> 1] >> ((j & 1) * 16)) & 0xffffu];
+                    par ^= (acc >> sh) & 1u;
+                } else {
+                    for (int e = g.cptr[c]; e < g.cptr[c + 1]; ++e) par ^= (dec[g.cvn[e]] >> sh) & 1u;
+                }
                 mine |= par;
             }
         if (mine) atomicOr(fword, 1u);
@@ -741,31 +798,47 @@
     __syncthreads();
     float* llx = msg;
     float* llz = msg + n;
+    float* plx = msg + 2 * n;
+    float* plz = msg + 3 * n;
     if (active)
         for (int v = lane; v < n; v += tpc) {
             const float* o = a.llr_out + (size_t)b * 3 * n;
             const float X = o[v], Y = o[n + v], Z = o[2 * n + v];
             const bool sat = opt_shortcut && FG_ABS(X) > FG_SOFTPLUS_THRESH && FG_ABS(Z) > FG_SOFTPLUS_THRESH &&
                              FG_ABS((-Z) - (-Y)) >= 20.0f && FG_ABS((-X) - (-Y)) >= 20.0f;
+            float lzv, lxv;
             if (opt_shortcut && __all(sat)) {
-                llz[v] = softplus_saturated(-X) - (0.0f + FG_MAX(-Z, -Y));
-                llx[v] = softplus_saturated(-Z) - (0.0f + FG_MAX(-X, -Y));
-                continue;
-            }
-            llz[v] = MX::softplus(-X) - MX::lse2(-Z, -Y);
-            llx[v] = MX::softplus(-Z) - MX::lse2(-X, -Y);
+                lzv = softplus_saturated(-X) - (0.0f + FG_MAX(-Z, -Y));
+                lxv = softplus_saturated(-Z) - (0.0f + FG_MAX(-X, -Y));
+            } else {
+                lzv = MX::softplus(-X) - MX::lse2(-Z, -Y);
+                lxv = MX::softplus(-Z) - MX::lse2(-X, -Y);
+            }
+            llz[v] = lzv;
+            llx[v] = lxv;
+            if constexpr (READY) {
+                const float xa[2] = {FG_ABS(lxv), FG_ABS(lzv)};
+                float oa[2];
+                phi_n<2, false>(xa, oa);
+                plx[v] = oa[0];
+                plz[v] = oa[1];
+            }
         }
     __syncthreads();
+    auto soft_row = [&](const float* llr, const float* phis, const int* col, const int deg) __attribute__((always_inline)) {
+        if constexpr (READY) return logit_row_ready(llr, phis, col, deg, phi0, opt_shortcut);
+        else return logit_row_opt<HWT>(llr, col, deg, phi0, opt_shortcut);
+    };
     if (active) {
         if (a.x_logit)
             for (int r = lane; r < g.rows[0]; r += tpc) {
                 const int p0 = g.rptr[0][r];
-                a.x_logit[(size_t)b * g.rows[0] + r] = logit_row_opt<HWT>(llx, g.rcol[0] + p0, g.rptr[0][r + 1] - p0, phi0, opt_shortcut);
+                a.x_logit[(size_t)b * g.rows[0] + r] = soft_row(llx, plx, g.rcol[0] + p0, g.rptr[0][r + 1] - p0);
             }
         if (a.z_logit)
             for (int r = lane; r < g.rows[1]; r += tpc) {
                 const int p0 = g.rptr[1][r];
-                a.z_logit[(size_t)b * g.rows[1] + r] = logit_row_opt<HWT>(llz, g.rcol[1] + p0, g.rptr[1][r + 1] - p0, phi0, opt_shortcut);
+                a.z_logit[(size_t)b * g.rows[1] + r] = soft_row(llz, plz, g.rcol[1] + p0, g.rptr[1][r + 1] - p0);
             }
     }
 }
@@ -795,6 +868,13 @@
         if constexpr (DVX == 3 && DVZ == 3 && DC == 6) {
             if (!a.trace_x && !a.hwt) kern = bp4_lse_kernels[a.lreg ? a.lreg - 3 : 0][a.shortcut][a.shared_lse];
             if (!a.trace_x && !a.hwt && a.nt) kern = bp4_nt_kernels[a.nt - 4][a.shortcut][a.shared_lse];
+            if (!a.trace_x && !a.hwt && (a.nt || a.lreg)) {
+                hipFuncAttributes fa;
+                FGNN_HIP_CHECK(hipFuncGetAttributes(&fa, reinterpret_cast<const void*>(kern)));
+                if (fa.sharedSizeBytes != (size_t)BP4_STATIC_LDS)
+                    return fgnn_fail(FGNN_ERR_STATE, "bp4_kernel: static LDS is " + std::to_string(fa.sharedSizeBytes) + " bytes, built for " +
+                                                         std::to_string(BP4_STATIC_LDS));
+            }
         }
     }
     return fgnn_launch(kern, dim3(L.blocks), dim3(L.threads), lds_bytes, st, g->d, a);
@@ -831,7 +911,7 @@
     a.lch_off = d.E > 2 * n ? d.E : 2 * n;
     const int per_thread = (n + L.tpc - 1) / L.tpc, per_thread_c = (d.m + L.tpc - 1) / L.tpc;
     const int trips = per_thread > per_thread_c ? per_thread : per_thread_c;
-    const bool r336 = d.cslot16 && !g->force_generic && d.dvx == 3 && d.dvz == 3 && d.dc == 6;
+    const bool r336 = d.cslot16 && d.cslot32 && d.cvn16 && !g->force_generic && d.dvx == 3 && d.dvz == 3 && d.dc == 6;
     const bool fixed_trips = !trace && !a.hwt && !gmem && phi && L.cpb == 1 && r336;
     a.lreg = (a.llr_ch && fixed_trips && trips <= 5) ? (trips <= 4 ? 4 : 5) : 0;
     a.nt = (!a.llr_ch && fixed_trips && L.tpc == 256 && per_thread == per_thread_c && (trips == 4 || trips == 5)) ? trips : 0;
diff --git a/feedback_gnn_amd/csrc/fgnn_channel.hip b/feedback_gnn_amd/csrc/fgnn_channel.hip
--- a/feedback_gnn_amd/csrc/fgnn_channel.hip
+++ b/feedback_gnn_amd/csrc/fgnn_channel.hip
@@ -67,7 +67,7 @@
     return a & 1u;
 }
 
-__global__ void __launch_bounds__(1024) syndrome_kernel(GraphDev g, int B, int tpc, int cpb, const uint8_t* __restrict__ ex,
+__global__ void __launch_bounds__(1024) syndrome_kernel(GraphDev g, int B, int tpc, int cpb, int use_rows, const uint8_t* __restrict__ ex,
                                                         const uint8_t* __restrict__ ez, uint8_t* __restrict__ sx,
                                                         uint8_t* __restrict__ sz)
 {
@@ -84,6 +84,21 @@
         }
     __syncthreads();
     if (!active) return;
+    if (use_rows) {
+        const int dc = g.dc;
+        for (int c = lane; c < g.m; c += tpc) {
+            const uint4 pk = reinterpret_cast<const uint4*>(g.cvn16)[c];
+            const unsigned w[4] = {pk.x, pk.y, pk.z, pk.w};
+            const uint8_t* x = c < g.m_x ? lz : lx;
+            unsigned par = 0;
+#pragma unroll
+            for (int j = 0; j < 8; ++j)
+                if (j < dc) par ^= x[(w[j >> 1] >> ((j & 1) * 16)) & 0xffffu];
+            if (c < g.m_x) sx[(size_t)b * g.m_x + c] = (uint8_t)(par & 1u);
+            else sz[(size_t)b * g.m_z + (c - g.m_x)] = (uint8_t)(par & 1u);
+        }
+        return;
+    }
     for (int c = lane; c < g.m; c += tpc) {
         const int p0 = g.cptr[c], p1 = g.cptr[c + 1];
         if (c < g.m_x) sx[(size_t)b * g.m_x + c] = (uint8_t)row_parity(lz, g.cvn, p0, p1);
@@ -360,7 +375,7 @@
     LaunchGeom L = fgnn_geom(g, B);
     size_t lds = (size_t)L.cpb * 2 * g->d.n;
     return fgnn_launch(syndrome_kernel, dim3(L.blocks), dim3(L.threads), lds, static_cast<hipStream_t>(stream), g->d, B, L.tpc,
-                       L.cpb, noise_x, noise_z, synd_x, synd_z);
+                       L.cpb, (g->d.cvn16 && !g->force_generic) ? 1 : 0, noise_x, noise_z, synd_x, synd_z);
 }
 
 int fgnn_flag_update_impl(const fgnn_graph* g, const uint8_t* x_hat, const uint8_t* z_hat, const uint8_t* synd_x,
diff --git a/feedback_gnn_amd/csrc/fgnn_gnn.hip b/feedback_gnn_amd/csrc/fgnn_gnn.hip
--- a/feedback_gnn_amd/csrc/fgnn_gnn.hip
+++ b/feedback_gnn_amd/csrc/fgnn_gnn.hip
@@ -374,7 +374,11 @@
     for (int e = 0; e < DV; ++e) {
         float ge = gv[0];
 #pragma unroll
-        for (int k = 1; k < DV; ++k) ge = e == k ? gv[k] : ge;
+        for (int k = 1; k < DV; ++k)
+            if (e == k) {
+                ge = gv[k];
+                asm volatile("" : "+v"(ge));
+            }
         f2 m[MSG / 2];
 #pragma unroll
         for (int i = 0; i < MSG / 2; ++i) m[i] = bc2(0.0f);
@@ -391,11 +395,20 @@
 #pragma unroll
             for (int i = 0; i < MSG / 2; ++i) m[i] = pk_fma(h, w2[i], m[i]);
         }
-#pragma unroll
-        for (int i = 0; i < MSG / 2; ++i) {
-            const float m0 = m[i].x + b2[2 * i], m1 = m[i].y + b2[2 * i + 1];
-            feat[2 * i] = (e == 0) ? m0 : feat[2 * i] + m0;
-            feat[2 * i + 1] = (e == 0) ? m1 : feat[2 * i + 1] + m1;
+        if (e == 0) {
+#pragma unroll
+            for (int i = 0; i < MSG / 2; ++i) {
+                feat[2 * i] = m[i].x + b2[2 * i];
+                feat[2 * i + 1] = m[i].y + b2[2 * i + 1];
+            }
+            asm volatile("" : "+v"(feat[0]));
+        } else {
+#pragma unroll
+            for (int i = 0; i < MSG / 2; ++i) {
+                const float m0 = m[i].x + b2[2 * i], m1 = m[i].y + b2[2 * i + 1];
+                feat[2 * i] = feat[2 * i] + m0;
+                feat[2 * i + 1] = feat[2 * i + 1] + m1;
+            }
         }
     }
 #pragma unroll
diff --git a/feedback_gnn_amd/csrc/fgnn_graph.hip b/feedback_gnn_amd/csrc/fgnn_graph.hip
--- a/feedback_gnn_amd/csrc/fgnn_graph.hip
+++ b/feedback_gnn_amd/csrc/fgnn_graph.hip
@@ -1,6 +1,7 @@
 #include <algorithm>
 #include <cstring>
 #include <numeric>
+#include <optional>
 
 #include "fgnn_internal.h"
 
@@ -19,6 +20,10 @@
 template <typename T>
 int upload(fgnn_graph* g, const std::vector<T>& h, const T** dst)
 {
+    if (g->host_only) {
+        *dst = nullptr;
+        return FGNN_OK;
+    }
     void* p = nullptr;
     size_t bytes = std::max<size_t>(h.size(), 1) * sizeof(T);
     FGNN_HIP_CHECK(hipMalloc(&p, bytes));
@@ -86,8 +91,8 @@
     return L;
 }
 
-extern "C" int fgnn_graph_create(int n, int m_x, int m_z, int nnz_x, const int32_t* chk_x, const int32_t* var_x,
-                                 int nnz_z, const int32_t* chk_z, const int32_t* var_z, int device, fgnn_graph** out)
+static int graph_build(int n, int m_x, int m_z, int nnz_x, const int32_t* chk_x, const int32_t* var_x, int nnz_z,
+                       const int32_t* chk_z, const int32_t* var_z, int device, bool host_only, fgnn_graph** out)
 {
     if (!out) return fgnn_fail(FGNN_ERR_ARG, "out is NULL");
     if (n <= 0 || m_x <= 0 || m_z <= 0 || nnz_x <= 0 || nnz_z <= 0)
@@ -100,8 +105,14 @@
         for (int i = 0; i < nnz[s]; ++i)
             if (chk[s][i] < 0 || chk[s][i] >= m[s] || var[s][i] < 0 || var[s][i] >= n)
                 return fgnn_fail(FGNN_ERR_ARG, "edge index out of range");
-    FGNN_DEVICE_GUARD(device);
+    std::optional<fgnn_device_guard> dev_guard;
+    if (!host_only) {
+        dev_guard.emplace(device);
+        if (dev_guard->err != hipSuccess)
+            return fgnn_fail(FGNN_ERR_HIP, std::string("hipSetDevice: ") + hipGetErrorString(dev_guard->err));
+    }
     fgnn_graph* g = new fgnn_graph();
+    g->host_only = host_only;
     std::memset(&g->d, 0, sizeof(g->d));
     std::memset(g->row_alloc, 0, sizeof(g->row_alloc));
     g->device = device;
@@ -169,6 +180,23 @@
             fgnn_graph_destroy(g);
             return rc;
         }
+        std::vector<uint32_t> wide((size_t)d.m * 8, 0);
+        for (size_t i = 0; i < wide.size(); ++i) wide[i] = pk[i];
+        g->h_cslot32 = wide;
+        if ((rc = upload(g, wide, &d.cslot32))) {
+            fgnn_graph_destroy(g);
+            return rc;
+        }
+    }
+    if (d.dc > 0 && d.dc <= 8 && n < 65536) {
+        std::vector<uint16_t> qv((size_t)d.m * 8, 0);
+        for (int c = 0; c < d.m; ++c)
+            for (int j = 0; j < d.dc; ++j) qv[(size_t)c * 8 + j] = (uint16_t)cvn[cptr[c] + j];
+        g->h_cvn16 = qv;
+        if ((rc = upload(g, qv, &d.cvn16))) {
+            fgnn_graph_destroy(g);
+            return rc;
+        }
     }
     if ((rc = upload(g, vptr_x, &d.vptr_x)) || (rc = upload(g, vptr_z, &d.vptr_z)) || (rc = upload(g, vchk, &d.vchk)) ||
         (rc = upload(g, cptr, &d.cptr)) || (rc = upload(g, cslot, &d.cslot)) || (rc = upload(g, cvn, &d.cvn))) {
@@ -180,9 +208,19 @@
     return FGNN_OK;
 }
 
+extern "C" int fgnn_graph_create(int n, int m_x, int m_z, int nnz_x, const int32_t* chk_x, const int32_t* var_x,
+                                 int nnz_z, const int32_t* chk_z, const int32_t* var_z, int device, fgnn_graph** out)
+{
+    return graph_build(n, m_x, m_z, nnz_x, chk_x, var_x, nnz_z, chk_z, var_z, device, false, out);
+}
+
 extern "C" void fgnn_graph_destroy(fgnn_graph* g)
 {
     if (!g) return;
+    if (g->host_only) {
+        delete g;
+        return;
+    }
     fgnn_device_guard _dg(g->device);
     for (hipEvent_t e : g->prof_ev) (void)hipEventDestroy(e);
     for (void* p : g->basis_dev)
@@ -309,6 +347,21 @@
     return FGNN_OK;
 }
 
+extern "C" int fgnn_check_rows(int n, int m_x, int m_z, int nnz_x, const int32_t* chk_x, const int32_t* var_x, int nnz_z,
+                               const int32_t* chk_z, const int32_t* var_z, int32_t have[2], uint32_t* cslot32, uint16_t* cvn16)
+{
+    if (!have) return fgnn_fail(FGNN_ERR_ARG, "have is NULL");
+    fgnn_graph* g = nullptr;
+    const int rc = graph_build(n, m_x, m_z, nnz_x, chk_x, var_x, nnz_z, chk_z, var_z, 0, true, &g);
+    if (rc) return rc;
+    have[0] = !g->h_cslot32.empty();
+    have[1] = !g->h_cvn16.empty();
+    if (cslot32) std::copy(g->h_cslot32.begin(), g->h_cslot32.end(), cslot32);
+    if (cvn16) std::copy(g->h_cvn16.begin(), g->h_cvn16.end(), cvn16);
+    fgnn_graph_destroy(g);
+    return FGNN_OK;
+}
+
 extern "C" int fgnn_profile_enable(fgnn_graph* g, int max_launches)
 {
     if (!g || max_launches < 0) return fgnn_fail(FGNN_ERR_ARG, "bad profile arguments");
diff --git a/feedback_gnn_amd/csrc/fgnn_internal.h b/feedback_gnn_amd/csrc/fgnn_internal.h
--- a/feedback_gnn_amd/csrc/fgnn_internal.h
+++ b/feedback_gnn_amd/csrc/fgnn_internal.h
@@ -15,6 +15,8 @@
     const int* cslot;
     const int* cvn;
     const uint16_t* cslot16;
+    const uint32_t* cslot32;
+    const uint16_t* cvn16;
     int rows[6];
     const int* rptr[6];
     const int* rcol[6];
@@ -39,6 +41,9 @@
     bool force_generic = false;
     std::vector<void*> allocs;
     std::vector<int32_t> h_chk[2], h_var[2];
+    bool host_only = false;
+    std::vector<uint32_t> h_cslot32;
+    std::vector<uint16_t> h_cvn16;
     void* row_alloc[6][4];
     void* basis_dev[2] = {nullptr, nullptr};
     int basis_rank[2] = {0, 0};
diff --git a/include/fgnn.h b/include/fgnn.h
--- a/include/fgnn.h
+++ b/include/fgnn.h
@@ -39,6 +39,8 @@
 int fgnn_graph_force_generic(fgnn_graph* g, int on);
 int fgnn_graph_info(const fgnn_graph* g, int32_t info[16]);
 int fgnn_graph_edges(const fgnn_graph* g, int side, int32_t* chk, int32_t* var);
+int fgnn_check_rows(int n, int m_x, int m_z, int nnz_x, const int32_t* chk_x, const int32_t* var_x, int nnz_z, const int32_t* chk_z,
+                    const int32_t* var_z, int32_t have[2], uint32_t* cslot32, uint16_t* cvn16);
 
 int fgnn_profile_enable(fgnn_graph* g, int max_launches);
 int fgnn_profile_read(fgnn_graph* g, float* ms, int32_t* iters, int32_t* batch, int cap, int32_t* count);
```
